# hiruna72/poregen

Measured on AMD Instinct MI355X. Metric: signal samples/sec aggregated into k-mer buckets, higher is better.
Workload: dtype int16 in / f64 arithmetic; 1 GPU; BASELINE configs[1]: synthetic rna004 SLOW5+PAF, 50000 reads x 4000 samples per GPU, k=5, scaling med-MAD, sample_limit=100, min/max_dur 20/40, --rna; reads_per_gpu=50000, samples_per_gpu=200000000, ss_ops_per_gpu=6499363, n_slots=1024, stats_mode=every read (as the reference), parallelism=read-shard x1

## Files before the change

### poregen_amd/csrc/pg_api.hip

```cpp
#include "../../include/pgmove.h"
#include "pg_internal.h"
#include "pg_hostmem.h"
#include "pg_hip_host.h"
#include "pg_select.h"
#include "pg_stats_plan.h"
#include "pg_model.h"
#include "pg_evstat.h"
#include "pg_modelcols.h"

#include <algorithm>
#include <thread>
#include <climits>
#include <cstdio>
#include <cstring>
#include <map>
#include <string>
#include <vector>

#define PG_VERSION_STR "pgmove 0.1.0 (gfx950)"

namespace {

hipError_t grow(PgDev<> &b, size_t bytes) { return b.ensure(bytes, bytes + bytes / 8 + 256); }

struct HostBatchResult {
    uint64_t n_reads = 0, n_events = 0, n_samples = 0;
    std::vector<uint64_t> keep, ev_off;
    BigVec64 samp_off;
    BigVec32 ev_len, ev_read;
    SampleVec samples;
    std::vector<uint8_t> skipped;
    PgDev<> dsamples; bool on_device = false;
    bool in_ctx = false;
};

struct ProfEntry { const char *name; hipEvent_t a, b; bool bracket; };

struct BatchState {
    PgStatsPlan plan{};
    uint32_t front_tiles = 0;
    bool in_submit = false;
    bool all_matches = false;
    bool cut_in_scan = false;
    bool stats_pending = false;
    bool rare_pending = false;
    PgRareArgs rare{};
};

}

struct pg_ctx {
    pg_params prm{};
    int device = 0;
    hipStream_t st = nullptr;
    PgStream st2, own_st;
    PgEvent ev_fork;
    PgEvent ev_join[2], ev_gathered[2];
    bool slot_used[2] = {false, false};
    PgPinned<PgSettlePack> settle_host;
    int slot = 0;
    bool user_stream = false, batch_is_host = false;
    std::string err;
    uint32_t n_codes = 0, key_bits = 1;

    PgDev<> table_t, table_u;
    int32_t tab_ok[2] = {0, 0}; uint32_t tab_lo[2] = {1, 1}, tab_hi[2] = {0, 0}; int32_t tab_delta[2] = {0, 0};
    PgDev<> s_sig, s_sig_off, s_dig, s_off, s_range, s_qs, s_ts, s_te, s_seq, s_seq_off, s_op_n, s_op_t, s_op_off;
    PgDev<> m_start, m_len, m_base, m_tix, ev_slot, status, errflag;
    PgDev<> sk[2], sv[2], hist, wcnt, totals, dbase, scount;
    PgDev<> slot_start, slot_end, acc_cnt, running, keep, keep32, ev_off, plan_totals, base_stage, tile_last;
    PgDev<> ev_rec, ev_len, ev_read, read_needed, samp_off, scan_scratch, samples;
    bool unpacked = false;
    uint32_t win_hint = 0;
    bool part_mode = false; uint32_t part_hi = 0, part_lo = 0;
    PgDev<> part_elem, part_lodig, part_rbase, part_tile_region, part_ntiles, part_histB, part_Bp, chunk_part, region_state; uint32_t region_epoch = 0;
    PgDev<> med[2], mad[2], gcal[2], read_plan[2], stat_status[2], stat_err[2], wide_list[2];
    PgDev<> long_ring; uint32_t long_seq = 0;
    PgDev<> meta, huge_scratch, oor;
    PgDev<> blk_read, gen_flag, gen_list, cum, btot, tile_read;
    uint32_t batch_id = 0;
    BatchState bt;
    uint64_t front_complete = 0, front_missed = 0, stats_cut_batches = 0, stats_cut_reads = 0, front_one_stream = 0;
    PgEvent ev_front;
    bool prev_one_stream = false;
    uint32_t gen_reads = 0;
    PgDev<> job_total, job_freq; bool have_job_totals = false;
    PgDev<> md_ev_off, md_samp_off, md_ev_len, md_samples, md_out, md_dwell, md_class;
    bool zero_running = false, totals_known = false;
    bool stats_in_flight = false;
    uint32_t wide_blocks = 0;
    PgDev<> cancel_flag; bool cancel_pending = false; uint64_t stats_cancelled = 0;
    PgDev<> long_tab, long_hist; uint32_t long_cap = 0, long_use = 0, long_want = 256; uint64_t long_reads_split = 0, long_helpers_short = 0;
    uint64_t gather_forms[PG_GATHER_FORMS] = {0, 0, 0, 0, 0};
    uint64_t sort_scatters = 0;

    PgDevBatch B{};
    bool have_count = false, have_batch_result = false, downloaded = true;
    int sorted_idx = 0;
    uint64_t cur_n_kept = 0, cur_n_samples = 0;
    uint64_t reads_before = 0;
    uint64_t full_slots = 0;
    bool full_before_batch = false;

    std::vector<HostBatchResult> batches;
    bool single_moved = false;
    bool want_samples = true;
    const double *fin_dev = nullptr;
    bool merged_valid = false;
    uint64_t m_events = 0, m_samples = 0, m_reads = 0;
    std::vector<uint64_t> r_counts, r_ev_off;
    BigVec64 r_samp_off;
    BigVec32 r_ev_len, r_ev_read;
    SampleVec r_samples;
    PgDev<> dmerged, dseg;
    PgDev<> tx_samp_off, tx_ev_off, tx_len, tx_off, tx_text, tx_slot_off, tx_flag;
    std::vector<uint64_t> tx_slot_off_host; uint64_t tx_bytes = 0;
    std::vector<uint8_t> r_skipped;
    std::vector<PgSlotModel> mo_raw;
    std::vector<PgSlotDwell> mo_dw;
    PgModelCols mo;
    PgDev<> me_mean, me_sd, me_flags, me_carry, me_id_off, me_len1, me_out, me_dw;
    std::vector<PgSlotModel> me_raw; std::vector<PgSlotDwell> me_rdw; std::vector<uint32_t> me_rflags;
    PgModelCols me_cm, me_cs;
    std::vector<uint32_t> me_status; std::vector<uint64_t> me_n;

    std::vector<ProfEntry> prof;
    std::vector<std::pair<hipEvent_t, hipEvent_t>> prof_pool;
    std::map<std::string, std::pair<uint64_t, double>> prof_acc;
    std::vector<std::string> prof_names;
};

static const char *read_status_text(int code) {
    switch (code) {
        case PGR_ERR_RNA: return "record is RNA-oriented (target_start > target_end) but allow_rna is 0 (gmove.cpp:795-797)";
        case PGR_ERR_NEG: return "negative PAF column or query_start >= len_raw_signal (assert at gmove.cpp:752)";
        case PGR_ERR_OP: return "ss op type outside {',','I','D'}";
        case PGR_ERR_SEQ_OVERRUN: return "ss consumes more bases than the fetched sequence holds (undefined in the reference, gmove.cpp:850-852)";
        case PGR_ERR_SHORT: return "fewer than k matched bases (unsigned wrap at gmove.cpp:891 in the reference)";
        case PGR_ERR_WINDOW: return "an accepted event has an empty/out-of-signal window or margin > start (undefined in the reference, gmove.cpp:928-941)";
        case PGR_ERR_RANGE: return "sample index exceeds INT32_MAX";
        case PGR_ERR_SCALE: return "range/digitisation is not a positive finite number";
        case PGR_ERR_WIDE: return "internal: statistics histogram too narrow for this read";
        case PGR_ERR_LAYOUT: return "op_off of the device batch is not monotone or ends behind pg_batch.n_ops";
        default: return "unknown";
    }
}

static void prof_begin(pg_ctx *c, const char *name, hipStream_t st, bool bracket = false) {
    if (!(c->prm.flags & PG_FLAG_PROFILE)) return;
    std::pair<hipEvent_t, hipEvent_t> ev;
    if (!c->prof_pool.empty()) { ev = c->prof_pool.back(); c->prof_pool.pop_back(); }
    else { (void)hipEventCreate(&ev.first); (void)hipEventCreate(&ev.second); }
    if (bracket) (void)hipEventRecord(ev.first, st);
    else { pg_prof_start = ev.first; pg_prof_stop = ev.second; }
    c->prof.push_back({name, ev.first, ev.second, bracket});
}
static void prof_end(pg_ctx *c, hipStream_t st) {
    if (!(c->prm.flags & PG_FLAG_PROFILE)) return;
    if (c->prof.back().bracket) { (void)hipEventRecord(c->prof.back().b, st); return; }
    if (pg_prof_start) {
        (void)hipEventRecord(c->prof.back().a, st); (void)hipEventRecord(c->prof.back().b, st);
        pg_prof_start = nullptr; pg_prof_stop = nullptr;
    }
}
static void prof_drain(pg_ctx *c) {
    for (auto &p : c->prof) {
        float ms = 0.f;
        if (hipEventElapsedTime(&ms, p.a, p.b) == hipSuccess) {
            auto it = c->prof_acc.find(p.name);
            if (it == c->prof_acc.end()) { c->prof_acc[p.name] = {1, (double)ms}; c->prof_names.push_back(p.name); }
            else { it->second.first++; it->second.second += ms; }
        }
        c->prof_pool.push_back({p.a, p.b});
    }
    c->prof.clear();
}

extern "C" {

const char *pg_version(void) { return PG_VERSION_STR; }

const char *pg_last_error(const pg_ctx *ctx) { return ctx ? ctx->err.c_str() : pg_create_error<pg_ctx>().c_str(); }

void pg_default_params(pg_params *p) {
    memset(p, 0, sizeof(*p));
    p->struct_size = sizeof(pg_params);
    p->kmer_size = 9; p->sig_move_offset = 0; p->signal_print_margin = 0; p->sample_limit = 100;
    p->max_dur = 70; p->min_dur = 5; p->kmer_pick_margin = 2; p->scaling = 0; p->allow_rna = 0;
    p->pa_min = 40.0; p->pa_max = 180.0; p->n_slots = 0; p->flags = 0; p->device = 0;
}

pg_status pg_build_slot_tables(uint32_t k, const char *const *kmers, uint32_t n_slots, int32_t *table_t, int32_t *table_u) {
    if (k < 1 || k > 13 || !kmers || !table_t || !table_u) return pg_fail<pg_ctx>(nullptr, PG_ERR_INVALID_ARG, "pg_build_slot_tables: bad arguments (1 <= k <= 13)");
    const size_t n_codes = (size_t)1 << (2 * k);
    for (size_t i = 0; i < n_codes; i++) table_t[i] = table_u[i] = -1;
    std::map<std::string, uint32_t> seen;
    for (uint32_t s = 0; s < n_slots; s++) {
        const char *km = kmers[s];
        if (!km || strlen(km) != k) return pg_fail<pg_ctx>(nullptr, PG_ERR_INVALID_ARG, "k-mer %u does not have length %u", s, k);
        if (!seen.emplace(km, s).second) return pg_fail<pg_ctx>(nullptr, PG_ERR_INVALID_ARG, "duplicate k-mer %s in the slice", km);
        uint32_t code = 0; bool has_t = false, has_u = false, other = false;
        for (uint32_t i = 0; i < k; i++) {
            uint32_t b;
            switch (km[i]) {
                case 'A': b = 0; break; case 'C': b = 1; break; case 'G': b = 2; break;
                case 'T': b = 3; has_t = true; break; case 'U': b = 3; has_u = true; break;
                default: b = 0; other = true;
            }
            code = (code << 2) | b;
        }
        if (other || (has_t && has_u)) continue;
        if (!has_u) table_t[code] = (int32_t)s;
        if (!has_t) table_u[code] = (int32_t)s;
    }
    return PG_OK;
}

void pg_destroy(pg_ctx *c) {
    if (!c) return;
    (void)hipSetDevice(c->device);
    if (c->st) (void)hipStreamSynchronize(c->st);
    if (c->st2) (void)hipStreamSynchronize(c->st2);
    for (auto &p : c->prof) { (void)hipEventDestroy(p.a); (void)hipEventDestroy(p.b); }
    for (auto &p : c->prof_pool) { (void)hipEventDestroy(p.first); (void)hipEventDestroy(p.second); }
    delete c;
}

static double wall_now() { struct timespec ts; clock_gettime(CLOCK_MONOTONIC, &ts); return ts.tv_sec + 1e-9 * ts.tv_nsec; }
static bool timing_on() { static const bool on = getenv("PGMOVE_TIMING") != nullptr; return on; }
#define PG_TMARK(label) do { if (timing_on()) { const double n_ = wall_now(); fprintf(stderr, "[pgmove timing] %-34s %8.3f ms\n", label, (n_ - tmark_) * 1e3); tmark_ = n_; } } while (0)

pg_status pg_runtime_init(int32_t device) {
    double tmark_ = timing_on() ? wall_now() : 0.0;
    if (timing_on()) {
        int ndev = 0;
// ... 115 lines not shown
    return PG_OK;
}

static pg_status settle_batch(pg_ctx *c);
static pg_status check_read_errors(pg_ctx *c, const PgSettlePack &pk);
static pg_status ensure_unpacked(pg_ctx *c);

static pg_status download_last(pg_ctx *c, bool more_coming) {
    if (!c->have_batch_result || c->downloaded) return PG_OK;
    { pg_status s0 = settle_batch(c); if (s0 != PG_OK) return s0; }
    c->batches.emplace_back();
    c->merged_valid = false;
    HostBatchResult &h = c->batches.back();
    const uint32_t ns = c->prm.n_slots;
    h.n_reads = c->B.n_reads; h.n_events = c->cur_n_kept; h.n_samples = c->cur_n_samples;
    h.keep.resize(ns); h.ev_off.resize(ns + 1); h.samp_off.resize(h.n_events + 1);
    h.ev_len.resize(h.n_events); h.ev_read.resize(h.n_events); h.samples.resize(h.n_samples);
    PG_HIP_TRY(c, hipMemcpy(h.keep.data(), c->keep.p, ns * 8ull, hipMemcpyDeviceToHost));
    PG_HIP_TRY(c, hipMemcpy(h.ev_off.data(), c->ev_off.p, (ns + 1) * 8ull, hipMemcpyDeviceToHost));
    if (h.n_events) {
        { pg_status su = ensure_unpacked(c); if (su != PG_OK) return su; }
        PG_HIP_TRY(c, hipMemcpy(h.samp_off.data(), c->samp_off.p, (h.n_events + 1) * 8ull, hipMemcpyDeviceToHost));
        PG_HIP_TRY(c, hipMemcpy(h.ev_len.data(), c->ev_len.p, h.n_events * 4ull, hipMemcpyDeviceToHost));
        PG_HIP_TRY(c, hipMemcpy(h.ev_read.data(), c->ev_read.p, h.n_events * 4ull, hipMemcpyDeviceToHost));
    } else h.samp_off[0] = 0;
    const char *hm = getenv("PGMOVE_HOLD_MIN_BYTES");
    const uint64_t hold_min = hm ? strtoull(hm, nullptr, 10) : (8ull << 20);
    if (h.n_samples && !c->want_samples && !more_coming && c->batches.size() == 1) {
        h.on_device = true; h.in_ctx = true;
        h.samples.clear(); h.samples.shrink_to_fit();
    } else if (h.n_samples && h.n_samples * 8ull >= hold_min && (more_coming || c->batches.size() > 1) && !getenv("PGMOVE_HOST_MERGE")) {
        if (grow(h.dsamples, h.n_samples * 8ull) == hipSuccess &&
            hipMemcpyAsync(h.dsamples.p, c->samples.p, h.n_samples * 8ull, hipMemcpyDeviceToDevice, c->st) == hipSuccess) {
            h.on_device = true;
            h.samples.clear(); h.samples.shrink_to_fit();
        } else { (void)hipGetLastError(); h.dsamples.release(); h.samples.resize(h.n_samples); }
    }
    if (h.n_samples && !h.on_device) {
        const uint64_t bytes = h.n_samples * 8ull;
        const unsigned parts = bytes >= (64ull << 20) ? 8u : 1u;
        if (parts == 1) PG_HIP_TRY(c, hipMemcpy(h.samples.data(), c->samples.p, bytes, hipMemcpyDeviceToHost));
        else {
            std::vector<hipError_t> rc(parts, hipSuccess);
            std::vector<std::thread> pool;
            const uint64_t step = ((h.n_samples + parts - 1) / parts + 511) & ~511ull;
            for (unsigned t = 0; t < parts; t++)
                pool.emplace_back([&, t]() {
                    const uint64_t a = std::min<uint64_t>(h.n_samples, t * step), b = std::min<uint64_t>(h.n_samples, a + step);
                    if (b <= a) return;
                    rc[t] = hipSetDevice(c->device);
                    if (rc[t] == hipSuccess) rc[t] = hipMemcpy(h.samples.data() + a, c->samples.as<double>() + a, (b - a) * 8ull, hipMemcpyDeviceToHost);
                });
            for (auto &th : pool) th.join();
            for (hipError_t e : rc) PG_HIP_TRY(c, e);
        }
    }
    std::vector<int32_t> st(h.n_reads);
    if (h.n_reads) PG_HIP_TRY(c, hipMemcpy(st.data(), c->status.p, h.n_reads * 4ull, hipMemcpyDeviceToHost));
    h.skipped.resize(h.n_reads);
    for (uint64_t i = 0; i < h.n_reads; i++) h.skipped[i] = st[i] == PGR_SKIPPED;
    c->downloaded = true;
    return PG_OK;
}

static pg_status stage_host_batch(pg_ctx *c, const pg_batch *b) {
    const uint32_t n = b->n_reads;
    if (!b->sig_off || !b->seq_off || !b->op_off) return pg_fail(c, PG_ERR_INVALID_ARG, "batch offsets missing");
    const uint64_t ns = b->sig_off[n], nq = b->seq_off[n], no = b->op_off[n];
    if (b->sig_off[0] != 0 || b->seq_off[0] != 0 || b->op_off[0] != 0) return pg_fail(c, PG_ERR_INVALID_ARG, "host batch offsets must start at 0");
    uint64_t helpers = 0;
    for (uint32_t r = 0; r < n; r++) {
        if (b->sig_off[r + 1] < b->sig_off[r] || b->seq_off[r + 1] < b->seq_off[r] || b->op_off[r + 1] < b->op_off[r])
            return pg_fail(c, PG_ERR_INVALID_ARG, "batch offsets of read %u are not monotone", r);
        const uint64_t L = b->sig_off[r + 1] - b->sig_off[r];
        if (L > PG_LONG_MIN) { uint32_t S; uint64_t sl; pg_long_geometry(L, &S, &sl); helpers += S - 1; }
    }
    c->long_want = (uint32_t)std::min<uint64_t>(helpers, 1u << 22);
    struct Item { PgDev<> *d; const void *src; size_t bytes; };
    Item items[] = {{&c->s_sig, b->sig, ns * 2}, {&c->s_sig_off, b->sig_off, (n + 1) * 8ull}, {&c->s_dig, b->digitisation, n * 8ull},
                    {&c->s_off, b->offset, n * 8ull}, {&c->s_range, b->range, n * 8ull}, {&c->s_qs, b->query_start, n * 4ull},
                    {&c->s_ts, b->target_start, n * 4ull}, {&c->s_te, b->target_end, n * 4ull}, {&c->s_seq, b->seq, nq},
                    {&c->s_seq_off, b->seq_off, (n + 1) * 8ull}, {&c->s_op_n, b->op_n, no * 4}, {&c->s_op_t, b->op_t, no},
                    {&c->s_op_off, b->op_off, (n + 1) * 8ull}};
    for (auto &it : items) {
        if (it.bytes && !it.src) return pg_fail(c, PG_ERR_INVALID_ARG, "batch array missing");
        PG_HIP_TRY(c, grow(*it.d, it.bytes + 16));
        if (it.bytes) PG_HIP_TRY(c, hipMemcpyAsync(it.d->p, it.src, it.bytes, hipMemcpyHostToDevice, c->st));
    }
    PgDevBatch &B = c->B;
    B.n_reads = n; B.n_ops = no;
    B.sig = c->s_sig.as<int16_t>(); B.sig_off = c->s_sig_off.as<uint64_t>();
    B.dig = c->s_dig.as<double>(); B.off = c->s_off.as<double>(); B.range = c->s_range.as<double>();
    B.qstart = c->s_qs.as<int32_t>(); B.tstart = c->s_ts.as<int32_t>(); B.tend = c->s_te.as<int32_t>();
    B.seq = c->s_seq.as<uint8_t>(); B.seq_off = c->s_seq_off.as<uint64_t>();
    B.op_n = c->s_op_n.as<uint32_t>(); B.op_t = c->s_op_t.as<uint8_t>(); B.op_off = c->s_op_off.as<uint64_t>();
    return PG_OK;
}

static pg_status check_read_errors(pg_ctx *c, const PgSettlePack &pk) {
    struct { unsigned long long word; int32_t layout, pad; uint32_t gen_count[2]; } ef;
    int32_t errv[1] = {INT_MAX}, errs[6] = {INT_MAX, 0, 0, 0, 0, 0};
    static_assert(sizeof ef == sizeof pk.errflag, "PgWalkOut's error words");
    memcpy(&ef, pk.errflag, sizeof ef);
    if (ef.layout) return pg_fail(c, PG_ERR_INVALID_ARG, "pg_batch.n_ops (%llu) is not op_off[n_reads] of the device batch", (unsigned long long)c->B.n_ops);
    if ((uint32_t)(ef.word >> 32) == c->batch_id) errv[0] = (int32_t)(0xFFFFFFFFu - (uint32_t)ef.word);
    c->gen_reads = ef.gen_count[c->batch_id & 1u];
    if (c->bt.all_matches && c->gen_reads) return pg_fail(c, PG_ERR_INVALID_ARG, "pg_batch.flags says PG_BATCH_ALL_MATCHES but %u reads hold I / D / unknown ops (or fewer ops than k, or more than bases)", c->gen_reads);
    memcpy(errs, pk.stat_err, sizeof errs);
    if (errs[4] > 0 || errs[5] > 0) {
        c->long_reads_split += (uint64_t)errs[5];
        if ((uint32_t)errs[4] > c->long_use) c->long_helpers_short++;
    }
    if (!c->batch_is_host) c->long_want = std::max<uint32_t>(256u, errs[4] > 0 ? (uint32_t)errs[4] : 0u);
    c->wide_blocks = errs[1] > 0 ? (uint32_t)errs[1] : 0u;
    if (c->bt.plan.place == PG_STATS_NONE) errs[0] = INT_MAX;
    if (errv[0] == INT_MAX && errs[0] == INT_MAX) return PG_OK;
    const bool walk = errv[0] <= errs[0];
    const int32_t idx = walk ? errv[0] : errs[0];
    if (c->prm.flags & PG_FLAG_STOP_WHEN_FULL) {
        if (c->full_before_batch) return PG_OK;
        const uint64_t tot[2] = {pk.n_kept, pk.full_slots};
        if (tot[1] == c->prm.n_slots && tot[0] == 0) return PG_OK;
        if (tot[1] == c->prm.n_slots && tot[0] > 0) {
            std::vector<uint32_t> er(tot[0]);
            const uint64_t kept_before = c->cur_n_kept; c->cur_n_kept = tot[0];
            const pg_status su = ensure_unpacked(c);
            c->cur_n_kept = kept_before; c->unpacked = false;
            if (su != PG_OK) return su;
            PG_HIP_TRY(c, hipMemcpy(er.data(), c->ev_read.p, tot[0] * 4ull, hipMemcpyDeviceToHost));
            uint32_t last = 0;
            for (uint32_t v : er) last = v > last ? v : last;
            if ((uint32_t)idx > last) return PG_OK;
        }
    }
    int32_t code = 0;
    PG_HIP_TRY(c, hipMemcpy(&code, (walk ? c->status.as<int32_t>() : c->stat_status[c->slot].as<int32_t>()) + idx, 4, hipMemcpyDeviceToHost));
    pg_status s = code == PGR_ERR_RNA ? PG_ERR_RNA_FLAG : (code == PGR_ERR_WIDE ? PG_ERR_UNSUPPORTED : (code == PGR_ERR_LAYOUT ? PG_ERR_INVALID_ARG : PG_ERR_INPUT));
    return pg_fail(c, s, "read %llu of the batch (global read %llu): %s", (unsigned long long)idx,
                (unsigned long long)(c->reads_before + idx), read_status_text(code));
}

static pg_status ensure_stats_buffers(pg_ctx *c) {
    const uint32_t n = c->B.n_reads;
    const int sl = c->slot;
    if (c->prm.flags & PG_FLAG_SKIP_OUT_OF_RANGE) PG_HIP_TRY(c, grow(c->oor, n + 1ull));
    PG_HIP_TRY(c, grow(c->med[sl], (n + 1) * 8ull)); PG_HIP_TRY(c, grow(c->mad[sl], (n + 1) * 8ull));
    PG_HIP_TRY(c, grow(c->gcal[sl], (n + 1) * 32ull));
    PG_HIP_TRY(c, grow(c->read_plan[sl], (n + 1) * (size_t)PG_STAT_REC_BYTES)); PG_HIP_TRY(c, grow(c->wide_list[sl], (n + 1) * 4ull));
    PG_HIP_TRY(c, grow(c->stat_status[sl], (n + 2) * 4ull)); PG_HIP_TRY(c, grow(c->huge_scratch, PG_HUGE_SCRATCH_WORDS * 4));
    return PG_OK;
}

static pg_status fill_long(pg_ctx *c, PgLongState &LS, bool ensure);
static pg_status launch_stats(pg_ctx *c) {
    const PgStatsPlan &P = c->bt.plan;
    hipStream_t st = pg_stats_on_second_stream(P.place) ? c->st2.h : c->st;
    const uint8_t *needed = P.place == PG_STATS_LAZY ? c->read_needed.as<uint8_t>() : nullptr;
    const int sl = c->slot;
    pg_status se = ensure_stats_buffers(c);
    if (se != PG_OK) return se;
    uint8_t *oor = P.place == PG_STATS_OOR_FIRST ? c->oor.as<uint8_t>() : nullptr;
    const int range_only = c->prm.scaling != 1;
    int32_t *flags = c->stat_err[sl].as<int32_t>();
    PgLongState LS{};
    { pg_status sl_ = fill_long(c, LS, false); if (sl_ != PG_OK) return sl_; }
    if (!P.records_in_init) {
        prof_begin(c, "k_read_plan", st);
        PG_HIP_TRY(c, pg_launch_read_plan(st, c->B, needed, c->prm.pa_min, c->prm.pa_max, c->read_plan[sl].p, flags, c->stat_status[sl].as<int32_t>(), P.flags_in_init, LS));
        prof_end(c, st);
    }
    const int win = (c->prm.flags & PG_FLAG_DEBUG_NARROW) ? 0 : 15;
    const bool cut = P.behind_cut;
    if (cut && P.place == PG_STATS_SECOND_STREAM) PG_HIP_TRY(c, hipStreamWaitEvent(st, c->ev_front, 0));
    uint32_t group_from = 0xffffffffu;
    if (cut) {
        const char *ov = getenv("PGMOVE_STATS_GROUP_FROM");
        group_from = ov ? (uint32_t)std::min<unsigned long long>(strtoull(ov, nullptr, 10), 0xffffffffull) : pg_stats_group_from(c->B.n_reads, c->B.n_ops, c->bt.front_tiles);
    }
    prof_begin(c, "k_read_stats", st);
    PG_HIP_TRY(c, pg_launch_read_stats(st, c->B, c->read_plan[sl].p, c->med[sl].as<double>(), c->mad[sl].as<double>(),
                         c->stat_status[sl].as<int32_t>(), flags, win, c->wide_list[sl].as<uint32_t>(), flags + 1, oor, range_only,
                         c->gcal[sl].as<double>(), LS, cut ? c->errflag.as<unsigned long long>() + 5 : nullptr, c->batch_id, group_from));
    prof_end(c, st);
    PgRareArgs &A = c->bt.rare;
    A.B = c->B; A.plan = c->read_plan[sl].as<PgStatRec>(); A.med = c->med[sl].as<double>(); A.mad = c->mad[sl].as<double>(); A.gcal = c->gcal[sl].as<double>();
    A.status = c->stat_status[sl].as<int32_t>(); A.err = flags; A.win = win; A.wide_list = c->wide_list[sl].as<uint32_t>(); A.wide_count = flags + 1;
    A.scratch = c->huge_scratch.as<uint32_t>(); A.oor = oor; A.range_only = range_only; A.wide_blocks = c->wide_blocks;
    if (P.rare_with_scan) c->bt.rare_pending = true;
    else {
        prof_begin(c, "k_read_stats_rare", st);
        PG_HIP_TRY(c, pg_launch_read_stats_rare(st, A));
        prof_end(c, st);
    }
    return PG_OK;
}

static void fill_walk(pg_ctx *c, PgWalkParams &W, PgWalkOut &O) {
    W.k = c->prm.kmer_size; W.sig_move_offset = c->prm.sig_move_offset; W.print_margin = c->prm.signal_print_margin;
    W.max_dur = c->prm.max_dur; W.min_dur = c->prm.min_dur; W.pick_margin = c->prm.kmer_pick_margin; W.allow_rna = c->prm.allow_rna;
    W.short_ok = (c->prm.flags & PG_FLAG_SHORT_READS_OK) ? 1 : 0;
    W.no_generic = c->bt.all_matches ? 1 : 0;
    W.n_codes = c->n_codes; W.table_t = c->table_t.as<int32_t>(); W.table_u = c->table_t.as<int32_t>() + c->n_codes;
    for (int x = 0; x < 2; x++) { W.aff_ok[x] = c->tab_ok[x]; W.aff_lo[x] = c->tab_lo[x]; W.aff_hi[x] = c->tab_hi[x]; W.aff_delta[x] = c->tab_delta[x]; }
    O.m_start = c->m_start.as<uint32_t>(); O.m_len = c->m_len.as<uint32_t>(); O.m_base = c->m_base.as<uint8_t>();
    O.m_tix = c->m_tix.as<uint32_t>() + PG_TIX_FRONT(c->prm.kmer_pick_margin); O.ev_slot = c->ev_slot.as<uint32_t>();
    O.meta = c->meta.as<PgReadMeta>();
    O.status = c->status.as<int32_t>();
    O.err = c->errflag.as<unsigned long long>(); O.layout_err = c->errflag.as<int32_t>() + 2; O.gen_count = c->errflag.as<uint32_t>() + 4;
    O.blk_read = c->blk_read.as<uint32_t>(); O.gen_flag = c->gen_flag.as<uint32_t>(); O.gen_list = c->gen_list.as<uint32_t>();
    O.cum = c->cum.as<uint32_t>(); O.btot = c->btot.as<uint32_t>(); O.batch_id = c->batch_id; O.tile_read = c->tile_read.as<uint32_t>();
    O.oor = (c->prm.flags & PG_FLAG_SKIP_OUT_OF_RANGE) ? c->oor.as<uint8_t>() : nullptr;
}

static pg_status fill_long(pg_ctx *c, PgLongState &LS, bool ensure) {
    LS = PgLongState{};
    if (getenv("PGMOVE_NO_LONG_SPLIT")) return PG_OK;
    if (ensure) {
        const char *ov = getenv("PGMOVE_LONG_HELPERS");
        uint32_t want = ov ? (uint32_t)strtoul(ov, nullptr, 10) : c->long_want;
        if (want > (1u << 22)) want = 1u << 22;
        if (want > c->long_cap || !c->long_tab.p) {
            const uint32_t cap = want + want / 4 + 64;
            PG_HIP_TRY(c, grow(c->long_tab, (size_t)cap * 8));
            const size_t before = c->long_hist.cap;
            PG_HIP_TRY(c, grow(c->long_hist, (size_t)cap * PG_LONG_WORDS * 4));
            if (c->long_hist.cap != before) {
                PG_HIP_TRY(c, hipMemsetAsync(c->long_hist.p, 0, c->long_hist.cap, c->st));
                PG_HIP_TRY(c, hipStreamSynchronize(c->st));
            }
            c->long_cap = cap;
        }
        c->long_use = ov ? std::min<uint32_t>(c->long_cap, want) : std::min<uint32_t>(c->long_cap, want + want / 4 + 64);
    }
    LS.tab = c->long_tab.as<uint2>(); LS.hist = c->long_hist.as<uint32_t>(); LS.cap = c->long_use;
    LS.cnt = c->long_ring.as<int32_t>() + 4u * (c->long_seq & 3u); LS.cnt_next = c->long_ring.as<int32_t>() + 4u * ((c->long_seq + 2u) & 3u);
    return PG_OK;
}

static void fill_sort(pg_ctx *c, PgSortBufs &S, uint32_t n_tiles) {
    S.keys[0] = c->sk[0].as<uint32_t>(); S.keys[1] = c->sk[1].as<uint32_t>();
    S.vals[0] = c->sv[0].as<uint32_t>(); S.vals[1] = c->sv[1].as<uint32_t>();
    S.hist = c->hist.as<uint32_t>(); S.wcnt = c->wcnt.as<uint32_t>(); S.totals = c->totals.as<uint32_t>();
    S.dbase = c->dbase.as<uint32_t>(); S.count = c->scount.as<uint32_t>(); S.n_tiles = n_tiles;
}

static int gather_lanes(const pg_ctx *c) {
    const char *ov = getenv("PGMOVE_GATHER_LANES");
    if (ov) return atoi(ov);
    const uint32_t mw = c->win_hint ? c->win_hint : c->prm.min_dur + (c->prm.max_dur > c->prm.min_dur ? (c->prm.max_dur - c->prm.min_dur) / 8 : 0) + 2 * c->prm.signal_print_margin;
    return mw > 16 ? 1 : 0;
}

static uint64_t dense_min() { const char *e = getenv("PGMOVE_DENSE_MIN"); return e ? strtoull(e, nullptr, 10) : 64ull * 4096; }
static bool dense_direct(const pg_ctx *c, uint64_t n_ops) {
    return c->prm.n_slots <= PG_DIRECT_MAX_SLOTS && std::min<uint64_t>(n_ops, (uint64_t)c->prm.n_slots * c->prm.sample_limit) > dense_min();
}

static uint32_t front_tiles_for(const pg_ctx *c, uint64_t n_ops, bool counts_wanted) {
    if (!c->bt.in_submit || counts_wanted || n_ops == 0 || c->prm.n_slots > PG_DIRECT_MAX_SLOTS || dense_direct(c, n_ops)) return 0;
    if (c->prm.sample_limit == 0 || c->prm.sig_move_offset != 0) return 0;
    const uint32_t n_tiles = pg_tiles(n_ops, true);
    uint64_t f;
    if (const char *ov = getenv("PGMOVE_FRONT_TILES")) f = (strtoull(ov, nullptr, 10) + 3) & ~3ull;
    else {
        f = ((n_tiles + 7) / 8 + 3) & ~3ull;
        if (n_tiles < 64 || f * PG_SORT_TILE < 4ull * c->prm.n_slots * c->prm.sample_limit) return 0;
    }
    return f > 0 && f < n_tiles ? (uint32_t)f : 0;
}

static void fill_part(pg_ctx *c, PgPartBufs &P, uint64_t n_ops) {
    P.elemA = c->part_elem.as<uint4>(); P.loA = c->part_lodig.as<uint16_t>(); P.hist = c->hist.as<uint32_t>(); P.totals = c->totals.as<uint32_t>(); P.rbase = c->part_rbase.as<uint32_t>();
    P.tile_region = c->part_tile_region.as<uint32_t>(); P.n_tilesB = c->part_ntiles.as<uint32_t>(); P.histB = c->part_histB.as<uint32_t>();
    P.Bp = c->part_Bp.as<uint32_t>(); P.hi_bits = c->part_hi; P.lo_bits = c->part_lo; P.tilesB_cap = pg_part_tiles_cap(n_ops, c->part_hi);
}

static pg_status ensure_unpacked(pg_ctx *c) {
    if (c->unpacked) return PG_OK;
    PG_HIP_TRY(c, grow(c->ev_len, (c->cur_n_kept + 1) * 4)); PG_HIP_TRY(c, grow(c->ev_read, (c->cur_n_kept + 1) * 4));
    PG_HIP_TRY(c, pg_launch_unpack_recs(c->st, c->ev_rec.as<PgKeptRec>(), c->cur_n_kept, c->ev_len.as<uint32_t>(), c->ev_read.as<uint32_t>()));
    PG_HIP_TRY(c, hipStreamSynchronize(c->st));
    c->unpacked = true;
    return PG_OK;
}

static pg_status count_impl(pg_ctx *c, const pg_batch *b, uint64_t *counts_out, int32_t counts_location, bool in_submit) {
    if (!c || !b) return PG_ERR_INVALID_ARG;
    if (b->struct_size != sizeof(pg_batch)) return pg_fail(c, PG_ERR_INVALID_ARG, "pg_batch.struct_size mismatch");
    PG_HIP_TRY(c, hipSetDevice(c->device));
    pg_status s = download_last(c, true);
    if (s != PG_OK) return s;
    for (auto &hb : c->batches)
        if (hb.in_ctx) {
            PG_HIP_TRY(c, grow(hb.dsamples, hb.n_samples * 8ull));
            PG_HIP_TRY(c, hipMemcpyAsync(hb.dsamples.p, c->samples.p, hb.n_samples * 8ull, hipMemcpyDeviceToDevice, c->st));
            hb.in_ctx = false; c->merged_valid = false; c->fin_dev = nullptr;
        }
    if (c->have_batch_result) { c->reads_before += c->B.n_reads; c->have_batch_result = false; }
    c->have_count = false;
    c->bt = BatchState{};
    c->bt.in_submit = in_submit;
    const uint32_t n = b->n_reads;

    double tmark_ = timing_on() ? wall_now() : 0.0;
    c->batch_is_host = b->location == PG_LOC_HOST;
    c->bt.all_matches = (b->flags & PG_BATCH_ALL_MATCHES) != 0 && !(c->prm.flags & PG_FLAG_DEBUG_SPLIT_WALK);
    if (b->location == PG_LOC_HOST) {
        s = stage_host_batch(c, b);
        if (s != PG_OK) return s;
        PG_TMARK("count: staging copies queued");
        if (timing_on()) { PG_HIP_TRY(c, hipStreamSynchronize(c->st)); PG_TMARK("count: staging copies done (sync)"); }
    } else if (b->location == PG_LOC_DEVICE) {
        PgDevBatch &B = c->B;
        B.sig = b->sig; B.sig_off = b->sig_off; B.dig = b->digitisation; B.off = b->offset; B.range = b->range;
        B.qstart = b->query_start; B.tstart = b->target_start; B.tend = b->target_end; B.seq = b->seq; B.seq_off = b->seq_off;
        B.op_n = b->op_n; B.op_t = b->op_t; B.op_off = b->op_off;
        if (!B.sig_off || !B.seq_off || !B.op_off) return pg_fail(c, PG_ERR_INVALID_ARG, "batch offsets missing");
        uint64_t no = b->n_ops;
        if (no == 0 && n > 0) {
            PG_HIP_TRY(c, hipMemcpyAsync(&no, b->op_off + n, 8, hipMemcpyDeviceToHost, c->st));
            PG_HIP_TRY(c, hipStreamSynchronize(c->st));
        }
        B.n_reads = n;
        B.n_ops = no;
    } else return pg_fail(c, PG_ERR_INVALID_ARG, "pg_batch.location must be PG_LOC_HOST or PG_LOC_DEVICE");
    if (((uintptr_t)c->B.sig & 15) != 0) return pg_fail(c, PG_ERR_INVALID_ARG, "sig must be 16-byte aligned");
    if (((uintptr_t)c->B.seq & 3) != 0 || ((uintptr_t)c->B.op_n & 15) != 0) return pg_fail(c, PG_ERR_INVALID_ARG, "seq must be 4-byte aligned and op_n 16-byte aligned");
    const uint64_t N = c->B.n_ops;
    if (N >= 0x7fffffffull) return pg_fail(c, PG_ERR_INVALID_ARG, "more than 2^31 ss ops in one batch; split the batch");

    const uint64_t Nn = N ? N : 1;
    const bool direct = c->prm.n_slots <= PG_DIRECT_MAX_SLOTS;
    PG_HIP_TRY(c, grow(c->m_start, (Nn + 32) * 4)); PG_HIP_TRY(c, grow(c->m_len, (Nn + 32) * 4)); PG_HIP_TRY(c, grow(c->m_base, Nn + 32));
    PG_HIP_TRY(c, grow(c->m_tix, (Nn + 64 + c->prm.kmer_size + 2 * PG_TIX_FRONT(c->prm.kmer_pick_margin)) * 4));
    PG_HIP_TRY(c, grow(c->ev_slot, (Nn + 32) * 4));
    PG_HIP_TRY(c, grow(c->blk_read, (Nn / 64 + 2) * 4)); PG_HIP_TRY(c, grow(c->cum, (Nn / 4 + 64) * 4)); PG_HIP_TRY(c, grow(c->btot, (Nn / 256 + 2) * 4));
    PG_HIP_TRY(c, grow(c->gen_list, (n + 1) * 4ull)); PG_HIP_TRY(c, grow(c->tile_read, (Nn / PG_SORT_TILE + 8) * 4));
    {
        const size_t before = c->gen_flag.cap;
        PG_HIP_TRY(c, grow(c->gen_flag, (n + 1) * 4ull));
        if (c->gen_flag.cap != before) PG_HIP_TRY(c, hipMemsetAsync(c->gen_flag.p, 0, c->gen_flag.cap, c->st));
    }
    if (++c->batch_id == 0) {
        c->batch_id = 1;
        PG_HIP_TRY(c, hipMemsetAsync(c->gen_flag.p, 0, c->gen_flag.cap, c->st));
        PG_HIP_TRY(c, hipMemsetAsync(c->errflag.as<uint32_t>() + 8, 0, 16, c->st));
    }
    PG_HIP_TRY(c, grow(c->meta, (n + 1) * sizeof(PgReadMeta))); PG_HIP_TRY(c, grow(c->status, (n + 1) * 4ull));
    PG_HIP_TRY(c, grow(c->read_needed, n + 2ull));
    const uint32_t n_tiles = pg_tiles(Nn, direct);
    uint32_t ndig;
    if (direct) {
        ndig = 2; while (ndig < c->prm.n_slots) ndig <<= 1;
        if (dense_direct(c, N)) { PG_HIP_TRY(c, grow(c->part_Bp, (Nn / 256 + 4) * 4)); PG_HIP_TRY(c, grow(c->chunk_part, PG_CHUNK_PART_N * 8)); }
    }
    else if (c->part_mode) {
        ndig = 1u << c->part_hi;
        const uint32_t tcap = pg_part_tiles_cap(Nn, c->part_hi);
        PG_HIP_TRY(c, grow(c->part_elem, (size_t)tcap * PG_SORT_TILE * 16)); PG_HIP_TRY(c, grow(c->part_lodig, (size_t)tcap * PG_SORT_TILE * 2)); PG_HIP_TRY(c, grow(c->part_rbase, (ndig + 2) * 4ull));
        PG_HIP_TRY(c, grow(c->part_tile_region, (tcap + 1) * 4ull)); PG_HIP_TRY(c, grow(c->part_ntiles, 16));
        PG_HIP_TRY(c, grow(c->part_histB, ((size_t)tcap << c->part_lo) * 4)); PG_HIP_TRY(c, grow(c->part_Bp, (Nn / 256 + 4) * 4));
        PG_HIP_TRY(c, grow(c->chunk_part, PG_CHUNK_PART_N * 8));
    } else {
        const uint32_t passes = (c->key_bits + PG_RANK_MAX_BITS - 1) / PG_RANK_MAX_BITS;
        ndig = 1u << ((c->key_bits + passes - 1) / passes);
        for (int i = 0; i < 2; i++) { PG_HIP_TRY(c, grow(c->sk[i], Nn * 4)); PG_HIP_TRY(c, grow(c->sv[i], Nn * 4)); }
    }
    const uint32_t n_tiles_hist = c->part_mode ? pg_tiles(Nn, true) : n_tiles;
    PG_HIP_TRY(c, grow(c->hist, (size_t)n_tiles_hist * ndig * 4));
    if (!direct && !c->part_mode) PG_HIP_TRY(c, grow(c->wcnt, (size_t)n_tiles * ndig * 16));
    PG_HIP_TRY(c, grow(c->totals, ndig * 4ull)); PG_HIP_TRY(c, grow(c->dbase, ndig * 4ull));

    PG_TMARK("count: work buffers");
    c->full_before_batch = c->full_slots == c->prm.n_slots && c->prm.n_slots > 0;
    c->slot ^= 1;
    c->bt.front_tiles = front_tiles_for(c, N, counts_out != nullptr);
    const PgFront FR{c->bt.front_tiles, c->errflag.as<uint32_t>() + 8};
    const PgStatsPlan P = c->bt.plan = pg_stats_plan(c->prm.flags, c->prm.scaling, FR.tiles, n, getenv("PGMOVE_FRONT_TWO_STREAMS") != nullptr);
    if (P.one_stream_batch && c->stats_in_flight) PG_HIP_TRY(c, hipStreamWaitEvent(c->st, c->ev_join[c->slot ^ 1], 0));
    if (P.place == PG_STATS_SECOND_STREAM) {
        if (pg_stats_fork_waits(c->batch_is_host, c->user_stream, (b->flags & PG_BATCH_RESIDENT) != 0, c->prev_one_stream)) {
            PG_HIP_TRY(c, hipEventRecord(c->ev_fork, c->st));
            PG_HIP_TRY(c, hipStreamWaitEvent(c->st2, c->ev_fork, 0));
        }
        if (c->slot_used[c->slot]) PG_HIP_TRY(c, hipStreamWaitEvent(c->st2, c->ev_gathered[c->slot], 0));
    }
    c->prev_one_stream = P.one_stream_batch;
    if (P.records_in_init) { pg_status se = ensure_stats_buffers(c); if (se != PG_OK) return se; }
    PgWalkParams W{}; PgWalkOut O{};
    fill_walk(c, W, O);
    const bool force_generic = (c->prm.flags & PG_FLAG_DEBUG_SPLIT_WALK) != 0;
    PgLongState LS{};
    ++c->long_seq;
    { pg_status sl_ = fill_long(c, LS, true); if (sl_ != PG_OK) return sl_; }
    prof_begin(c, "k_batch_init", c->st);
    PG_HIP_TRY(c, pg_launch_batch_init(c->st, n, c->read_needed.as<uint8_t>(), c->running.as<uint64_t>(), c->prm.n_slots,
                         c->zero_running ? 1 : 0, P.flags_in_init ? c->stat_err[c->slot].as<int32_t>() : nullptr, c->B, c->prm.pa_min, c->prm.pa_max,
                         P.records_in_init ? c->read_plan[c->slot].p : nullptr, P.records_in_init ? c->stat_status[c->slot].as<int32_t>() : nullptr,
                         W, O, force_generic ? 1 : 0, LS, FR.tiles ? FR.word + 1 : nullptr));
    prof_end(c, c->st);
    c->zero_running = false;

    if (P.place == PG_STATS_OOR_FIRST) {
        pg_status s2 = launch_stats(c); if (s2 != PG_OK) return s2;
        PG_HIP_TRY(c, pg_launch_apply_oor(c->st, c->B, O));
    }
    if (!c->bt.all_matches) {
        prof_begin(c, "k_walk", c->st);
        PG_HIP_TRY(c, pg_launch_walk(c->st, c->B, W, O));
        prof_end(c, c->st);
    }

    PgSortBufs S{};
    fill_sort(c, S, n_tiles);
    prof_begin(c, "k_events", c->st);
    PG_HIP_TRY(c, pg_launch_events(c->st, c->B, W, O, c->prm.n_slots, (direct || c->part_mode) ? S.hist : nullptr, c->part_mode ? c->part_hi : 0u, c->part_lo,
                                   FR, FR.tiles ? PG_PASS_FRONT : PG_PASS_WHOLE));
    prof_end(c, c->st);
    uint64_t *acc_copy = (counts_out && counts_location == PG_LOC_DEVICE) ? counts_out : nullptr;
    if (direct) {
        prof_begin(c, "rank_scan", c->st);
        const bool fuse_plan = c->bt.in_submit;
        PG_HIP_TRY(c, pg_launch_rank_direct_count(c->st, O.ev_slot, N, c->prm.n_slots, S, c->acc_cnt.as<uint64_t>(), c->running.as<uint64_t>(), c->prm.sample_limit,
                                    c->tile_last.as<int32_t>(), acc_copy, fuse_plan ? c->keep.as<uint64_t>() : nullptr, c->ev_off.as<uint64_t>(),
                                    c->plan_totals.as<uint64_t>(), c->errflag.as<uint32_t>() + 6, &c->bt.cut_in_scan,
                                    O.btot, dense_direct(c, N) ? c->part_Bp.as<uint32_t>() : nullptr, dense_direct(c, N) ? c->chunk_part.as<uint64_t>() : nullptr,
                                    FR, FR.tiles ? PG_PASS_FRONT : PG_PASS_WHOLE, c->batch_id, O.tile_read, n));
        prof_end(c, c->st);
        if (P.behind_cut && P.place == PG_STATS_SECOND_STREAM) PG_HIP_TRY(c, hipEventRecord(c->ev_front, c->st));
        if (FR.tiles) {
            prof_begin(c, "k_events_tail", c->st);
            PG_HIP_TRY(c, pg_launch_events(c->st, c->B, W, O, c->prm.n_slots, S.hist, 0u, 0u, FR, PG_PASS_TAIL));
            prof_end(c, c->st);
            prof_begin(c, "rank_scan_tail", c->st);
            PG_HIP_TRY(c, pg_launch_rank_direct_count(c->st, O.ev_slot, N, c->prm.n_slots, S, c->acc_cnt.as<uint64_t>(), c->running.as<uint64_t>(), c->prm.sample_limit,
                                        c->tile_last.as<int32_t>(), nullptr, c->keep.as<uint64_t>(), c->ev_off.as<uint64_t>(), c->plan_totals.as<uint64_t>(),
                                        c->errflag.as<uint32_t>() + 6, &c->bt.cut_in_scan, O.btot, nullptr, nullptr, FR, PG_PASS_TAIL, c->batch_id));
            prof_end(c, c->st);
        }
    } else if (c->part_mode) {
        PgPartBufs P{};
        fill_part(c, P, Nn);
        if (N) {
            prof_begin(c, "part_tile_scan", c->st);
            PG_HIP_TRY(c, pg_launch_part_tile_scan(c->st, P, N, O.btot, c->chunk_part.as<uint64_t>()));
            prof_end(c, c->st);
            prof_begin(c, "k_part_bases", c->st);
            PG_HIP_TRY(c, pg_launch_part_bases(c->st, P, c->B, O));
            prof_end(c, c->st);
            prof_begin(c, "k_part_scatter", c->st);
            PG_HIP_TRY(c, pg_launch_part_scatter(c->st, P, O.ev_slot, N, c->B, W, O));
            prof_end(c, c->st);
            PgRegionCutArgs cut{};
            const bool fuse_cut = c->bt.in_submit && !acc_copy && !getenv("PGMOVE_NO_FUSED_CUT");
            if (fuse_cut) {
                const size_t before = c->region_state.cap;
                PG_HIP_TRY(c, grow(c->region_state, ((size_t)(1u << c->part_hi) + 2) * 8));
                if (c->region_state.cap != before) PG_HIP_TRY(c, hipMemsetAsync(c->region_state.p, 0, c->region_state.cap, c->st));
                if (++c->region_epoch > pg_region_cut_epochs()) { c->region_epoch = 1; PG_HIP_TRY(c, hipMemsetAsync(c->region_state.p, 0, c->region_state.cap, c->st)); }
                PG_HIP_TRY(c, grow(c->keep32, c->prm.n_slots * 4ull));
                cut.running = c->running.as<uint64_t>(); cut.keep = c->keep.as<uint64_t>(); cut.ev_off = c->ev_off.as<uint64_t>(); cut.totals = c->plan_totals.as<uint64_t>();
                cut.keep32 = c->keep32.as<uint32_t>(); cut.state = c->region_state.as<uint64_t>(); cut.limit = c->prm.sample_limit; cut.epoch = c->region_epoch;
            }
            prof_begin(c, "region_counts", c->st, true);
            PG_HIP_TRY(c, pg_launch_region_counts(c->st, P, c->prm.n_slots, c->acc_cnt.as<uint64_t>(), acc_copy, fuse_cut ? &cut : nullptr));
            prof_end(c, c->st);
            c->bt.cut_in_scan = fuse_cut;
        } else {
            PG_HIP_TRY(c, hipMemsetAsync(c->acc_cnt.p, 0, c->prm.n_slots * 8ull, c->st));
            if (acc_copy) PG_HIP_TRY(c, hipMemsetAsync(acc_copy, 0, c->prm.n_slots * 8ull, c->st));
            PG_HIP_TRY(c, hipMemsetAsync(c->part_ntiles.p, 0, 4, c->st));
        }
    } else {
        prof_begin(c, "sort_events", c->st, true);
        if (N) PG_HIP_TRY(c, pg_launch_sort_events(c->st, O.ev_slot, N, c->key_bits, S, &c->sorted_idx, &c->sort_scatters));
        else { c->sorted_idx = 0; PG_HIP_TRY(c, hipMemsetAsync(c->scount.p, 0, 8, c->st)); }
        prof_end(c, c->st);
        prof_begin(c, "slot_bounds", c->st, true);
        PG_HIP_TRY(c, pg_launch_slot_bounds(c->st, S.keys[c->sorted_idx], S.count, N, c->slot_start.as<uint32_t>(), c->slot_end.as<uint32_t>(),
                              c->prm.n_slots, c->acc_cnt.as<uint64_t>(), acc_copy));
        prof_end(c, c->st);
    }

    c->stats_in_flight = false;
    c->bt.stats_pending = P.place == PG_STATS_DEFERRED;
    if (P.place == PG_STATS_SECOND_STREAM || P.place == PG_STATS_CHAIN || P.place == PG_STATS_TAIL_FORK) {
        if (P.place == PG_STATS_TAIL_FORK) {
            PG_HIP_TRY(c, hipEventRecord(c->ev_fork, c->st));
            PG_HIP_TRY(c, hipStreamWaitEvent(c->st2, c->ev_fork, 0));
        }
        pg_status s2 = launch_stats(c);
        if (s2 != PG_OK) return s2;
        if (pg_stats_on_second_stream(P.place)) {
            PG_HIP_TRY(c, hipEventRecord(c->ev_join[c->slot], c->st2));
            c->stats_in_flight = true;
        }
    }

    if (counts_out && counts_location != PG_LOC_DEVICE) {
        PG_HIP_TRY(c, hipMemcpyAsync(counts_out, c->acc_cnt.p, c->prm.n_slots * 8ull, hipMemcpyDeviceToHost, c->st));
        PG_HIP_TRY(c, hipStreamSynchronize(c->st));
    }
    c->have_count = true;
    PG_TMARK("count: kernels queued");
    if (timing_on()) { PG_HIP_TRY(c, hipStreamSynchronize(c->st)); PG_TMARK("count: kernels done (sync)"); }
    return PG_OK;
}

static pg_status collect_impl(pg_ctx *c, const uint64_t *base, int32_t base_location, const uint64_t *all_counts, uint32_t world, uint32_t rank);

pg_status pg_count(pg_ctx *c, const pg_batch *b, uint64_t *counts_out, int32_t counts_location) { return count_impl(c, b, counts_out, counts_location, false); }

static pg_status launch_pending_stats(pg_ctx *c) {
    if (!c->bt.stats_pending) return PG_OK;
    c->bt.stats_pending = false;
    return launch_stats(c);
}

pg_status pg_stats(pg_ctx *c) {
    if (!c) return PG_ERR_INVALID_ARG;
    if (!c->have_count) return pg_fail(c, PG_ERR_STATE, "pg_stats without a preceding pg_count");
    if (!c->bt.stats_pending) return PG_OK;
    PG_HIP_TRY(c, hipSetDevice(c->device));
    return launch_pending_stats(c);
}

pg_status pgi_stats_gathered(pg_ctx *c, const uint64_t *all_counts, uint32_t world, uint32_t rank) {
    if (!c) return PG_ERR_INVALID_ARG;
    if (!c->have_count) return pg_fail(c, PG_ERR_STATE, "pgi_stats_gathered without a preceding pg_count");
    if (!all_counts || rank >= world) return pg_fail(c, PG_ERR_INVALID_ARG, "pgi_stats_gathered: all_counts / world / rank");
    if (!c->bt.stats_pending) return PG_OK;
    if (rank == 0 || c->prm.sample_limit == 0 || !c->bt.plan.records_in_init) return pg_stats(c);
    PG_HIP_TRY(c, hipSetDevice(c->device));
    { pg_status se = ensure_stats_buffers(c); if (se != PG_OK) return se; }
    PG_HIP_TRY(c, grow(c->cancel_flag, 16));
    PG_HIP_TRY(c, pg_launch_stats_cancel_if_full(c->st, all_counts, rank, c->prm.n_slots, c->prm.sample_limit, c->cancel_flag.as<uint32_t>(),
                                              c->read_plan[c->slot].p, c->B.n_reads));
    c->cancel_pending = true;
    return launch_pending_stats(c);
}

pg_status pg_collect(pg_ctx *c, const uint64_t *base, int32_t base_location) { return collect_impl(c, base, base_location, nullptr, 0, 0); }

pg_status pg_collect_gathered(pg_ctx *c, const uint64_t *all_counts, uint32_t world, uint32_t rank) {
    if (!c) return PG_ERR_INVALID_ARG;
    if (!all_counts || world == 0 || rank >= world) return pg_fail(c, PG_ERR_INVALID_ARG, "pg_collect_gathered: all_counts / world / rank");
    return collect_impl(c, nullptr, PG_LOC_DEVICE, all_counts, world, rank);
}

static pg_status collect_impl(pg_ctx *c, const uint64_t *base, int32_t base_location, const uint64_t *all_counts, uint32_t world, uint32_t rank) {
    if (!c) return PG_ERR_INVALID_ARG;
    if (!c->have_count) return pg_fail(c, PG_ERR_STATE, "pg_collect without a preceding pg_count");
    PG_HIP_TRY(c, hipSetDevice(c->device));
    double tmark_ = timing_on() ? wall_now() : 0.0;
    { pg_status s2 = launch_pending_stats(c); if (s2 != PG_OK) return s2; }
    const uint32_t ns = c->prm.n_slots;
    const uint64_t N = c->B.n_ops;
    const bool direct = ns <= PG_DIRECT_MAX_SLOTS;
    const uint64_t *d_base = c->running.as<uint64_t>();
    PgGathered G{};
    if (all_counts) {
        G.all_counts = all_counts; G.world = world; G.rank = rank; G.total = c->job_total.as<uint64_t>(); G.freq = c->job_freq.as<uint64_t>();
        c->have_job_totals = true;
        d_base = nullptr;
    } else if (base) {
        PG_HIP_TRY(c, hipMemcpyAsync(c->base_stage.p, base, ns * 8ull,
                                  base_location == PG_LOC_DEVICE ? hipMemcpyDeviceToDevice : hipMemcpyHostToDevice, c->st));
        d_base = c->base_stage.as<uint64_t>();
    }
    uint64_t *totals = c->plan_totals.as<uint64_t>();
    const uint64_t ke_cap = std::min<uint64_t>(N, (uint64_t)ns * c->prm.sample_limit);
    {
        const size_t before = c->scan_scratch.cap;
        PG_HIP_TRY(c, grow(c->scan_scratch, (std::max<uint64_t>(ke_cap, ns) / 4096 + 84) * 8));
        if (c->scan_scratch.cap != before) PG_HIP_TRY(c, hipMemsetAsync(c->scan_scratch.p, 0, c->scan_scratch.cap, c->st));
    }
    if (!direct) PG_HIP_TRY(c, grow(c->keep32, ns * 4ull));
    const bool plan_in_scan = c->bt.cut_in_scan && !all_counts && !base;
    c->bt.cut_in_scan = false;
    if (!plan_in_scan) {
    prof_begin(c, "k_slot_plan", c->st, true);
    PG_HIP_TRY(c, pg_launch_slot_plan(c->st, c->acc_cnt.as<uint64_t>(), d_base, c->running.as<uint64_t>(), c->prm.sample_limit, ns,
                        c->keep.as<uint64_t>(), c->ev_off.as<uint64_t>(), totals, direct ? c->hist.as<uint32_t>() : nullptr,
                        pg_tiles(N ? N : 1, true), direct ? nullptr : c->keep32.as<uint32_t>(), c->scan_scratch.as<uint64_t>(),
                        direct ? c->tile_last.as<int32_t>() : nullptr, G));
    prof_end(c, c->st);
    }

    const uint64_t win_cap = (uint64_t)c->prm.max_dur + 2ull * c->prm.signal_print_margin;
    const uint64_t samp_cap = ke_cap * win_cap;
    PG_HIP_TRY(c, grow(c->ev_rec, (ke_cap + 1) * sizeof(PgKeptRec)));
    PG_HIP_TRY(c, grow(c->samp_off, (ke_cap + 2) * 8));
    c->unpacked = false;

    PgWalkParams W{}; PgWalkOut O{};
    fill_walk(c, W, O);
    PgKeptOut K{};
    K.rec = c->ev_rec.as<PgKeptRec>();
    K.read_needed = c->bt.plan.place == PG_STATS_LAZY ? c->read_needed.as<uint8_t>() : nullptr;
    const bool chunked = ke_cap > dense_min() && (win_cap + 1) * 4096 < (1ull << 32);
    bool sums_ready = false;
    if (chunked) PG_HIP_TRY(c, grow(c->chunk_part, PG_CHUNK_PART_N * 8));
    if (direct) {
        PgSortBufs S{};
        fill_sort(c, S, 0);
        prof_begin(c, "k_rank_emit", c->st);
        if (dense_direct(c, N)) PG_HIP_TRY(c, pg_launch_rank_emit2(c->st, O.ev_slot, N, ns, S.hist, c->keep.as<uint64_t>(), c->ev_off.as<uint64_t>(), totals, c->B, W, O, K, c->part_Bp.as<uint32_t>()));
        else PG_HIP_TRY(c, pg_launch_rank_direct_emit(c->st, O.ev_slot, N, ns, S, c->keep.as<uint64_t>(), c->ev_off.as<uint64_t>(), totals, c->B, W, O, K));
        prof_end(c, c->st);
    } else if (c->part_mode) {
        PgPartBufs P{};
        fill_part(c, P, N ? N : 1);
        if (N) {
            prof_begin(c, "k_region_place", c->st);
            PG_HIP_TRY(c, pg_launch_region_place(c->st, P, ns, c->keep32.as<uint32_t>(), c->ev_off.as<uint64_t>(), O, K, chunked ? c->chunk_part.as<uint64_t>() : nullptr, chunked ? ke_cap : 0));
            prof_end(c, c->st);
            sums_ready = chunked;
        }
    } else {
        prof_begin(c, "k_kept_meta", c->st, true);
        PG_HIP_TRY(c, pg_launch_kept_meta(c->st, c->sk[c->sorted_idx].as<uint32_t>(), c->sv[c->sorted_idx].as<uint32_t>(), c->scount.as<uint32_t>(), N,
                            c->slot_start.as<uint32_t>(), c->keep.as<uint64_t>(), c->ev_off.as<uint64_t>(), c->B, W, O, K,
                            c->sv[c->sorted_idx ^ 1].as<uint32_t>()));
        prof_end(c, c->st);
    }

    if (c->bt.plan.place == PG_STATS_LAZY) { pg_status s2 = launch_stats(c); if (s2 != PG_OK) return s2; }

    uint64_t gather_cap = ke_cap;
    if (chunked) {
        if (!sums_ready) {
            if (!(direct && dense_direct(c, N)) && !c->part_mode) PG_HIP_TRY(c, hipMemsetAsync(c->chunk_part.p, 0, PG_CHUNK_PART_N * 8, c->st));
            prof_begin(c, "len_partials", c->st);
            PG_HIP_TRY(c, pg_launch_len_partials(c->st, ke_cap, totals, c->ev_rec.as<PgKeptRec>(), c->chunk_part.as<uint64_t>(), c->bt.rare_pending ? &c->bt.rare : nullptr));
            prof_end(c, c->st);
        } else if (c->bt.rare_pending) {
            prof_begin(c, "k_read_stats_rare", c->st);
            PG_HIP_TRY(c, pg_launch_read_stats_rare(c->st, c->bt.rare));
            prof_end(c, c->st);
        }
        c->bt.rare_pending = false;
    } else {
        prof_begin(c, "scan_ev_len", c->st, (ke_cap + 4095) / 4096 > 64);
        PG_HIP_TRY(c, pg_launch_scan_u32_u64(c->st, reinterpret_cast<const uint32_t *>(c->ev_rec.p) + 2, 4, ke_cap, totals, c->samp_off.as<uint64_t>(), c->scan_scratch.as<uint64_t>(),
                                          c->bt.rare_pending ? &c->bt.rare : nullptr, totals + 2));
        c->bt.rare_pending = false;
        prof_end(c, c->st);
    }

    if (samp_cap * 8 > c->samples.cap) {
        size_t mem_free = 0, mem_total = 0;
        if (hipMemGetInfo(&mem_free, &mem_total) != hipSuccess) { (void)hipGetLastError(); mem_total = 0; }
        const uint64_t moderate = std::max<uint64_t>(4ull << 30, std::min<uint64_t>(mem_total / 8, mem_free / 2));
        bool sized = false;
        if (samp_cap * 8 <= moderate && !getenv("PGMOVE_SAMPLES_EXACT")) {
            sized = grow(c->samples, samp_cap * 8 + 8) == hipSuccess;
            if (!sized) (void)hipGetLastError();
        }
        if (!sized) {
            uint64_t tot[3] = {0, 0, 0};
            PG_HIP_TRY(c, hipMemcpyAsync(tot, totals, 24, hipMemcpyDeviceToHost, c->st));
            if (chunked) {
                uint64_t coarse[PG_CHUNK_COARSE];
                PG_HIP_TRY(c, hipMemcpyAsync(coarse, c->chunk_part.as<uint64_t>() + PG_CHUNK_FINE, sizeof coarse, hipMemcpyDeviceToHost, c->st));
                PG_HIP_TRY(c, hipStreamSynchronize(c->st));
                tot[2] = 0;
                for (uint64_t v : coarse) tot[2] += v;
            } else PG_HIP_TRY(c, hipStreamSynchronize(c->st));
            PG_HIP_TRY(c, grow(c->samples, (tot[2] + 1) * 8));
            gather_cap = tot[0];
        }
    }
    if (c->stats_in_flight) { PG_HIP_TRY(c, hipStreamWaitEvent(c->st, c->ev_join[c->slot], 0)); c->stats_in_flight = false; }
    prof_begin(c, "k_gather", c->st);
    const int lanes = chunked ? gather_lanes(c) : 0;
    if (chunked) c->gather_forms[pg_gather_form(lanes)]++;
    if (chunked)
        PG_HIP_TRY(c, pg_launch_gather_chunks(c->st, c->B, ke_cap, totals, c->ev_rec.as<PgKeptRec>(), c->chunk_part.as<uint64_t>(), c->samp_off.as<uint64_t>(), totals + 2, c->prm.scaling,
                                           c->prm.pa_min, c->prm.pa_max, c->samples.as<double>(), c->prm.scaling == 1 ? c->gcal[c->slot].as<double>() : nullptr, lanes,
                                           c->prm.scaling == 1 ? c->stat_err[c->slot].as<int32_t>() : nullptr));
    else
        PG_HIP_TRY(c, pg_launch_gather(c->st, c->B, gather_cap, totals, c->ev_rec.as<PgKeptRec>(),
                     c->samp_off.as<uint64_t>(), c->prm.scaling, c->prm.pa_min, c->prm.pa_max, c->med[c->slot].as<double>(), c->mad[c->slot].as<double>(),
                     c->samples.as<double>(), c->prm.scaling == 1 ? c->gcal[c->slot].as<double>() : nullptr));
    prof_end(c, c->st);
    if (c->st2) PG_HIP_TRY(c, hipEventRecord(c->ev_gathered[c->slot], c->st));
    PG_TMARK("collect: buffers + kernels queued");
    if (timing_on()) { PG_HIP_TRY(c, hipStreamSynchronize(c->st)); PG_TMARK("collect: kernels done (sync)"); }
    c->slot_used[c->slot] = true;
    c->have_count = false; c->have_batch_result = true; c->downloaded = false; c->totals_known = false;
    return PG_OK;
}

static pg_status settle_batch(pg_ctx *c) {
    if (!c->have_batch_result || c->totals_known) return PG_OK;
    if (c->st2) PG_HIP_TRY(c, hipStreamSynchronize(c->st2));
    PG_HIP_TRY(c, pg_launch_settle_pack(c->st, c->errflag.as<uint32_t>(), c->stat_err[c->slot].as<int32_t>(), c->long_ring.as<int32_t>() + 4u * (c->long_seq & 3u), c->plan_totals.as<uint64_t>(),
                                     c->samp_off.as<uint64_t>(), c->samp_off.cap / 8, c->cancel_pending ? c->cancel_flag.as<uint32_t>() : nullptr,
                                     c->bt.front_tiles ? c->errflag.as<uint32_t>() + 8 : nullptr, c->settle_host.p));
    PG_HIP_TRY(c, hipStreamSynchronize(c->st));
    const PgSettlePack pk = *c->settle_host.p;
    if (c->bt.front_tiles) { if (pk.front[0]) c->front_complete++; else c->front_missed++; }
    if (c->bt.plan.one_stream_batch) c->front_one_stream++;
    if (c->bt.plan.behind_cut && pk.front[0]) { c->stats_cut_batches++; c->stats_cut_reads += c->B.n_reads - std::min(pk.front[1], c->B.n_reads); }
    pg_status s = check_read_errors(c, pk);
    if (s != PG_OK) { c->have_batch_result = false; c->downloaded = true; return s; }
    const uint64_t tot[2] = {pk.n_kept, pk.full_slots};
    c->cur_n_kept = tot[0]; c->full_slots = tot[1];
    const uint64_t n_samples = pk.n_samples;
    c->cur_n_samples = n_samples;
    if (c->cancel_pending) {
        if (pk.cancel[1]) c->stats_cancelled++;
        c->cancel_pending = false;
    }
    if (tot[0]) c->win_hint = (uint32_t)((n_samples + tot[0] - 1) / tot[0]);
    c->totals_known = true;
    return PG_OK;
}

pg_status pg_submit(pg_ctx *c, const pg_batch *b) {
    if (!c) return PG_ERR_INVALID_ARG;
    pg_status s = count_impl(c, b, nullptr, PG_LOC_HOST, true);
    if (s != PG_OK) return s;
    return pg_collect(c, nullptr, PG_LOC_HOST);
}

pg_status pg_job_totals_device(pg_ctx *c, const uint64_t **d_total, const uint64_t **d_freq) {
    if (!c) return PG_ERR_INVALID_ARG;
    if (!c->have_job_totals) return pg_fail(c, PG_ERR_STATE, "pg_job_totals_device without a preceding pg_collect_gathered");
    if (d_total) *d_total = c->job_total.as<uint64_t>();
    if (d_freq) *d_freq = c->job_freq.as<uint64_t>();
    return PG_OK;
}

pg_status pg_sync(pg_ctx *c) {
    if (!c) return PG_ERR_INVALID_ARG;
    PG_HIP_TRY(c, hipSetDevice(c->device));
    PG_HIP_TRY(c, hipStreamSynchronize(c->st));
    if (c->st2) PG_HIP_TRY(c, hipStreamSynchronize(c->st2));
    return settle_batch(c);
}

pg_status pg_set_stream(pg_ctx *c, void *hip_stream) {
    if (!c) return PG_ERR_INVALID_ARG;
    PG_HIP_TRY(c, hipSetDevice(c->device));
    PG_HIP_TRY(c, hipStreamSynchronize(c->st));
    if (c->st2) PG_HIP_TRY(c, hipStreamSynchronize(c->st2));
    c->prev_one_stream = false;
    c->st = hip_stream ? (hipStream_t)hip_stream : c->own_st;
    c->user_stream = hip_stream != nullptr;
    return PG_OK;
}

void *pgi_stream(pg_ctx *c) { return c ? (void *)c->st : nullptr; }
const double *pgi_fin_dev(pg_ctx *c) { return c && c->merged_valid ? c->fin_dev : nullptr; }
pg_status pgi_skip_stats(pg_ctx *c) {
    if (!c) return PG_ERR_INVALID_ARG;
    if (!c->have_count) return pg_fail(c, PG_ERR_STATE, "pgi_skip_stats without a preceding pg_count");
    c->bt.stats_pending = false;
    return PG_OK;
}

int32_t pg_all_slots_full(pg_ctx *c) {
    if (!c) return 0;
    if (settle_batch(c) != PG_OK) return 0;
    return c->full_slots == c->prm.n_slots;
}

int32_t pg_poll(pg_ctx *c) {
    if (!c) return PG_ERR_INVALID_ARG;
    if (!c->have_batch_result || c->totals_known) return 1;
    if (hipSetDevice(c->device) != hipSuccess) return PG_ERR_HIP;
    if (hipStreamQuery(c->st) != hipSuccess || (c->st2 && hipStreamQuery(c->st2) != hipSuccess)) { (void)hipGetLastError(); return 0; }
    const pg_status s = settle_batch(c);
    return s == PG_OK ? 1 : s;
}

int32_t pg_all_slots_full_settled(const pg_ctx *c) { return c && c->full_slots == c->prm.n_slots; }
uint64_t pgi_full_slots_settled(const pg_ctx *c) { return c ? c->full_slots : 0; }

pg_status pg_last_batch_device(pg_ctx *c, pg_device_view *v) {
    if (!c || !v) return PG_ERR_INVALID_ARG;
    if (!c->have_batch_result) return pg_fail(c, PG_ERR_STATE, "no collected batch");
    { pg_status s0 = settle_batch(c); if (s0 != PG_OK) return s0; }
    { pg_status su = ensure_unpacked(c); if (su != PG_OK) return su; }
    v->n_events = c->cur_n_kept; v->n_samples = c->cur_n_samples;
    v->d_keep = c->keep.as<uint64_t>(); v->d_ev_off = c->ev_off.as<uint64_t>(); v->d_ev_len = c->ev_len.as<uint32_t>();
    v->d_ev_read = c->ev_read.as<uint32_t>(); v->d_samp_off = c->samp_off.as<uint64_t>(); v->d_samples = c->samples.as<double>();
    v->d_med = c->prm.scaling == 1 ? c->med[c->slot].as<double>() : nullptr; v->d_mad = c->prm.scaling == 1 ? c->mad[c->slot].as<double>() : nullptr;
    return PG_OK;
}

pg_status pg_finish(pg_ctx *c, pg_result *out) {
    if (!c || !out) return PG_ERR_INVALID_ARG;
    PG_HIP_TRY(c, hipSetDevice(c->device));
    pg_status s = download_last(c, false);
    if (s != PG_OK) return s;
    const uint32_t ns = c->prm.n_slots;
    if (c->merged_valid && c->want_samples && c->fin_dev && c->m_samples) {
        c->r_samples.resize(c->m_samples);
        PG_HIP_TRY(c, hipMemcpy(c->r_samples.data(), c->fin_dev, c->m_samples * 8ull, hipMemcpyDeviceToHost));
        c->fin_dev = nullptr;
        for (auto &hb : c->batches) if (hb.on_device && c->batches.size() == 1) { hb.on_device = false; hb.in_ctx = false; hb.dsamples.release(); }
    }
    if (c->merged_valid) {
        out->n_slots = ns; out->reserved = 0; out->n_events = c->m_events; out->n_samples = c->m_samples; out->n_reads = c->m_reads;
        out->counts = c->r_counts.data(); out->ev_off = c->r_ev_off.data(); out->ev_len = c->r_ev_len.data();
        out->ev_read = c->r_ev_read.data(); out->samp_off = c->r_samp_off.data(); out->samples = c->fin_dev ? nullptr : c->r_samples.data();
        out->read_skipped = c->r_skipped.data();
        return PG_OK;
    }
    if (c->single_moved && !c->batches.empty()) {
        HostBatchResult &h = c->batches[0];
        c->r_ev_off.swap(h.ev_off); c->r_samp_off.swap(h.samp_off); c->r_ev_len.swap(h.ev_len); c->r_ev_read.swap(h.ev_read);
        c->r_samples.swap(h.samples); c->r_skipped.swap(h.skipped);
    }
    c->single_moved = false;
    uint64_t n_events = 0, n_samples = 0, n_reads = 0;
    for (auto &h : c->batches) { n_events += h.n_events; n_samples += h.n_samples; n_reads += h.n_reads; }
    if (c->batches.size() == 1) {
        HostBatchResult &h = c->batches[0];
        c->fin_dev = nullptr;
        if (h.on_device && !c->want_samples) c->fin_dev = h.in_ctx ? c->samples.as<double>() : h.dsamples.as<double>();
        else if (h.on_device) {
            h.samples.resize(h.n_samples);
            PG_HIP_TRY(c, hipMemcpy(h.samples.data(), h.in_ctx ? c->samples.p : h.dsamples.p, h.n_samples * 8ull, hipMemcpyDeviceToHost));
            h.dsamples.release(); h.on_device = false; h.in_ctx = false;
        }
        c->r_counts.resize(ns);
        for (uint32_t sl = 0; sl < ns; sl++) c->r_counts[sl] = h.ev_off[sl + 1] - h.ev_off[sl];
        c->r_ev_off.swap(h.ev_off); c->r_samp_off.swap(h.samp_off); c->r_ev_len.swap(h.ev_len); c->r_ev_read.swap(h.ev_read);
        c->r_samples.swap(h.samples); c->r_skipped.swap(h.skipped);
        c->single_moved = true;
        out->n_slots = ns; out->reserved = 0; out->n_events = n_events; out->n_samples = n_samples; out->n_reads = n_reads;
        out->counts = c->r_counts.data(); out->ev_off = c->r_ev_off.data(); out->ev_len = c->r_ev_len.data();
        out->ev_read = c->r_ev_read.data(); out->samp_off = c->r_samp_off.data(); out->samples = c->fin_dev ? nullptr : c->r_samples.data();
        out->read_skipped = c->r_skipped.data();
        c->merged_valid = true; c->m_events = n_events; c->m_samples = n_samples; c->m_reads = n_reads;
        return PG_OK;
    }
    c->fin_dev = nullptr;
    c->r_counts.assign(ns, 0); c->r_ev_off.assign(ns + 1, 0); c->r_samp_off.resize(n_events + 1);
    c->r_ev_len.resize(n_events); c->r_ev_read.resize(n_events);
    c->r_skipped.resize(n_reads);
    std::vector<uint64_t> slot_e(ns + 1, 0), slot_s(ns + 1, 0);
    for (uint32_t sl = 0; sl < ns; sl++) {
        uint64_t ne = 0, nsmp = 0;
        for (auto &h : c->batches) { const uint64_t a = h.ev_off[sl], b = h.ev_off[sl + 1]; ne += b - a; nsmp += h.samp_off[b] - h.samp_off[a]; }
        slot_e[sl + 1] = slot_e[sl] + ne; slot_s[sl + 1] = slot_s[sl] + nsmp;
        c->r_counts[sl] = ne; c->r_ev_off[sl] = slot_e[sl];
    }
    bool all_dev = true;
    for (auto &h : c->batches) if (h.n_samples && !h.on_device) all_dev = false;
    if (all_dev && n_samples) {
        size_t nseg = 0;
        for (uint32_t sl = 0; sl < ns; sl++) for (auto &h : c->batches) nseg += h.ev_off[sl + 1] > h.ev_off[sl];
// ... 186 lines not shown
    c->mo.fill(*out, flags);
    return PG_OK;
}

static pg_status model_arrays(pg_ctx *c, pg_result &R, const uint64_t *&d_ev_off, const uint64_t *&d_samp_off, const uint32_t *&d_ev_len, const double *&d_samples) {
    pg_status s = pg_finish_deferred(c, &R);
    if (s != PG_OK) return s;
    const uint32_t ns = c->prm.n_slots;
    if (c->batches.size() == 1 && c->have_batch_result && c->cur_n_kept == R.n_events && c->cur_n_samples == R.n_samples) {
        { pg_status su = ensure_unpacked(c); if (su != PG_OK) return su; }
        d_ev_off = c->ev_off.as<uint64_t>(); d_samp_off = c->samp_off.as<uint64_t>(); d_ev_len = c->ev_len.as<uint32_t>(); d_samples = c->samples.as<double>();
    } else {
        PG_HIP_TRY(c, grow(c->md_ev_off, (ns + 1) * 8ull)); PG_HIP_TRY(c, grow(c->md_samp_off, (R.n_events + 1) * 8ull));
        PG_HIP_TRY(c, grow(c->md_ev_len, R.n_events * 4ull + 4));
        PG_HIP_TRY(c, hipMemcpyAsync(c->md_ev_off.p, R.ev_off, (ns + 1) * 8ull, hipMemcpyHostToDevice, c->st));
        PG_HIP_TRY(c, hipMemcpyAsync(c->md_samp_off.p, R.samp_off, (R.n_events + 1) * 8ull, hipMemcpyHostToDevice, c->st));
        if (R.n_events) PG_HIP_TRY(c, hipMemcpyAsync(c->md_ev_len.p, R.ev_len, R.n_events * 4ull, hipMemcpyHostToDevice, c->st));
        if (c->fin_dev || !R.n_samples) d_samples = c->fin_dev;
        else {
            PG_HIP_TRY(c, grow(c->md_samples, R.n_samples * 8ull + 8));
            PG_HIP_TRY(c, hipMemcpyAsync(c->md_samples.p, R.samples, R.n_samples * 8ull, hipMemcpyHostToDevice, c->st));
            d_samples = c->md_samples.as<double>();
        }
        d_ev_off = c->md_ev_off.as<uint64_t>(); d_samp_off = c->md_samp_off.as<uint64_t>(); d_ev_len = c->md_ev_len.as<uint32_t>();
    }
    return PG_OK;
}

pg_status pg_model(pg_ctx *c, uint32_t flags, pg_model_result *out) {
    if (!c || !out) return PG_ERR_INVALID_ARG;
    pg_result R;
    const uint64_t *d_ev_off, *d_samp_off; const uint32_t *d_ev_len; const double *d_samples;
    if (pg_status s = model_arrays(c, R, d_ev_off, d_samp_off, d_ev_len, d_samples)) return s;
    const uint32_t ns = c->prm.n_slots;
    int any_kind[PG_MODEL_KINDS] = {0, 0, 0, 0};
    const uint64_t drop = (flags & PG_MODEL_KEEP_FIRST) ? 0 : 1;
    for (uint32_t i = 0; i < ns; i++) {
        const uint64_t all = R.samp_off[R.ev_off[i + 1]] - R.samp_off[R.ev_off[i]], nv = all > drop ? all - drop : 0;
        any_kind[pg_model_kind(nv, R.ev_off[i + 1] - R.ev_off[i])]++;
    }
    return model_run(c, ns, any_kind, d_ev_off, d_samp_off, d_ev_len, d_samples, flags, out);
}

pg_status pg_model_events(pg_ctx *c, uint32_t flags, pg_events_result *out) {
    if (!c || !out) return PG_ERR_INVALID_ARG;
    if (flags) return pg_fail(c, PG_ERR_INVALID_ARG, "pg_model_events: unknown flags 0x%x", flags);
    pg_result R;
    const uint64_t *d_ev_off, *d_samp_off; const uint32_t *d_ev_len; const double *d_samples;
    if (pg_status s = model_arrays(c, R, d_ev_off, d_samp_off, d_ev_len, d_samples)) return s;
    const uint32_t ns = c->prm.n_slots;
    const uint64_t ne = R.n_events, nv = R.n_samples;
    if (ne && R.samp_off[0] != 0) return pg_fail(c, PG_ERR_UNSUPPORTED, "pg_model_events: the kept samples' offsets do not begin at 0");
    for (uint64_t e = 0; e < ne; e++)
        if (R.ev_len[e] == 0) return pg_fail(c, PG_ERR_UNSUPPORTED, "pg_model_events: kept event %llu holds no sample", (unsigned long long)e);
    PG_HIP_TRY(c, grow(c->me_mean, (ne + 1) * 8)); PG_HIP_TRY(c, grow(c->me_sd, (ne + 1) * 8)); PG_HIP_TRY(c, grow(c->me_flags, (ns + 1) * 4ull));
    PG_HIP_TRY(c, grow(c->me_carry, pg_ev_carry_bytes(nv))); PG_HIP_TRY(c, grow(c->me_id_off, (ne + 1) * 8)); PG_HIP_TRY(c, grow(c->me_len1, (ne + 1) * 4));
    PG_HIP_TRY(c, grow(c->me_out, 2 * (ns + 1ull) * sizeof(PgSlotModel))); PG_HIP_TRY(c, grow(c->me_dw, 2 * (ns + 1ull) * sizeof(PgSlotDwell)));
    PG_HIP_TRY(c, grow(c->md_class, pg_slot_model_scratch_bytes(ns)));
    int64_t *ev_mean = c->me_mean.as<int64_t>(), *ev_sd = c->me_sd.as<int64_t>();
    PgSlotModel *om = c->me_out.as<PgSlotModel>(); PgSlotDwell *od = c->me_dw.as<PgSlotDwell>();
    PG_HIP_TRY(c, hipMemsetAsync(c->me_flags.p, 0, (ns + 1) * 4ull, c->st));
    PG_HIP_TRY(c, pg_launch_ev_identity(c->st, ne, c->me_id_off.as<uint64_t>(), c->me_len1.as<uint32_t>()));
    prof_begin(c, "k_ev_stats", c->st, true);
    PG_HIP_TRY(c, pg_launch_ev_stats(c->st, ns, d_ev_off, d_samp_off, d_samples, ne, nv, ev_mean, ev_sd, c->me_flags.as<uint32_t>(), c->me_carry.p));
    prof_end(c, c->st);
    const int all_kinds[PG_MODEL_KINDS] = {1 << 20, 1 << 20, 1 << 20, 1 << 20};
    PG_HIP_TRY(c, pg_launch_slot_model_units(c->st, ns, all_kinds, d_ev_off, c->me_id_off.as<uint64_t>(), c->me_len1.as<uint32_t>(), ev_mean, 0u, om, od, c->md_class.p));
    PG_HIP_TRY(c, pg_launch_slot_model_units(c->st, ns, all_kinds, d_ev_off, c->me_id_off.as<uint64_t>(), c->me_len1.as<uint32_t>(), ev_sd, 0u, om + ns, od + ns, c->md_class.p));
    c->me_raw.resize(2 * (size_t)ns); c->me_rdw.resize(2 * (size_t)ns); c->me_rflags.resize(ns);
    if (ns) {
        PG_HIP_TRY(c, hipMemcpyAsync(c->me_raw.data(), om, 2 * (size_t)ns * sizeof(PgSlotModel), hipMemcpyDeviceToHost, c->st));
        PG_HIP_TRY(c, hipMemcpyAsync(c->me_rdw.data(), od, 2 * (size_t)ns * sizeof(PgSlotDwell), hipMemcpyDeviceToHost, c->st));
        PG_HIP_TRY(c, hipMemcpyAsync(c->me_rflags.data(), c->me_flags.p, (size_t)ns * 4, hipMemcpyDeviceToHost, c->st));
    }
    PG_HIP_TRY(c, hipStreamSynchronize(c->st));
    c->me_cm.clear(); c->me_cs.clear(); c->me_status.clear(); c->me_n.clear();
    for (uint32_t i = 0; i < ns; i++) {
        const uint32_t declined = (c->me_rdw[i].flags | c->me_rdw[ns + i].flags) & (PG_MODEL_BAD_VALUE | PG_MODEL_BAD_SPREAD | PG_MODEL_BAD_COUNT);
        uint32_t st = (c->me_rflags[i] & 15u) << 1;
        if (!st && declined) st = PG_EVENTS_DECLINED;
        c->me_status.push_back(st); c->me_n.push_back(R.ev_off[i + 1] - R.ev_off[i]);
        c->me_cm.push(st ? PgSlotModel{} : c->me_raw[i]); c->me_cs.push(st ? PgSlotModel{} : c->me_raw[ns + i]);
    }
    c->me_cm.fill(out->means, PG_MODEL_KEEP_FIRST); c->me_cs.fill(out->sds, PG_MODEL_KEEP_FIRST);
    out->status = c->me_status.data(); out->n_events = c->me_n.data();
    return PG_OK;
}

pg_status pg_model_device(pg_ctx *c, uint32_t n_slots, const uint64_t *d_ev_off, const uint64_t *d_samp_off, const uint32_t *d_ev_len,
                          const double *d_samples, uint32_t flags, pg_model_result *out) {
    if (!c || !out) return PG_ERR_INVALID_ARG;
    if (n_slots && (!d_ev_off || !d_samp_off)) return pg_fail(c, PG_ERR_INVALID_ARG, "pg_model_device: ev_off / samp_off missing");
    PG_HIP_TRY(c, hipSetDevice(c->device));
    const int all_kinds[PG_MODEL_KINDS] = {1 << 20, 1 << 20, 1 << 20, 1 << 20};
    return model_run(c, n_slots, all_kinds, d_ev_off, d_samp_off, d_ev_len, d_samples, flags, out);
}

size_t pg_model_format(const pg_model_result *m, uint32_t slot, int32_t which, char *buf, size_t cap) {
    if (!m || !buf || cap == 0 || slot >= m->n_slots) return 0;
    int w = 0;
    buf[0] = 0;
    if (which == PG_MODEL_TEXT_DWELL) {
        if (m->dwell_n[slot] == 0) return 0;
        w = snprintf(buf, cap, "%.14Lg", (long double)m->dwell_median[slot]);
    } else if (which == PG_MODEL_TEXT_MEDIAN || which == PG_MODEL_TEXT_SSTDEV) {
        if (m->n_values[slot] == 0) return 0;
        PgSlotModel r{};
        r.n = m->n_values[slot]; r.mid_lo = m->mid_lo[slot]; r.mid_hi = m->mid_hi[slot]; r.s1 = m->sum1[slot];
        if (which == PG_MODEL_TEXT_MEDIAN) w = snprintf(buf, cap, "%.14Lg", pg_model_median(r));
        else if (r.n < 2) w = snprintf(buf, cap, "nan");
        else {
            const unsigned __int128 s2 = ((unsigned __int128)m->sum2_hi[slot] << 64) | m->sum2_lo[slot];
            const __int128 s1 = r.s1;
            const unsigned __int128 num = (unsigned __int128)r.n * s2 - (unsigned __int128)(s1 * s1);
            w = pg_model_sstdev_text(r.n, num, buf, cap);
        }
    } else return 0;
    return (w < 0 || (size_t)w >= cap) ? 0 : (size_t)w;
}

pg_status pg_kernel_stats(pg_ctx *c, pg_kernel_stat *out, uint32_t cap, uint32_t *n_out) {
    if (!c || !n_out) return PG_ERR_INVALID_ARG;
    PG_HIP_TRY(c, hipSetDevice(c->device));
    PG_HIP_TRY(c, hipStreamSynchronize(c->st));
    if (c->st2) PG_HIP_TRY(c, hipStreamSynchronize(c->st2));
    prof_drain(c);
    uint32_t n = 0;
    for (auto &name : c->prof_names) {
        if (out && n < cap) { auto &a = c->prof_acc[name]; out[n].name = name.c_str(); out[n].launches = a.first; out[n].total_ms = a.second; }
        n++;
    }
    if (c->stats_cancelled) {
        if (out && n < cap) { out[n].name = "stats_cancelled_on_device"; out[n].launches = c->stats_cancelled; out[n].total_ms = 0.0; }
        n++;
    }
    if (c->long_reads_split) {
        if (out && n < cap) { out[n].name = "long_reads_split"; out[n].launches = c->long_reads_split; out[n].total_ms = 0.0; }
        n++;
    }
    if (c->front_complete) {
        if (out && n < cap) { out[n].name = "front_complete"; out[n].launches = c->front_complete; out[n].total_ms = 0.0; }
        n++;
    }
    if (c->front_missed) {
        if (out && n < cap) { out[n].name = "front_missed"; out[n].launches = c->front_missed; out[n].total_ms = 0.0; }
        n++;
    }
    if (c->stats_cut_batches) {
        if (out && n < cap) { out[n].name = "stats_cut_batches"; out[n].launches = c->stats_cut_batches; out[n].total_ms = 0.0; }
        n++;
        if (out && n < cap) { out[n].name = "stats_cut_reads"; out[n].launches = c->stats_cut_reads; out[n].total_ms = 0.0; }
        n++;
    }
    if (c->front_one_stream) {
        if (out && n < cap) { out[n].name = "front_one_stream"; out[n].launches = c->front_one_stream; out[n].total_ms = 0.0; }
        n++;
    }
    if (c->long_helpers_short) {
        if (out && n < cap) { out[n].name = "long_helpers_short_batches"; out[n].launches = c->long_helpers_short; out[n].total_ms = 0.0; }
        n++;
    }
    static const char *const form_names[PG_GATHER_FORMS] = {"gather_form_wave", "gather_form_evpair", "gather_form_lanes4", "gather_form_lanes8", "gather_form_lanes16"};
    for (int f = 0; f < PG_GATHER_FORMS; ++f)
        if (c->gather_forms[f]) {
            if (out && n < cap) { out[n].name = form_names[f]; out[n].launches = c->gather_forms[f]; out[n].total_ms = 0.0; }
            n++;
        }
    if (c->sort_scatters) {
        if (out && n < cap) { out[n].name = "k_sort_scatter"; out[n].launches = c->sort_scatters; out[n].total_ms = 0.0; }
        n++;
    }
    *n_out = n;
    return PG_OK;
}

pg_status pg_kernel_stats_reset(pg_ctx *c) {
    if (!c) return PG_ERR_INVALID_ARG;
    PG_HIP_TRY(c, hipStreamSynchronize(c->st));
    if (c->st2) PG_HIP_TRY(c, hipStreamSynchronize(c->st2));
    prof_drain(c);
    c->prof_acc.clear(); c->prof_names.clear(); c->stats_cancelled = 0; c->long_reads_split = 0; c->long_helpers_short = 0; c->front_complete = 0; c->front_missed = 0; c->stats_cut_batches = 0; c->stats_cut_reads = 0; c->front_one_stream = 0;
    for (uint64_t &f : c->gather_forms) f = 0;
    c->sort_scatters = 0;
    return PG_OK;
}

}
```

### poregen_amd/csrc/pg_hosttest.cpp

```cpp
#include "pg_select.h"
#include <vector>
#include <cstdint>
#include <cstring>

extern "C" int pgt_plan(double dig, double off, double range, double pa_min, double pa_max, int32_t *out4) {
    PgReadPlan p = pg_make_plan(dig, off, range, pa_min, pa_max);
    out4[0] = p.c_lo; out4[1] = p.span; out4[2] = p.z0; out4[3] = p.status;
    return p.status;
}

extern "C" int pgt_medmad(const int16_t *raw, uint64_t n, double dig, double off, double range,
                          double pa_min, double pa_max, double *med, double *mad, double *mad_raw) {
    PgReadPlan p = pg_make_plan(dig, off, range, pa_min, pa_max);
    if (p.status != 0) return p.status;
    std::vector<uint32_t> pre((size_t)(p.span > 0 ? p.span : 1), 0u);
    for (uint64_t i = 0; i < n; i++) {
        int idx = (int)raw[i] - p.c_lo;
        if (idx >= 0 && idx < p.span) pre[(size_t)idx]++;
    }
    for (int b = 1; b < p.span; b++) pre[(size_t)b] += pre[(size_t)b - 1];
    PgMedMad mm = pg_medmad_from_prefix(pre.data(), p, n, off, range / dig);
    *med = mm.med; *mad = mm.mad; *mad_raw = mm.mad_raw;
    return 0;
}
// ... 22 lines not shown
}
extern "C" int pgt_div_domain_ok(double offset, double scale) { return pg_div_domain_ok(offset, scale) ? 1 : 0; }

#include "host/pg_host.h"
#include <cstring>
#include <string>

extern "C" size_t pgt_format_f8(double v, char *buf) { return pgh::format_f8(v, buf); }

extern "C" long pgt_tokenize_ss(const char *ss, uint32_t *op_n, uint8_t *op_t, size_t cap) {
    std::vector<uint32_t> n; std::vector<uint8_t> t; std::string err;
    if (!pgh::tokenize_ss(ss, strlen(ss), n, t, err)) return -1;
    for (size_t i = 0; i < n.size() && i < cap; i++) { op_n[i] = n[i]; op_t[i] = t[i]; }
    return (long)n.size();
}

extern "C" long pgt_fastx_fetch(const char *path, const char *name, long beg, long end, char *out, size_t cap) {
    pgh::FastxIndex fx; std::string err, s;
    if (!fx.load(path, err)) return -3;
    if (!fx.fetch(name, beg, end, s)) return -2;
    if (s.size() < cap) { memcpy(out, s.data(), s.size()); out[s.size()] = 0; }
    return (long)s.size();
}

extern "C" long pgt_slow5_get(const char *path, const char *read_id, double *dig_off_range, int16_t *raw, size_t cap) {
    pgh::Slow5File f; std::string err;
    if (!f.open(path, err)) return -1;
    pgh::Slow5Rec r;
    if (!f.get(read_id, r, err)) return -1;
    dig_off_range[0] = r.digitisation; dig_off_range[1] = r.offset; dig_off_range[2] = r.range;
    for (size_t i = 0; i < r.raw.size() && i < cap; i++) raw[i] = r.raw[i];
    return (long)r.raw.size();
}

extern "C" long pgt_slow5_count(const char *path) {
    pgh::Slow5File f; std::string err;
    if (!f.open(path, err)) return -1;
    return (long)f.n_reads();
}

extern "C" int pgt_parse_paf(char *line, int32_t *cols6, char *rid, char *tid, char *ss, size_t cap) {
    pgh::PafRec p;
    int rc = pgh::parse_paf_line(line, strlen(line), p);
    if (rc != 0) return rc;
    cols6[0] = p.qlen; cols6[1] = p.query_start; cols6[2] = p.query_end; cols6[3] = p.tlen; cols6[4] = p.target_start; cols6[5] = p.target_end;
    snprintf(rid, cap, "%s", p.rid.c_str()); snprintf(tid, cap, "%s", p.tid.c_str());
    if (p.ss_len < cap) { memcpy(ss, p.ss, p.ss_len); ss[p.ss_len] = 0; }
    return 0;
}

extern "C" long pgt_sam_first(const char *path, char *qname, char *seq, size_t cap, long long *stride_ns_ts, uint8_t *is_one, size_t mcap) {
    pgh::SamBamReader r; std::string err;
    if (!r.open(path, err)) return -1;
    pgh::MoveRec m;
    if (r.next(m, err) != 1) return -1;
    snprintf(qname, cap, "%s", m.qname.c_str()); snprintf(seq, cap, "%s", m.seq.c_str());
    stride_ns_ts[0] = m.stride; stride_ns_ts[1] = m.has_ns ? (long long)m.ns : -1; stride_ns_ts[2] = m.has_ts ? (long long)m.ts : -1;
    const long n_moves = (long)m.is_one.size();
    for (size_t i = 0; i < m.is_one.size() && i < mcap; i++) is_one[i] = m.is_one[i];
    pgh::MoveRec m2;
    if (r.next(m2, err) != 0) return -2;
    return n_moves;
}

#include "pg_model.h"
#include <algorithm>
#include <cstdio>
extern "C" long long pgt_fixed8(double x, int *bad) { bool b = false; const long long v = pg_fixed8(x, b); *bad = b; return v; }
extern "C" void pgt_model_texts(const long long *units, size_t n, char *med, char *sd, size_t cap) {
    std::vector<long long> v(units, units + n);
    PgSlotModel m{};
    m.n = n; m.origin = n ? v[0] : 0;
    for (size_t i = 0; i < n; i++) {
        const long long d = v[i] - m.origin; const unsigned long long ad = (unsigned long long)(d < 0 ? -d : d);
        const unsigned long long h = ad >> PG_MODEL_LIMB_BITS, l = ad & ((1u << PG_MODEL_LIMB_BITS) - 1);
        m.s1 += d; m.s2_hh += h * h; m.s2_hl += h * l; m.s2_ll += l * l;
    }
    std::sort(v.begin(), v.end());
    if (n) { m.mid_lo = v[(n - 1) / 2]; m.mid_hi = v[n / 2]; }
    med[0] = sd[0] = 0;
    if (!n) return;
    snprintf(med, cap, "%.14Lg", pg_model_median(m));
    if (n < 2) snprintf(sd, cap, "nan");
    else {
        const unsigned __int128 s2 = ((unsigned __int128)m.s2_hh << 40) + ((unsigned __int128)m.s2_hl << 21) + m.s2_ll;
        const __int128 s1 = m.s1;
        pg_model_sstdev_text(n, (unsigned __int128)n * s2 - (unsigned __int128)(s1 * s1), sd, cap);
    }
}
extern "C" void pgt_sstdev_text(unsigned long long n, unsigned long long num_hi, unsigned long long num_lo, char *exact, char *plain, size_t cap) {
    const unsigned __int128 num = ((unsigned __int128)num_hi << 64) | num_lo;
    pg_model_sstdev_text(n, num, exact, cap);
    snprintf(plain, cap, "%.14Lg", sqrtl((long double)num / ((long double)n * (long double)(n - 1))) / 1e8L);
}

#include "pg_hostmem.h"
#include <fstream>
#include <sstream>
extern "C" int pgt_samplevec_hugepage(size_t n, long *anon_huge_kb) {
    SampleVec v;
    v.resize(n);
    for (size_t i = 0; i < n; i += 512) v[i] = 1.0;
    const uintptr_t p = reinterpret_cast<uintptr_t>(v.data());
    std::ifstream f("/proc/self/smaps");
    if (!f) return -1;
    std::string line; bool inside = false; int hg = 0; long ahp = 0;
    while (std::getline(f, line)) {
        unsigned long a = 0, b = 0;
        if (sscanf(line.c_str(), "%lx-%lx ", &a, &b) == 2) { inside = p >= a && p < b; continue; }
        if (!inside) continue;
        if (line.rfind("AnonHugePages:", 0) == 0) ahp = atol(line.c_str() + 14);
        if (line.rfind("VmFlags:", 0) == 0) { std::istringstream is(line.substr(8)); std::string t; while (is >> t) if (t == "hg") hg = 1; }
    }
    if (anon_huge_kb) *anon_huge_kb = ahp;
    return hg;
}

static void put_err(const std::string &e, char *errbuf, size_t cap) { if (errbuf && cap) { const size_t n = e.size() < cap - 1 ? e.size() : cap - 1; memcpy(errbuf, e.data(), n); errbuf[n] = 0; } }
extern "C" long pgt_slow5_scan(const char *path, char *errbuf, size_t cap) {
    pgh::Slow5File f; std::string err;
    if (!f.open(path, err)) { put_err(err, errbuf, cap); return -1; }
    long n = 0;
    for (const std::string &id : f.ids_in_file_order()) {
        pgh::Slow5Rec r;
        if (!f.get(id, r, err)) { put_err(err, errbuf, cap); return -1; }
        ++n;
    }
    return n;
}
extern "C" long pgt_sambam_scan(const char *path, char *errbuf, size_t cap) {
    pgh::SamBamReader rd; std::string err;
    if (!rd.open(path, err)) { put_err(err, errbuf, cap); return -1; }
    long n = 0;
    for (;;) {
        pgh::MoveRec m;
        const int rc = rd.next(m, err);
        if (rc < 0) { put_err(err, errbuf, cap); return -1; }
        if (rc == 0) break;
        ++n;
    }
    return n;
}

#include "pg_job_rule.h"
extern "C" int pgt_job_stats_rule(uint32_t rank, const uint64_t *shard_ops, const uint64_t *shard_reads, uint32_t n_slots, uint64_t sample_limit,
                                  int have_batch, uint64_t full_slots_prev, const char *mode) {
    return (int)pg_job_stats_place(rank, shard_ops, shard_reads, n_slots, sample_limit, have_batch != 0, full_slots_prev, mode && *mode ? mode : nullptr);
}

#include "pg_stats_plan.h"
extern "C" void pgt_stats_plan(uint32_t ctx_flags, int32_t scaling, uint32_t front_tiles, uint32_t n_reads, int front_two_streams, int32_t *out6) {
    const PgStatsPlan p = pg_stats_plan(ctx_flags, scaling, front_tiles, n_reads, front_two_streams != 0);
    out6[0] = p.place; out6[1] = p.behind_cut; out6[2] = p.one_stream_batch; out6[3] = p.records_in_init; out6[4] = p.flags_in_init; out6[5] = p.rare_with_scan;
}
extern "C" int pgt_stats_fork_waits(int batch_is_host, int user_stream, int batch_resident, int prev_one_stream) {
    return pg_stats_fork_waits(batch_is_host != 0, user_stream != 0, batch_resident != 0, prev_one_stream != 0) ? 1 : 0;
}

#include "pg_pamean.h"
extern "C" int pgt_pa_shift(double offset) { return pg_pa_shift(offset); }
extern "C" int pgt_pa_certify(uint64_t n, int64_t s1, uint64_t sa, double offset, double scale, double *mean) {
    return pg_pa_certify(n, s1, sa, pg_pa_shift(offset), offset, scale, mean);
}
extern "C" double pgt_pa_sequential_mean(const int16_t *raw, uint64_t n, double dig, double off, double range) {
    return pg_pa_sequential_mean(raw, n, dig, off, range);
}
extern "C" long pgt_slow5_walk(const char *path, char *ids, size_t cap, uint64_t *lens, size_t max, char *errbuf, size_t ecap) {
    pgh::Slow5File f; std::string err, all;
    if (!f.open_walk(path, err)) { put_err(err, errbuf, ecap); return -1; }
    for (size_t i = 0; i < f.n_records(); i++) {
        std::string id; pgh::Slow5Rec r;
        if (!f.record(i, id, r, err)) { put_err(err, errbuf, ecap); return -1; }
        all += id; all += '\n';
        if (i < max) lens[i] = r.raw.size();
    }
    if (all.size() < cap) { memcpy(ids, all.data(), all.size()); ids[all.size()] = 0; }
    return (long)f.n_records();
}

#include "pg_svb.h"
extern "C" int pgt_svb_check(uint64_t len, uint32_t count) { return pg_svb_check(len, count); }
extern "C" uint64_t pgt_svb_nctrl(uint32_t count) { return pg_svb_nctrl(count); }
extern "C" void pgt_svb_levels(uint32_t *out3) { out3[0] = PG_SVB_LANE_VALUES; out3[1] = PG_SVB_WAVE_VALUES; out3[2] = PG_SVB_PIECE_VALUES; }
extern "C" long pgt_slow5_svb_walk(const char *path, uint32_t *counts, uint64_t *lens, size_t max, uint8_t *blocks, size_t cap, char *errbuf, size_t ecap) {
    pgh::Slow5File f; std::string err;
    if (!f.open_walk(path, err)) { put_err(err, errbuf, ecap); return -1; }
    if (!f.has_svb_views()) { put_err("no svb-zd signals", errbuf, ecap); return -1; }
    size_t at = 0;
    for (size_t i = 0; i < f.n_records(); i++) {
        std::string id; pgh::Slow5File::SvbView v; std::vector<unsigned char> inflated;
        if (!f.record_svb(i, id, v, inflated, err)) { put_err("record " + std::to_string(i) + ": " + err, errbuf, ecap); return -1; }
        if (i < max) { counts[i] = v.count; lens[i] = v.len; }
        if (at + v.len <= cap) memcpy(blocks + at, v.block, v.len);
        at += v.len;
    }
    return (long)f.n_records();
}

#include "pg_dumphost.h"
#include "host/pg_dumpdir.h"
extern "C" long pgt_dump_model_host(const char *const *dirs, size_t n_dirs, int which, const char *limit, int keep_first, int n_threads,
                                    char *out, size_t cap, char *errbuf, size_t ecap) {
    pgh::DumpSet ds; std::string err, text;
    if (!pgh::list_dump_dirs(std::vector<std::string>(dirs, dirs + n_dirs), n_threads, ds, err)) { put_err(err, errbuf, ecap); return -1; }
    std::vector<uint8_t> bytes; std::vector<uint64_t> off;
    if (!pgh::read_dump_files(ds, 0, ds.names.size(), n_threads, bytes, off, err)) { put_err(err, errbuf, ecap); return -1; }
    for (size_t i = 0; i < ds.names.size(); i++) {
        const char *b = reinterpret_cast<const char *>(bytes.data()) + off[i];
        const size_t len = off[i + 1] - off[i];
        text += ds.names[i]; text += '\t';
        if (which == 0) {
            PgDumpHostStats hs;
            pg_dump_host_stats(b, len, keep_first != 0, hs);
            text += hs.median; text += '\t'; text += pg_dump_sd_capped(hs.sstdev.c_str(), limit) ? std::string(limit) : hs.sstdev;
        } else {
            PgDumpHostDwell hd;
            pg_dump_host_dwell(b, len, hd);
            char t[64]; t[0] = 0;
            if (hd.n) snprintf(t, sizeof t, "%.14Lg", ((long double)hd.mid_lo + (long double)hd.mid_hi) / 2.0L);
            text += t;
        }
        text += '\n';
    }
    if (out && cap) { const size_t n = text.size() < cap - 1 ? text.size() : cap - 1; memcpy(out, text.data(), n); out[n] = 0; }
    return (long)text.size();
}

#include "pg_kfreq_codes.h"
extern "C" int pgt_kf_code_of_byte(int byte) { return (int)pg_kf_code_of_byte((uint32_t)byte & 0xff); }
extern "C" int pgt_kf_letter(int code) { return (int)pg_kf_letter((uint32_t)code & 15); }
extern "C" int pgt_kf_complement(int code) { return (int)pg_kf_complement((uint32_t)code & 15); }

#include "pg_kfreq_fasta.h"
#include <map>
namespace {
constexpr uint64_t kFaTile = (uint64_t)kFaSpan * kFaTileSpans;
struct FaHostSink {
    uint32_t k; std::map<uint32_t, uint64_t> *hist; std::map<std::string, uint64_t> *odd_map;
    void dense(uint32_t code) { (*hist)[code]++; }
    void odd(uint64_t lo, uint32_t hi) {
        std::string key(k, '\0');
        for (uint32_t i = 0; i < k; i++) { const uint32_t sh = k - 1 - i; key[i] = (char)(sh < 8 ? lo >> (8 * sh) : hi >> (8 * (sh - 8))); }
        (*odd_map)[key]++;
    }
};
struct FaHostLoad {
    const uint8_t *p; uint64_t base, n;
    void operator()(uint32_t ch, uint32_t (&ws)[4]) const {
        for (int i = 0; i < 4; i++) ws[i] = 0;
        for (uint32_t b = 0; b < 16; b++) { const uint64_t o = base + 16 * ch + b; if (o < n) ws[b >> 2] |= (uint32_t)p[o] << (8 * (b & 3)); }
    }
};
struct FaHostState { uint32_t kind; PgFaSum rec; };
uint32_t fa_host_span(const uint8_t *p, uint64_t base, uint64_t n, PgFaSpan &sp) {
    uint32_t w[kFaSpan / 4];
    FaHostLoad load{p, base, n};
    for (uint32_t ch = 0; ch < kFaSpan / 16; ch++) { uint32_t ws[4]; load(ch, ws); for (int i = 0; i < 4; i++) w[4 * ch + i] = ws[i]; }
    pg_fa_span_summary(w, (uint32_t)std::min<uint64_t>(kFaSpan, n - base), sp);
    return w[0] & 0xff;
}
bool fa_host_unit(const uint8_t *p, uint64_t n, uint32_t k, FaHostState &st, FaHostSink &sink) {
    const uint64_t n_tiles = (n + kFaTile - 1) / kFaTile;
    std::vector<uint64_t> tile_ls(n_tiles, 0);
    std::vector<PgFaSum> tile_fa(n_tiles), tile_pb(n_tiles);
    for (uint64_t t = 0; t < n_tiles; t++) {
        const uint64_t tile0 = t * kFaTile, tile_end = std::min<uint64_t>(n, tile0 + kFaTile);
        uint64_t ls = 0, fa_end = tile_end;
        PgFaSum rest = pg_fa_empty();
        for (uint64_t base = tile0; base < tile_end; base += kFaSpan) {
            PgFaSpan sp;
            const uint32_t first_byte = fa_host_span(p, base, n, sp);
            rest = pg_fa_compose(rest, ls ? pg_fa_resolve(pg_fa_kind_at(p, ls, base, PG_FA_SEQ), first_byte, sp.fa, sp.pb) : sp.pb);
            if (sp.has_nl) {
                if (!ls) { fa_end = base; while (p[fa_end] != '\n') fa_end++; }
                ls = base + sp.last_nl + 1;
            }
        }
        PgFaSum f = pg_fa_empty();
        for (uint64_t q = fa_end - tile0 > kFaTail ? fa_end - kFaTail : tile0; q < fa_end; q++) pg_fa_append(f, p[q]);
        tile_ls[t] = ls; tile_fa[t] = f; tile_pb[t] = rest;
    }
    bool bad = false;
    uint64_t line_in = 0;
    PgFaSum rec_in = st.rec;
    for (uint64_t t = 0; t < n_tiles; t++) {
        const uint64_t tile0 = t * kFaTile, tile_end = std::min<uint64_t>(n, tile0 + kFaTile);
        uint64_t ls = line_in;
        PgFaSum rec = rec_in;
        for (uint64_t base = tile0; base < tile_end; base += kFaSpan) {
            PgFaSpan sp;
            const uint32_t first_byte = fa_host_span(p, base, n, sp);
            const uint32_t kind = pg_fa_kind_at(p, ls, base, st.kind);
            FaHostLoad load{p, base, n};
            bad |= pg_fa_walk(load, (uint32_t)std::min<uint64_t>(kFaSpan, n - base), k, kind, rec, sink);
            rec = pg_fa_compose(rec, pg_fa_resolve(kind, first_byte, sp.fa, sp.pb));
            if (sp.has_nl) ls = base + sp.last_nl + 1;
        }
        rec_in = pg_fa_compose(rec_in, pg_fa_resolve(pg_fa_kind_at(p, line_in, tile0, st.kind), p[tile0], tile_fa[t], tile_pb[t]));
        line_in = std::max(line_in, tile_ls[t]);
    }
    st.kind = pg_fa_kind_at(p, line_in, n, st.kind);
    st.rec = rec_in;
    return bad;
}
}
extern "C" long pgt_kf_fasta(const uint8_t *data, uint64_t n, const uint64_t *cuts, size_t n_cuts, uint32_t k, uint64_t unit,
// ... 389 lines not shown
```

### poregen_amd/csrc/pg_internal.h

```cpp
#pragma once
#include <hip/hip_runtime.h>
#include <stdint.h>

struct PgDevBatch {
    uint32_t n_reads;
    uint64_t n_ops;
    const int16_t *sig;
    const uint64_t *sig_off;
    const double *dig, *off, *range;
    const int32_t *qstart, *tstart, *tend;
    const uint8_t *seq;
    const uint64_t *seq_off;
    const uint32_t *op_n;
    const uint8_t *op_t;
    const uint64_t *op_off;
};

struct PgWalkParams {
    uint32_t k, sig_move_offset, print_margin, max_dur, min_dur;
    int32_t pick_margin, allow_rna, short_ok;
    int32_t no_generic;
    uint32_t n_codes;
    const int32_t *table_t, *table_u;
    int32_t aff_ok[2]; uint32_t aff_lo[2], aff_hi[2]; int32_t aff_delta[2];
// ... 114 lines not shown
hipError_t pg_launch_len_partials(hipStream_t st, uint64_t n_kept_cap, const uint64_t *n_kept_ptr, const PgKeptRec *rec, uint64_t *part, const PgRareArgs *rare);
uint32_t pg_gather_chunks(uint64_t n_kept_cap, uint32_t *sub_per_chunk);
#define PG_GATHER_FORMS 5
int pg_gather_form(int lanes);
hipError_t pg_launch_gather_chunks(hipStream_t st, const PgDevBatch &B, uint64_t n_kept_cap, const uint64_t *n_kept_ptr, const PgKeptRec *rec, const uint64_t *part,
                                   uint64_t *samp_off, uint64_t *total_out, int scaling, double pa_min, double pa_max, double *samples, const double *gcal, int lanes,
                                   const int32_t *stat_flags );
hipError_t pg_launch_text_lens(hipStream_t st, const double *samples, const uint64_t *samp_off, uint64_t n_events, uint32_t *tlen, uint32_t *flag);
hipError_t pg_launch_text_write(hipStream_t st, const double *samples, const uint64_t *samp_off, uint64_t n_events, const uint64_t *toff, char *text,
                                const uint64_t *ev_off, uint32_t n_slots, uint64_t *slot_toff);
hipError_t pg_launch_unpack_recs(hipStream_t st, const PgKeptRec *rec, uint64_t n, uint32_t *ev_len, uint32_t *ev_read);

#define PG_STATS_BINS 2048
#define PG_HUGE_BLOCKS 64
struct PgStatRec {
    uint64_t beg, end;
    int32_t c_lo, span, z0;
    int32_t mode;
    double offset, scale;
    double inv;
    uint32_t sym;
    uint32_t split;
};
enum { PG_STAT_RUN = 0, PG_STAT_SKIP = 1, PG_STAT_BAD = 2 };
#ifndef PG_LONG_MIN
#define PG_LONG_MIN 32768u
#endif
#ifndef PG_LONG_SLICE
#define PG_LONG_SLICE 16384u
#endif
#define PG_LONG_MAX_SLICES 1024u
#define PG_LONG_WORDS 1128u
#define PG_LONG_INVALID 0xFFFFFFFFu
struct PgLongState {
    uint2 *tab;
    uint32_t *hist;
    int32_t *cnt;
    int32_t *cnt_next;
    uint32_t cap;
};
static inline __host__ __device__ void pg_long_geometry(uint64_t L, uint32_t *slices, uint64_t *slen) {
    uint64_t sl = PG_LONG_SLICE;
    while ((L + sl - 1) / sl > PG_LONG_MAX_SLICES) sl *= 2;
    *slen = sl; *slices = (uint32_t)((L + sl - 1) / sl);
}
#define PG_STAT_REC_BYTES 64
#define PG_HUGE_SCRATCH_WORDS ((size_t)PG_HUGE_BLOCKS * (65536 + 64))

struct PgGathered {
    const uint64_t *all_counts;
    uint32_t world, rank;
    uint64_t *total, *freq;
};
struct PgFront { uint32_t tiles; uint32_t *word; };
enum { PG_PASS_WHOLE = 0, PG_PASS_FRONT = 1, PG_PASS_TAIL = 2 };
struct __attribute__((aligned(16))) PgKeptRec {
    uint64_t src;
    uint32_t len;
    uint32_t read;
};
struct PgKeptOut {
    PgKeptRec *rec;
    uint8_t *read_needed;
};
extern thread_local hipEvent_t pg_prof_start, pg_prof_stop;
hipError_t pg_launch_batch_init(hipStream_t st, uint32_t n_reads, uint8_t *read_needed, uint64_t *running, uint32_t n_slots,
                          int zero_running, int32_t *stat_flags,
                          const PgDevBatch &B, double pa_min, double pa_max, void *plan_buf, int32_t *stat_status,
                          const PgWalkParams &W, const PgWalkOut &O, int force_generic, const PgLongState &LS,
                          uint32_t *big_op = nullptr);
static inline uint32_t pg_tiles(uint64_t n_events, bool direct) {
    const uint64_t t = (n_events + PG_SORT_TILE - 1) / PG_SORT_TILE;
    return (uint32_t)(direct ? (t + 3) & ~3ull : t);
}
struct PgSlotModel; struct PgSlotDwell;
hipError_t pg_launch_slot_model(hipStream_t st, uint32_t n_slots, const int any_kind[4], const uint64_t *ev_off, const uint64_t *samp_off,
                                const uint32_t *ev_len, const double *samples, uint32_t drop_first, PgSlotModel *out, PgSlotDwell *dwell,
                                void *scratch );
hipError_t pg_launch_slot_model_units(hipStream_t st, uint32_t n_slots, const int any_kind[4], const uint64_t *ev_off, const uint64_t *samp_off,
                                      const uint32_t *ev_len, const int64_t *units, uint32_t drop_first, PgSlotModel *out, PgSlotDwell *dwell, void *scratch);
size_t pg_slot_model_scratch_bytes(uint32_t n_slots);
struct PgDtBatch {
    const uint8_t *p; uint64_t n;
    const uint64_t *file_off; uint32_t n_files;
    uint32_t n_tiles;
    uint2 *tile_pre;
    uint32_t *fflags;
    uint2 *fstart;
    uint64_t *val_base;
    uint64_t *ev_off;
    int64_t *units; uint64_t *samp_off; uint32_t *ev_len;
    uint64_t cap_values;
};
hipError_t pg_launch_dump_parse(hipStream_t st, const PgDtBatch &b);
static inline uint64_t pg_ev_tiles(uint64_t cap_values) { return (cap_values + 127) / 128 + 1; }
size_t pg_ev_carry_bytes(uint64_t cap_values);
hipError_t pg_launch_ev_stats_units(hipStream_t st, uint32_t n_files, const uint64_t *ev_off, const uint64_t *samp_off, const int64_t *units, uint64_t cap_events,
                                    uint64_t cap_values, int64_t *ev_mean, int64_t *ev_sd, uint32_t *fflags, void *carry);
hipError_t pg_launch_ev_stats(hipStream_t st, uint32_t n_files, const uint64_t *ev_off, const uint64_t *samp_off, const double *samples, uint64_t cap_events,
                              uint64_t cap_values, int64_t *ev_mean, int64_t *ev_sd, uint32_t *fflags, void *carry);
hipError_t pg_launch_ev_identity(hipStream_t st, uint64_t n, uint64_t *id_off, uint32_t *len1);
hipError_t pg_launch_walk(hipStream_t st, const PgDevBatch &B, const PgWalkParams &W, const PgWalkOut &O);
hipError_t pg_launch_events(hipStream_t st, const PgDevBatch &B, const PgWalkParams &W, const PgWalkOut &O, uint32_t n_slots, uint32_t *hist,
                            uint32_t part_hi_bits, uint32_t part_lo_bits, const PgFront &F = PgFront{}, int pass = PG_PASS_WHOLE);
hipError_t pg_launch_apply_oor(hipStream_t st, const PgDevBatch &B, const PgWalkOut &O);
hipError_t pg_launch_rank_direct_count(hipStream_t st, const uint32_t *ev_slot, uint64_t n, uint32_t n_slots, const PgSortBufs &S,
                                 uint64_t *acc_cnt, uint64_t *running, uint32_t limit, int32_t *tile_last,
                                 uint64_t *acc_copy ,
                                 uint64_t *plan_keep, uint64_t *plan_ev_off, uint64_t *plan_totals, uint32_t *plan_ticket, bool *plan_done,
                                 const uint32_t *btot , uint32_t *Bp ,
                                 uint64_t *zero64 ,
                                 const PgFront &F = PgFront{}, int pass = PG_PASS_WHOLE, uint32_t batch_id = 0,
                                 const uint32_t *tile_read = nullptr, uint32_t n_reads = 0);
hipError_t pg_launch_rank_direct_emit(hipStream_t st, const uint32_t *ev_slot, uint64_t n, uint32_t n_slots, const PgSortBufs &S,
                                const uint64_t *keep, const uint64_t *ev_off, const uint64_t *totals, const PgDevBatch &B,
                                const PgWalkParams &W, const PgWalkOut &O, const PgKeptOut &K);
hipError_t pg_launch_sort_events(hipStream_t st, const uint32_t *ev_slot, uint64_t n, uint32_t key_bits, const PgSortBufs &S, int *sorted_idx,
                                 uint64_t *scatter_launches);
hipError_t pg_launch_slot_bounds(hipStream_t st, const uint32_t *skey, const uint32_t *m_ptr, uint64_t n_upper,
                           uint32_t *slot_start, uint32_t *slot_end, uint32_t n_slots, uint64_t *acc_cnt, uint64_t *acc_copy);
hipError_t pg_launch_kept_meta(hipStream_t st, const uint32_t *skey, const uint32_t *sval, const uint32_t *m_ptr, uint64_t n_upper,
                         const uint32_t *slot_start, const uint64_t *keep, const uint64_t *ev_off,
                         const PgDevBatch &B, const PgWalkParams &W, const PgWalkOut &O, const PgKeptOut &K, uint32_t *dst_scratch);
hipError_t pg_launch_slot_plan(hipStream_t st, const uint64_t *acc_cnt, const uint64_t *base, uint64_t *running,
                         uint32_t limit, uint32_t n_slots, uint64_t *keep, uint64_t *ev_off, uint64_t *totals,
                         const uint32_t *hist, uint32_t n_tiles, uint32_t *keep32, uint64_t *scan_scratch,
                         const int32_t *tile_last ,
                         const PgGathered &G );
struct PgRareArgs {
    PgDevBatch B;
    const PgStatRec *plan;
    double *med, *mad, *gcal;
    int32_t *status, *err;
    int win;
    const uint32_t *wide_list;
    const int32_t *wide_count;
    uint32_t *scratch;
    uint8_t *oor;
    int range_only;
    uint32_t wide_blocks;
};
hipError_t pg_launch_scan_u32_u64(hipStream_t st, const uint32_t *in, uint32_t stride, uint64_t n_cap, const uint64_t *n_ptr, uint64_t *out, uint64_t *scratch,
                                  const PgRareArgs *rare, uint64_t *total_out);
hipError_t pg_launch_read_stats_rare(hipStream_t st, const PgRareArgs &A);
struct PgSettlePack { uint32_t errflag[6]; int32_t stat_err[6]; uint64_t n_kept, full_slots, n_samples; uint32_t cancel[2]; uint32_t front[2]; };
hipError_t pg_launch_settle_pack(hipStream_t st, const uint32_t *errflag, const int32_t *stat_err, const int32_t *long_cnt, const uint64_t *totals, const uint64_t *samp_off,
                                 uint64_t samp_off_entries, const uint32_t *cancel_flag, const uint32_t *front_word, PgSettlePack *out);
hipError_t pg_launch_stats_cancel_if_full(hipStream_t st, const uint64_t *all_counts, uint32_t rows_below, uint32_t n_slots, uint64_t limit, uint32_t *flag, void *plan_buf, uint32_t n_reads);
hipError_t pg_launch_read_plan(hipStream_t st, const PgDevBatch &B, const uint8_t *read_needed, double pa_min, double pa_max, void *plan_buf,
                         int32_t *flags, int32_t *stat_status, bool flags_are_reset, const PgLongState &LS);
hipError_t pg_launch_read_stats(hipStream_t st, const PgDevBatch &B, const void *plan_buf, double *med, double *mad, int32_t *status, int32_t *err, int win,
                                uint32_t *wide_list, int32_t *wide_count, uint8_t *oor, int range_only, double *gcal, const PgLongState &LS,
                                const unsigned long long *cut_word = nullptr, uint32_t batch_id = 0, uint32_t group_from = 0xffffffffu);
uint32_t pg_stats_group_from(uint32_t n_reads, uint64_t n_ops, uint32_t front_tiles);
struct PgSeg { const double *src; uint64_t dst_off, n; };
hipError_t pg_launch_merge_segments(hipStream_t st, const PgSeg *d_seg, uint32_t n_seg, double *dst, uint64_t n_total );
hipError_t pg_launch_gather(hipStream_t st, const PgDevBatch &B, uint64_t n_kept_cap, const uint64_t *n_kept_ptr, const PgKeptRec *rec,
                      const uint64_t *samp_off, int scaling, double pa_min,
                      double pa_max, const double *med, const double *mad, double *samples, const double *gcal);
```

### poregen_amd/csrc/pg_kernels.hip

```cpp
#include "pg_dev.h"
#include "pg_select.h"
#include <limits.h>
#include <type_traits>

#ifdef PG_PHASE_PROBE
#define PG_PROBE_WAVES 65536
__device__ unsigned long long g_pg_phase[3][PG_PROBE_WAVES][8];
extern "C" void pg_debug_phases(unsigned long long *out, int kernel, int reset) {
    (void)hipMemcpyFromSymbol(out, HIP_SYMBOL(g_pg_phase), sizeof(unsigned long long) * PG_PROBE_WAVES * 8, sizeof(unsigned long long) * PG_PROBE_WAVES * 8 * kernel);
    if (reset) { void *p = nullptr; (void)hipGetSymbolAddress(&p, HIP_SYMBOL(g_pg_phase)); (void)hipMemset(p, 0, sizeof(unsigned long long) * 3 * PG_PROBE_WAVES * 8); }
}
#define PG_PROBE_BEGIN(k) unsigned long long pg_acc_[8] = {0, 0, 0, 0, 0, 0, 0, 0}; unsigned long long pg_t_ = __builtin_readcyclecounter(); const unsigned long long pg_t0_ = pg_t_
#define PG_MARK(k, i) do { __builtin_amdgcn_s_waitcnt(0); const unsigned long long n_ = __builtin_readcyclecounter(); pg_acc_[i] += n_ - pg_t_; pg_t_ = n_; } while (0)
#define PG_PROBE_END(k, wave) do { if (lane_id() == 0 && (wave) < PG_PROBE_WAVES) { pg_acc_[7] = __builtin_readcyclecounter() - pg_t0_; for (int i_ = 0; i_ < 8; ++i_) g_pg_phase[k][wave][i_] = pg_acc_[i_]; } } while (0)
#define PG_PROBE_PARAM , unsigned long long &pg_t_, unsigned long long (&pg_acc_)[8]
#define PG_PROBE_ARG , pg_t_, pg_acc_
#else
#define PG_PROBE_BEGIN(k) do {} while (0)
#define PG_MARK(k, i) do {} while (0)
#define PG_PROBE_END(k, wave) do {} while (0)
#define PG_PROBE_PARAM
#define PG_PROBE_ARG
#endif

// ... 957 lines not shown
                                                  uint64_t *__restrict__ acc_cnt, uint32_t n_slots, uint32_t n_digits, const uint64_t *running,
                                                  uint32_t limit, int32_t *__restrict__ tile_last, PgScanPlan plan, uint32_t *front_word, uint32_t batch_id,
                                                  const uint32_t *tile_read, uint32_t n_reads) {
    if (TAIL && front_word[0]) return;
    const uint32_t d = blockIdx.x * PG_SCAN_WAVES + (threadIdx.x >> 6);
    const int lane = lane_id();
    if (d < n_digits) {
        const uint32_t c_begin = TAIL ? F : 0u, c_end = TAIL ? n_tiles : F;
        uint32_t run = TAIL ? totals[d] : 0u;
        const bool want_last = d < n_slots;
        const uint64_t base0 = want_last ? running[d] : 0;
        const uint32_t room = base0 >= limit ? 0u : limit - (uint32_t)base0;
        int candA = -1, candB = -1;
        uint32_t *__restrict__ row = hist + (uint64_t)d * n_tiles;
        for (uint32_t c0 = c_begin; c0 < c_end; c0 += 8 * WAVE) {
            uint32_t v[8];
#pragma unroll
            for (int u = 0; u < 8; ++u) { const uint32_t i = c0 + u * WAVE + lane; v[u] = i < c_end ? row[i] : 0u; }
#pragma unroll
            for (int u = 0; u < 8; ++u) {
                const uint32_t i = c0 + u * WAVE + lane;
                const uint32_t inc = wave_incl_scan_u32(v[u]);
                const uint32_t excl = run + inc - v[u];
                if (i < c_end) {
                    row[i] = excl;
                    if (excl < room) candA = (int)i;
                    if (v[u] > 0) candB = (int)i;
                }
                run += (uint32_t)__builtin_amdgcn_readlane((int)inc, WAVE - 1);
            }
        }
        int last = -1;
        if (want_last) {
            last = run >= room ? candA : candB;
            for (int o = 32; o >= 1; o >>= 1) { const int t = __shfl_xor(last, o, WAVE); last = t > last ? t : last; }
            if (TAIL && last < 0) last = __hip_atomic_load(tile_last + d, __ATOMIC_RELAXED, __HIP_MEMORY_SCOPE_AGENT);
            if (room == 0 || run == 0) last = -1;
        }
        if (lane == 0) {
            totals[d] = run;
            if (d < n_slots) {
                __hip_atomic_store(reinterpret_cast<unsigned long long *>(acc_cnt + d), (unsigned long long)run, __ATOMIC_RELAXED, __HIP_MEMORY_SCOPE_AGENT);
                __hip_atomic_store(tile_last + d, last, __ATOMIC_RELAXED, __HIP_MEMORY_SCOPE_AGENT);
            }
        }
    }
    rank_scan_cut(plan, acc_cnt, tile_last, running, limit, n_slots, gridDim.x - 1u, TAIL ? nullptr : front_word, batch_id, tile_read, F, n_reads);
}

__global__ __launch_bounds__(256) void k_sort_dbase(const uint32_t *__restrict__ totals, uint32_t ndig, uint32_t *__restrict__ dbase,
                                                    uint32_t *__restrict__ count_out) {
    __shared__ uint32_t wsum[4];
    const uint32_t tid = threadIdx.x;
    const uint32_t per = ndig >= 256 ? ndig / 256 : 1;
    uint32_t v[4] = {0, 0, 0, 0}, s = 0;
    for (uint32_t i = 0; i < per; ++i) { const uint32_t d = tid * per + i; v[i] = d < ndig ? totals[d] : 0u; s += v[i]; }
    const uint32_t inc = wave_incl_scan_u32(s);
    if (lane_id() == WAVE - 1) wsum[tid >> 6] = inc;
    __syncthreads();
    uint32_t off = inc - s;
    for (uint32_t w = 0; w < (tid >> 6); ++w) off += wsum[w];
    for (uint32_t i = 0; i < per; ++i) { const uint32_t d = tid * per + i; if (d < ndig) dbase[d] = off; off += v[i]; }
    if (tid == 255) *count_out = off;
}

__global__ __launch_bounds__(256) void k_sort_scatter(const uint32_t *__restrict__ keys, const uint32_t *__restrict__ vals,
                                                      uint32_t n_scalar, const uint32_t *__restrict__ n_ptr, uint32_t shift,
                                                      int nbits, uint32_t n_tiles, const uint32_t *__restrict__ hist,
                                                      const uint32_t *__restrict__ dbase, const uint32_t *__restrict__ wcnt,
                                                      uint32_t *__restrict__ keys_out, uint32_t *__restrict__ vals_out) {
    __shared__ uint32_t wbase[4][PG_RANK_MAX_DIGITS];
    __shared__ uint32_t gb[PG_RANK_MAX_DIGITS], ls[PG_RANK_MAX_DIGITS + 1];
    __shared__ uint32_t lkey[PG_SORT_TILE], lval[PG_SORT_TILE];
    __shared__ uint32_t wsum[4];
    const uint32_t tid = threadIdx.x, tile = blockIdx.x, w = tid >> 6;
    const int lane = lane_id();
    const uint32_t ndig = 1u << nbits;
    const uint32_t n = n_ptr ? *n_ptr : n_scalar;
    const uint32_t mask = ndig - 1u;
    const uint64_t base = (uint64_t)tile * PG_SORT_TILE + (uint64_t)w * PG_SORT_ROWS * WAVE;
    uint32_t kv[PG_SORT_ROWS], vv[PG_SORT_ROWS];
#pragma unroll
    for (int row = 0; row < PG_SORT_ROWS; ++row) {
        const uint64_t idx = base + (uint64_t)row * WAVE + lane;
        kv[row] = idx < n ? keys[idx] : PG_INVALID_SLOT;
        vv[row] = idx < n ? (vals ? vals[idx] : (uint32_t)idx) : 0u;
    }
    const uint32_t per = ndig >= 256 ? ndig / 256 : 1;
    uint32_t cnt_d[4] = {0, 0, 0, 0}, sum = 0;
    for (uint32_t i = 0; i < per; ++i) {
        const uint32_t d = tid * per + i;
        if (d < ndig) {
            uint32_t b = dbase[d] + hist[(uint64_t)d * n_tiles + tile];
            gb[d] = b;
            for (uint32_t ww = 0; ww < 4; ++ww) { wbase[ww][d] = b; b += wcnt[((uint64_t)tile * 4 + ww) * ndig + d]; }
            cnt_d[i] = b - gb[d]; sum += cnt_d[i];
        }
    }
    const uint32_t inc = wave_incl_scan_u32(sum);
    if (lane == WAVE - 1) wsum[w] = inc;
    __syncthreads();
    {
        uint32_t off = inc - sum;
        for (uint32_t ww = 0; ww < w; ++ww) off += wsum[ww];
        for (uint32_t i = 0; i < per; ++i) { const uint32_t d = tid * per + i; if (d < ndig) { ls[d] = off; off += cnt_d[i]; } }
        if (tid == 255) ls[ndig] = off;
    }
    __syncthreads();
    volatile uint32_t *mybase = wbase[w];
#pragma unroll
    for (int row = 0; row < PG_SORT_ROWS; ++row) {
        const uint32_t key = kv[row];
        const bool valid = key != PG_INVALID_SLOT;
        const uint32_t d = (key >> shift) & mask;
        const uint64_t peers = match_digit(d, valid, nbits);
        uint32_t b = 0;
        if (valid) b = mybase[d];
        __builtin_amdgcn_wave_barrier();
        if (valid && lane == __ffsll((long long)peers) - 1) mybase[d] = b + (uint32_t)__popcll(peers);
        __builtin_amdgcn_wave_barrier();
        if (valid) {
            const uint32_t dest = b + (uint32_t)__popcll(peers & lanemask_lt());
            const uint32_t j = ls[d] + (dest - gb[d]);
            lkey[j] = key; lval[j] = vv[row];
        }
    }
    __syncthreads();
    const uint32_t total = ls[ndig];
    for (uint32_t j = tid; j < total; j += 256) {
        const uint32_t key = lkey[j], d = (key >> shift) & mask;
        const uint32_t dest = gb[d] + (j - ls[d]);
        keys_out[dest] = key;
        vals_out[dest] = lval[j];
    }
}

__device__ __forceinline__ void write_kept(const PgDevBatch &B, const PgWalkParams &W, const PgWalkOut &O, const PgKeptOut &K,
                                           uint64_t e, uint64_t g) {
    const uint32_t rd = owner_of(B, O, g);
    const KeptRead kr = kept_read(O, rd);
    uint32_t start, len;
    if (!kept_window(B, W, O, kr, g, start, len)) { report_error(O, rd, PGR_ERR_RANGE); start = 0; len = 0; }
    const uint64_t L = kr.L;
    const uint64_t we64 = (uint64_t)start + len + W.print_margin;
    uint32_t we = (uint32_t)(we64 > L ? L : we64), ws = start - W.print_margin;
    if (W.print_margin > start || we <= ws) { report_error(O, rd, PGR_ERR_WINDOW); ws = we = 0; }
    K.rec[e] = PgKeptRec{kr.sig0 + ws, we - ws, rd};
    if (K.read_needed) K.read_needed[rd] = 1;
}

#define PG_EMIT_WAVES 16
#define PG_EMIT_GRID 512
#define PG_EMIT_ROWS (PG_SORT_TILE / (PG_EMIT_WAVES * WAVE))
__global__ __launch_bounds__(PG_EMIT_WAVES * WAVE) void k_rank_emit(const uint32_t *__restrict__ keys, uint32_t n, int nbits, uint32_t n_slots, uint32_t n_tiles,
                                                   const uint32_t *__restrict__ hist,
                                                   const uint64_t *__restrict__ keep, const uint64_t *__restrict__ ev_off,
                                                   const uint64_t *__restrict__ totals, PgDevBatch B, PgWalkParams W, PgWalkOut O,
                                                   PgKeptOut K) {
    __shared__ uint32_t wbase[PG_EMIT_WAVES][PG_RANK_MAX_DIGITS];
    __shared__ uint32_t s_keep[PG_RANK_MAX_DIGITS], s_off[PG_RANK_MAX_DIGITS];
    static_assert(PG_RANK_MAX_DIGITS <= PG_EMIT_WAVES * WAVE, "one digit per thread");
    const uint32_t tid = threadIdx.x, w = tid >> 6;
    const int lane = lane_id();
    const uint32_t ndig = 1u << nbits;
    PG_PROBE_BEGIN(2);
    const int64_t last_tile = (int64_t)totals[3];
    for (uint32_t tile = blockIdx.x; tile < n_tiles && (int64_t)tile <= last_tile; tile += gridDim.x) {
    if (tile != blockIdx.x) __syncthreads();
    PG_MARK(2, 0);
    const uint32_t tile_first = O.tile_read[tile];
    const uint64_t base = (uint64_t)tile * PG_SORT_TILE + (uint64_t)w * PG_EMIT_ROWS * WAVE;
    uint32_t kv[PG_EMIT_ROWS], kp[PG_EMIT_ROWS], eo[PG_EMIT_ROWS];
#pragma unroll
    for (int row = 0; row < PG_EMIT_ROWS; ++row) {
        const uint64_t idx = base + (uint64_t)row * WAVE + lane;
        kv[row] = idx < n ? keys[idx] : PG_INVALID_SLOT;
    }
    uint32_t hcol = 0; uint64_t kd = 0, od = 0;
    if (tid < n_slots) { hcol = hist[(uint64_t)tid * n_tiles + tile]; kd = keep[tid]; od = ev_off[tid]; }
    PG_MARK(2, 1);
    int any = 0;
    if (tid < ndig) {
        if (tid < n_slots && (uint64_t)hcol < kd) any = 1;
        s_keep[tid] = (uint32_t)kd;
        s_off[tid] = (uint32_t)od;
        for (uint32_t ww = 0; ww < PG_EMIT_WAVES; ++ww) wbase[ww][tid] = 0;
    }
    uint32_t rd[PG_EMIT_ROWS]; KeptRead kr[PG_EMIT_ROWS]; bool have[PG_EMIT_ROWS];
#pragma unroll
    for (int row = 0; row < PG_EMIT_ROWS; ++row) {
        const uint32_t rel = kv[row] >> PG_SLOT_BITS;
        have[row] = kv[row] != PG_INVALID_SLOT && rel != PG_REL_UNKNOWN;
        rd[row] = tile_first + rel;
        if (have[row]) kr[row] = kept_read(O, rd[row]);
    }
    if (!__syncthreads_or(any)) break;
    volatile uint32_t *mybase = wbase[w];
#pragma unroll
    for (int row = 0; row < PG_EMIT_ROWS; ++row) {
        const bool valid = kv[row] != PG_INVALID_SLOT;
        kp[row] = valid ? s_keep[kv[row] & (ndig - 1u)] : 0u;
        eo[row] = valid ? s_off[kv[row] & (ndig - 1u)] : 0u;
    }
#pragma unroll
    for (int row = 0; row < PG_EMIT_ROWS; ++row) if (kv[row] != PG_INVALID_SLOT) atomicAdd(&wbase[w][kv[row] & (ndig - 1u)], 1u);
    __syncthreads();
    if (tid < ndig) {
        uint32_t cw[PG_EMIT_WAVES];
#pragma unroll
        for (int ww = 0; ww < PG_EMIT_WAVES; ++ww) cw[ww] = wbase[ww][tid];
        uint32_t b = hcol;
#pragma unroll
        for (int ww = 0; ww < PG_EMIT_WAVES; ++ww) { wbase[ww][tid] = b; b += cw[ww]; }
    }
    __syncthreads();
    PG_MARK(2, 2);
    uint32_t dst[PG_EMIT_ROWS];
#pragma unroll
    for (int row = 0; row < PG_EMIT_ROWS; ++row) {
        const uint32_t key = kv[row];
        const bool valid = key != PG_INVALID_SLOT;
        const uint32_t d = key & (ndig - 1u);
        const uint64_t peers = match_digit(d, valid, nbits);
        uint32_t b = 0;
        if (valid) b = mybase[d];
        __builtin_amdgcn_wave_barrier();
        if (valid && lane == __ffsll((long long)peers) - 1) mybase[d] = b + (uint32_t)__popcll(peers);
        __builtin_amdgcn_wave_barrier();
        const uint32_t rank = b + (uint32_t)__popcll(peers & lanemask_lt());
        dst[row] = (valid && rank < kp[row]) ? eo[row] + rank : 0xFFFFFFFFu;
    }
    PG_MARK(2, 3);
#pragma unroll
    for (int row = 0; row < PG_EMIT_ROWS; ++row)
        if (dst[row] != 0xFFFFFFFFu && !have[row]) { rd[row] = owner_of(B, O, base + (uint64_t)row * WAVE + lane); kr[row] = kept_read(O, rd[row]); }
    uint32_t ws[PG_EMIT_ROWS], wl[PG_EMIT_ROWS]; bool okr[PG_EMIT_ROWS];
#pragma unroll
    for (int row = 0; row < PG_EMIT_ROWS; ++row) {
        ws[row] = 0; wl[row] = 0; okr[row] = true;
        if (dst[row] != 0xFFFFFFFFu) okr[row] = kept_window(B, W, O, kr[row], base + (uint64_t)row * WAVE + lane, ws[row], wl[row]);
    }
    PG_MARK(2, 4);
#pragma unroll
    for (int row = 0; row < PG_EMIT_ROWS; ++row) {
        if (dst[row] == 0xFFFFFFFFu) continue;
        if (!okr[row]) { report_error(O, rd[row], PGR_ERR_RANGE); ws[row] = 0; wl[row] = 0; }
        const uint32_t Lr = kr[row].L;
        uint32_t start = ws[row] - W.print_margin;
        const uint64_t we64 = (uint64_t)ws[row] + wl[row] + W.print_margin;
        uint32_t we = (uint32_t)(we64 > Lr ? Lr : we64);
        if (W.print_margin > ws[row] || we <= start) { report_error(O, rd[row], PGR_ERR_WINDOW); start = we = 0; }
        K.rec[dst[row]] = PgKeptRec{kr[row].sig0 + start, we - start, rd[row]};
        if (K.read_needed) K.read_needed[rd[row]] = 1;
    }
    PG_MARK(2, 5);
    if (tile == blockIdx.x) PG_PROBE_END(2, tile * PG_EMIT_WAVES + w);
    }
}


__global__ __launch_bounds__(256) void k_slot_bounds(const uint32_t *__restrict__ skey, const uint32_t *__restrict__ m_ptr,
                                                     uint32_t *__restrict__ slot_start, uint32_t *__restrict__ slot_end) {
    const uint64_t pos = (uint64_t)blockIdx.x * 256 + threadIdx.x;
    const uint32_t M = *m_ptr;
    if (pos >= M) return;
    const uint32_t s = skey[pos];
    if (pos == 0 || skey[pos - 1] != s) slot_start[s] = (uint32_t)pos;
    if (pos == M - 1 || skey[pos + 1] != s) slot_end[s] = (uint32_t)pos + 1;
}

__global__ __launch_bounds__(256) void k_slot_counts(const uint32_t *__restrict__ slot_start, const uint32_t *__restrict__ slot_end,
                                                     uint32_t n_slots, uint64_t *__restrict__ acc_cnt, uint64_t *__restrict__ acc_copy) {
    const uint32_t s = blockIdx.x * 256 + threadIdx.x;
    if (s < n_slots) {
        acc_cnt[s] = (uint64_t)(slot_end[s] - slot_start[s]);
        if (acc_copy) acc_copy[s] = acc_cnt[s];
    }
}

__device__ __forceinline__ uint64_t slot_base(const PgGathered &G, const uint64_t *base, uint32_t s, uint32_t n_slots, uint32_t limit) {
    if (!G.all_counts) return base[s];
    uint64_t b = 0, t = 0;
    for (uint32_t g = 0; g < G.world; ++g) {
        if (g == G.rank) b = t;
        t += G.all_counts[(uint64_t)g * n_slots + s];
    }
    G.total[s] = t;
    G.freq[s] = t < limit ? t : limit;
    return b;
}

__global__ __launch_bounds__(1024) void k_slot_plan(const uint64_t *__restrict__ acc_cnt, const uint64_t *base, uint64_t *running,
                                                    uint32_t limit, uint32_t n_slots, uint64_t *__restrict__ keep,
                                                    uint64_t *__restrict__ ev_off, uint64_t *__restrict__ totals,
                                                    const uint32_t *__restrict__ hist, uint32_t n_tiles, const int32_t *__restrict__ tile_last,
                                                    PgGathered G) {
    __shared__ uint64_t wsum[16];
    __shared__ uint64_t wfull[16];
    (void)hist; (void)n_tiles;
    const uint32_t tid = threadIdx.x, w = tid >> 6;
    const int lane = lane_id();
    uint64_t carry = 0, full = 0;
    int base_below_running = 0;
    for (uint32_t c = 0; c < n_slots; c += 1024) {
        const uint32_t s = c + tid;
        uint64_t kp = 0, isfull = 0;
        if (s < n_slots) {
            const uint64_t cnt = acc_cnt[s], b = slot_base(G, base, s, n_slots, limit);
            if (tile_last && running && b < running[s]) base_below_running = 1;
            const uint64_t room = b >= limit ? 0 : (uint64_t)limit - b;
            kp = cnt < room ? cnt : room;
            isfull = (limit > 0 && b + cnt >= limit) ? 1 : 0;
            if (running) running[s] = b + cnt;
            keep[s] = kp;
        }
        const uint64_t inc = wave_incl_scan_u64(kp);
        const uint64_t fsum = wave_incl_scan_u64(isfull);
        if (lane == WAVE - 1) { wsum[w] = inc; wfull[w] = fsum; }
        __syncthreads();
        uint64_t off = 0, tot = 0, ftot = 0;
        for (uint32_t ww = 0; ww < 16; ++ww) { if (ww < w) off += wsum[ww]; tot += wsum[ww]; ftot += wfull[ww]; }
        if (s < n_slots) ev_off[s] = carry + off + inc - kp;
        carry += tot; full += ftot;
        __syncthreads();
    }
    __syncthreads();
    int last = -1;
    if (tile_last) {
        __shared__ int wlast[16];
        for (uint32_t s2 = tid; s2 < n_slots; s2 += 1024) { const int t = tile_last[s2]; last = t > last ? t : last; }
        for (int o = 32; o >= 1; o >>= 1) { const int t = __shfl_xor(last, o, WAVE); last = t > last ? t : last; }
        if (lane == 0) wlast[w] = last;
        __syncthreads();
        if (tid == 0) for (int ww = 0; ww < 16; ++ww) last = wlast[ww] > last ? wlast[ww] : last;
    }
    base_below_running = __syncthreads_or(base_below_running);
    if (tid == 0) {
        ev_off[n_slots] = carry; totals[0] = carry; totals[1] = full;
        totals[3] = tile_last ? (base_below_running ? ~0ull >> 1 : (uint64_t)(int64_t)last) : (hist ? ~0ull : ~0ull >> 1);
    }
}

__global__ __launch_bounds__(256) void k_slot_keep(const uint64_t *__restrict__ acc_cnt, const uint64_t *base, uint64_t *running, uint32_t limit,
                                                   uint32_t n_slots, uint64_t *__restrict__ keep, uint32_t *__restrict__ keep32,
                                                   uint64_t *__restrict__ totals, PgGathered G) {
    __shared__ uint32_t wfull[4];
    const uint32_t s = blockIdx.x * 256 + threadIdx.x;
    bool isfull = false;
    if (s < n_slots) {
        const uint64_t cnt = acc_cnt[s], b = slot_base(G, base, s, n_slots, limit);
        const uint64_t room = b >= limit ? 0 : (uint64_t)limit - b;
        const uint64_t kp = cnt < room ? cnt : room;
        isfull = limit > 0 && b + cnt >= limit;
        if (running) running[s] = b + cnt;
        keep[s] = kp; keep32[s] = (uint32_t)kp;
    }
    const uint32_t nfull = (uint32_t)__popcll(__ballot(isfull));
    if (lane_id() == 0) wfull[threadIdx.x >> 6] = nfull;
    __syncthreads();
    if (threadIdx.x == 0) atomicAdd(reinterpret_cast<unsigned long long *>(&totals[1]), (unsigned long long)(wfull[0] + wfull[1] + wfull[2] + wfull[3]));
}
#define SCAN_CHUNK 4096
__global__ __launch_bounds__(256) void k_slot_cut(const uint64_t *__restrict__ acc_cnt, const uint64_t *base, uint64_t *running, uint32_t limit, uint32_t n_slots,
                                                  uint64_t *__restrict__ keep, uint32_t *__restrict__ keep32, uint64_t *__restrict__ ev_off, uint64_t *__restrict__ totals,
                                                  uint64_t *__restrict__ state, uint32_t n_scan, PgGathered G) {
    __shared__ uint64_t wsum[4];
    __shared__ uint64_t sh_prefix;
    __shared__ uint32_t sh_block, wfull[4];
    if (threadIdx.x == 0) sh_block = (uint32_t)atomicAdd(reinterpret_cast<unsigned long long *>(state), 1ull);
    __syncthreads();
    const uint32_t b = sh_block;
    const uint64_t s0 = (uint64_t)b * SCAN_CHUNK + (uint64_t)threadIdx.x * 16;
    uint32_t v[16]; uint64_t s = 0; uint32_t nfull = 0;
#pragma unroll
    for (int i = 0; i < 16; ++i) {
        const uint64_t sl = s0 + i;
        v[i] = 0;
        if (sl < n_slots) {
            const uint64_t cnt = acc_cnt[sl], bb = slot_base(G, base, (uint32_t)sl, n_slots, limit);
            const uint64_t room = bb >= limit ? 0 : (uint64_t)limit - bb;
            const uint64_t kp = cnt < room ? cnt : room;
            nfull += (limit > 0 && bb + cnt >= limit) ? 1u : 0u;
            if (running) running[sl] = bb + cnt;
            keep[sl] = kp; keep32[sl] = (uint32_t)kp; v[i] = (uint32_t)kp;
        }
        s += v[i];
    }
    const uint64_t inc = wave_incl_scan_u64(s);
    for (int o = 32; o >= 1; o >>= 1) nfull += __shfl_xor(nfull, o, WAVE);
    if (lane_id() == WAVE - 1) { wsum[threadIdx.x >> 6] = inc; wfull[threadIdx.x >> 6] = nfull; }
    __syncthreads();
    const uint64_t block_sum = wsum[0] + wsum[1] + wsum[2] + wsum[3];
    uint64_t *st = state + 2;
    if (threadIdx.x < WAVE) {
        const int lane = threadIdx.x;
        if (lane == 0) __hip_atomic_store(st + b, (block_sum << 2) | (b == 0 ? 2ull : 1ull), __ATOMIC_RELAXED, __HIP_MEMORY_SCOPE_AGENT);
        uint64_t excl = 0;
        int64_t hi = (int64_t)b - 1;
        while (hi >= 0) {
            const int64_t j = hi - lane;
            uint64_t wv = 0;
            if (j >= 0) do { wv = __hip_atomic_load(st + j, __ATOMIC_RELAXED, __HIP_MEMORY_SCOPE_AGENT); } while ((wv & 3ull) == 0);
            const uint64_t pm = __ballot(j >= 0 && (wv & 3ull) == 2ull);
            const int stop = pm ? __ffsll((long long)pm) - 1 : WAVE;
            uint64_t part = (j >= 0 && lane <= stop) ? (wv >> 2) : 0ull;
            part = wave_incl_scan_u64(part);
            excl += (uint64_t)__shfl(part, WAVE - 1, WAVE);
            if (pm) break;
            hi -= WAVE;
        }
// ... 591 lines not shown
                                                int32_t *__restrict__ status, int32_t *__restrict__ err) {
    if (lane == 0) stats_no_result_lane(r, code, med, mad, gcal, status, err);
}

template <int BINS>
__device__ __forceinline__ void stats_one_read(uint32_t *hist, const PgDevBatch &B, uint32_t r, const PgStatRec *__restrict__ rec,
                                               double *__restrict__ med, double *__restrict__ mad, double *__restrict__ gcal, int32_t *__restrict__ status,
                                               int32_t *__restrict__ err, int win, uint8_t *__restrict__ oor, int range_only) {
    using C = StatsCfg<BINS>;
    const int lane = lane_id();
    const PgStatRec m = rec[r];
    if (m.mode != PG_STAT_RUN) return;
    if (m.span > BINS) { stats_no_result(lane, r, PGR_ERR_WIDE, med, mad, gcal, status, err); return; }
    const uint64_t beg = m.beg, end = m.end;
    stats_zero<BINS>(hist, lane);
    const int c_lo = m.c_lo;
    const int16_t *__restrict__ sig = B.sig;
    auto bin8 = [&](const int4 &q) {
        if constexpr (C::GLOBAL) {
            const int w[4] = {q.x, q.y, q.z, q.w};
#pragma unroll
            for (int i = 0; i < 4; ++i) { stats_bin1<BINS>(hist, (int)(short)(w[i] & 0xffff), c_lo, lane); stats_bin1<BINS>(hist, w[i] >> 16, c_lo, lane); }
        } else {
            const uint32_t c16 = (uint32_t)c_lo & 0xffffu, cap = (uint32_t)BINS + (lane & 31u);
            stats_bin8<BINS>(hist, q, c16 | (c16 << 16), cap | (cap << 16));
        }
    };
    const uint64_t va = (beg + 7) >> 3, vb = end >> 3;
    if (va < vb) {
        for (uint64_t s2 = beg + lane; s2 < (va << 3); s2 += WAVE) stats_bin1<BINS>(hist, (int)sig[s2], c_lo, lane);
        for (uint64_t s2 = (vb << 3) + lane; s2 < end; s2 += WAVE) stats_bin1<BINS>(hist, (int)sig[s2], c_lo, lane);
        const int4 *__restrict__ vec = reinterpret_cast<const int4 *>(sig);
        for (uint64_t v = va + lane; v < vb; v += 8 * WAVE) {
            int4 q[8];
#pragma unroll
            for (int u = 0; u < 8; ++u) if (v + u * WAVE < vb) q[u] = vec[v + u * WAVE];
#pragma unroll
            for (int u = 0; u < 8; ++u) if (v + u * WAVE < vb) bin8(q[u]);
        }
    } else {
        for (uint64_t s2 = beg + lane; s2 < end; s2 += WAVE) stats_bin1<BINS>(hist, (int)sig[s2], c_lo, lane);
    }
#ifdef PG_PHASE_PROBE
    unsigned long long pg_t_ = 0, pg_acc_[8];
#endif
    if (lane == 0 && gcal && !pg_div_domain_ok(m.offset, m.scale)) atomicOr(err + 3, 1);
    stats_finish<BINS>(hist, lane, r, m, med, mad, gcal, win, oor, range_only PG_PROBE_ARG);
}

#ifndef PG_STATS_SETPRIO
#define PG_STATS_SETPRIO 2
#endif
#ifndef PG_STATS_NT_LOADS
#define PG_STATS_NT_LOADS 1
#endif
#ifndef PG_STATS_CACHED_FRACTION
#define PG_STATS_CACHED_FRACTION 8
#endif
#ifndef PG_STATS_WPB
#define PG_STATS_WPB 1
#endif
#ifndef PG_STATS_WAVES_PER_EU
#define PG_STATS_WAVES_PER_EU 6
#endif
#ifndef PG_STATS_GROUP
#define PG_STATS_GROUP 8
#endif
static_assert(PG_STATS_GROUP >= 1 && PG_STATS_GROUP <= 64, "a lane per read of the group");
__device__ __forceinline__ void stats_read_body(uint32_t *hist, const PgDevBatch &B, const uint32_t r, const uint32_t slice, const PgStatRec &m, const int lane,
                                                double *__restrict__ med, double *__restrict__ mad, int32_t *__restrict__ status, int32_t *__restrict__ err,
                                                int win, uint8_t *__restrict__ oor, int range_only, uint32_t *__restrict__ wide_list,
                                                int32_t *__restrict__ wide_count, uint32_t keep_cached, double *__restrict__ gcal, const PgLongState &LS) {
    PG_PROBE_BEGIN(0);
    if (m.span > 1024) { if (lane == 0) stats_list_wide(r, m.span, B.n_reads, wide_list, wide_count); return; }
    const int16_t *__restrict__ sig = B.sig;
    const int c_lo = m.c_lo;
    const uint32_t c16 = (uint32_t)c_lo & 0xffffu, c2 = c16 | (c16 << 16);
    const uint32_t cap = 1024u + (lane & 31u), cap2 = cap | (cap << 16);
    uint64_t beg = m.beg, end = m.end;
    uint32_t n_slices = 1;
    if (m.split) {
        uint64_t slen;
        pg_long_geometry(m.end - m.beg, &n_slices, &slen);
        beg = m.beg + (uint64_t)slice * slen;
        end = beg + slen < m.end ? beg + slen : m.end;
    }
    const uint64_t va = (beg + 7) >> 3, vb = end >> 3;
    if (va < vb) {
        const uint64_t n_vec = vb - va;
        for (uint64_t p = 0; p < n_vec; p += 8 * WAVE) {
            const int4 *__restrict__ vp = reinterpret_cast<const int4 *>(sig) + (va + p);
            const uint32_t last = n_vec - p > 8 * WAVE ? 8 * WAVE - 1 : (uint32_t)(n_vec - p) - 1;
            int4 q[8];
#if PG_STATS_NT_LOADS
            if (r >= keep_cached) {
                typedef int pg_i4 __attribute__((ext_vector_type(4)));
#pragma unroll
                for (int u = 0; u < 8; ++u) {
                    const pg_i4 x = __builtin_nontemporal_load(reinterpret_cast<const pg_i4 *>(vp) + min((uint32_t)(u * WAVE + lane), last));
                    q[u] = make_int4(x.x, x.y, x.z, x.w);
                }
            } else
#endif
            {
#pragma unroll
                for (int u = 0; u < 8; ++u) q[u] = vp[min((uint32_t)(u * WAVE + lane), last)];
            }
            if (p == 0) stats_zero<1024>(hist, lane);
            PG_MARK(0, 1);
#pragma unroll
            for (int u = 0; u < 8; ++u) if ((uint32_t)(u * WAVE + lane) <= last) stats_bin8<1024>(hist, q[u], c2, cap2);
            PG_MARK(0, 2);
        }
        if ((va << 3) != beg || (vb << 3) != end) {
            for (uint64_t s2 = beg + lane; s2 < (va << 3); s2 += WAVE) stats_bin1<1024>(hist, (int)sig[s2], c_lo, lane);
            for (uint64_t s2 = (vb << 3) + lane; s2 < end; s2 += WAVE) stats_bin1<1024>(hist, (int)sig[s2], c_lo, lane);
        }
    } else {
        stats_zero<1024>(hist, lane);
        for (uint64_t s2 = beg + lane; s2 < end; s2 += WAVE) stats_bin1<1024>(hist, (int)sig[s2], c_lo, lane);
    }
    if (m.split) {
        uint32_t *__restrict__ gh = LS.hist + (size_t)(m.split - 1u) * PG_LONG_WORDS;
        __builtin_amdgcn_fence(__ATOMIC_RELEASE, "wavefront");
        __builtin_amdgcn_wave_barrier();
        constexpr uint32_t REAL = 1024u + WAVE;
        static_assert(REAL % WAVE == 0, "rows of the padded histogram");
        uint32_t got[REAL / WAVE];
#pragma unroll
        for (uint32_t j = 0; j < REAL / WAVE; ++j) {
            const uint32_t v = hist[j * WAVE + lane];
            got[j] = 0;
            if (v) got[j] = __hip_atomic_fetch_add(gh + j * WAVE + lane, v, __ATOMIC_RELAXED, __HIP_MEMORY_SCOPE_AGENT);
        }
        uint32_t seen = 0;
#pragma unroll
        for (uint32_t j = 0; j < REAL / WAVE; ++j) seen += got[j];
        asm volatile("; long-read merge: per-bin sums returned" : "+v"(seen) : : "memory");
        __builtin_amdgcn_s_waitcnt(0);
        uint32_t t = 0;
        if (lane == 0) t = __hip_atomic_fetch_add(gh + PG_LONG_WORDS - 1u, 1u, __ATOMIC_RELAXED, __HIP_MEMORY_SCOPE_AGENT);
        t = (uint32_t)__builtin_amdgcn_readfirstlane((int)t);
        if (t + 1u != n_slices) return;
        for (uint32_t i = lane; i < REAL; i += WAVE) hist[i] = __hip_atomic_exchange(gh + i, 0u, __ATOMIC_RELAXED, __HIP_MEMORY_SCOPE_AGENT);
        if (lane == 0) __hip_atomic_store(gh + PG_LONG_WORDS - 1u, 0u, __ATOMIC_RELAXED, __HIP_MEMORY_SCOPE_AGENT);
    }
    if (PG_STATS_SETPRIO) __builtin_amdgcn_s_setprio(PG_STATS_SETPRIO);
    if (lane == 0 && gcal && !pg_div_domain_ok(m.offset, m.scale)) atomicOr(err + 3, 1);
    stats_finish<1024>(hist, lane, r, m, med, mad, gcal, win, oor, range_only PG_PROBE_ARG);
    PG_MARK(0, 4);
    PG_PROBE_END(0, r);
}

__global__ __launch_bounds__(64 * PG_STATS_WPB) __attribute__((amdgpu_waves_per_eu(PG_STATS_WAVES_PER_EU, PG_STATS_WAVES_PER_EU))) void k_read_stats(PgDevBatch B, const PgStatRec *__restrict__ rec, double *__restrict__ med,
                                                   double *__restrict__ mad, int32_t *__restrict__ status, int32_t *__restrict__ err,
                                                   int win, uint8_t *__restrict__ oor, int range_only, uint32_t *__restrict__ wide_list,
                                                   int32_t *__restrict__ wide_count, uint32_t keep_cached, double *__restrict__ gcal, PgLongState LS,
                                                   const unsigned long long *__restrict__ cut_word, uint32_t batch_id, uint32_t r1, uint32_t n_groups) {
    __shared__ __attribute__((aligned(16))) uint32_t hist_all[PG_STATS_WPB][StatsGeom<1024>::LDS_WORDS];
    static_assert(StatsGeom<1024>::LDS_WORDS + 1 <= PG_LONG_WORDS, "a long read's histogram in global memory");
    static_assert(PG_STATS_WPB == 1, "the group workgroups and the helpers of long reads are found from blockIdx.x: [0, r1) reads, [r1, r1 + n_groups) groups, then helper blockIdx.x - r1 - n_groups");
    uint32_t *hist = hist_all[0];
    const uint32_t b = blockIdx.x;
    const int lane = lane_id();
    uint32_t r = b;
    uint32_t slice = 0, base = 0;
    unsigned long long todo = 0;
    const bool grouped = b >= r1 && b - r1 < n_groups;
    unsigned long long cw = 0;
    if (grouped) {
        base = r1 + (b - r1) * (uint32_t)PG_STATS_GROUP;
        const uint32_t rl = base + (uint32_t)lane;
        const bool mine = lane < PG_STATS_GROUP && rl < B.n_reads;
        int32_t mode = PG_STAT_SKIP; uint32_t split = 0;
        if (mine) { mode = rec[rl].mode; split = rec[rl].split; }
        if (cut_word) cw = *cut_word;
        bool compute = false;
        if (mine) {
            if (mode != PG_STAT_RUN) stats_no_result_lane(rl, mode == PG_STAT_BAD ? PGR_ERR_SCALE : 0, med, mad, gcal, status, err);
            else if (split == 0 && (uint32_t)(cw >> 32) == batch_id && cut_word && rl >= (uint32_t)cw) stats_no_result_lane(rl, 0, med, mad, gcal, status, err);
            else compute = true;
        }
        todo = __ballot(compute);
        if (todo == 0) return;
    } else if (b >= r1) {
        const uint32_t h = b - r1 - n_groups;
        const uint32_t reserved = LS.tab ? (uint32_t)LS.cnt[0] : 0u;
        if (h >= LS.cap || h >= reserved) return;
        const uint2 e = LS.tab[h];
        if (e.x == PG_LONG_INVALID) return;
        r = (uint32_t)__builtin_amdgcn_readfirstlane((int)e.x); slice = (uint32_t)__builtin_amdgcn_readfirstlane((int)e.y);
    }
    for (;;) {
        if (grouped) {
            const int i = __builtin_ctzll(todo);
            todo &= todo - 1;
            r = (uint32_t)__builtin_amdgcn_readfirstlane((int)(base + (uint32_t)i));
        }
        const PgStatRec m = rec[r];
        if (!grouped) {
            if (cut_word) cw = *cut_word;
            if (m.mode != PG_STAT_RUN) { if (slice == 0) stats_no_result(lane, r, m.mode == PG_STAT_BAD ? PGR_ERR_SCALE : 0, med, mad, gcal, status, err); return; }
            if (cut_word && m.split == 0 && (uint32_t)(cw >> 32) == batch_id && r >= (uint32_t)cw) { stats_no_result(lane, r, 0, med, mad, gcal, status, err); return; }
        }
        stats_read_body(hist, B, r, slice, m, lane, med, mad, status, err, win, oor, range_only, wide_list, wide_count, keep_cached, gcal, LS);
        if (!grouped || todo == 0) return;
        __builtin_amdgcn_fence(__ATOMIC_RELEASE, "wavefront");
        __builtin_amdgcn_wave_barrier();
        if (PG_STATS_SETPRIO) __builtin_amdgcn_s_setprio(0);
    }
}

static_assert(PG_RARE_LDS_WORDS == StatsGeom<PG_STATS_BINS>::LDS_WORDS, "k_scan_chained's rare histogram");
__device__ __forceinline__ void rare_worker(uint32_t worker, uint32_t n_wide, uint32_t *hist, const PgRareArgs &A) {
    if (worker < n_wide) {
        const uint32_t n_list = (uint32_t)A.wide_count[0];
        for (uint32_t it = worker; it < n_list; it += n_wide) {
            stats_one_read<PG_STATS_BINS>(hist, A.B, A.wide_list[it], A.plan, A.med, A.mad, A.gcal, A.status, A.err, A.win, A.oor, A.range_only);
            __builtin_amdgcn_fence(__ATOMIC_RELEASE, "wavefront");
            __builtin_amdgcn_wave_barrier();
        }
    } else if (worker < n_wide + PG_HUGE_BLOCKS) {
        const uint32_t hb = worker - n_wide, n_list = (uint32_t)A.wide_count[1];
        uint32_t *gh = A.scratch + (size_t)hb * PG_HUGE_WORDS;
        for (uint32_t it = hb; it < n_list; it += PG_HUGE_BLOCKS) {
            stats_one_read<PG_HUGE_BINS>(gh, A.B, A.wide_list[A.B.n_reads - 1 - it], A.plan, A.med, A.mad, A.gcal, A.status, A.err, A.win, A.oor, A.range_only);
            __builtin_amdgcn_fence(__ATOMIC_RELEASE, "agent"); __builtin_amdgcn_s_waitcnt(0);
            __builtin_amdgcn_wave_barrier();
        }
    }
}
__global__ __launch_bounds__(64) void k_read_stats_rare(PgRareArgs A) {
    __shared__ __attribute__((aligned(16))) uint32_t hist[StatsGeom<PG_STATS_BINS>::LDS_WORDS];
    rare_worker(blockIdx.x, gridDim.x - PG_HUGE_BLOCKS, hist, A);
}

template <int G>
__device__ __forceinline__ void gather_events(const PgDevBatch &B, uint64_t n_kept, uint64_t total, const PgKeptRec *__restrict__ rec,
                                              const uint64_t *__restrict__ samp_off, int scaling, double pa_min, double pa_max,
                                              const double *__restrict__ med, const double *__restrict__ mad, const double *__restrict__ gcal, double *__restrict__ samples) {
    const int lane = lane_id();
    const int g0 = lane & ~(G - 1);
    const uint32_t sub = (uint32_t)lane & (uint32_t)(G - 1);
    const uint64_t stride = (uint64_t)gridDim.x * (256 / G);
    auto pair64 = [&](uint32_t v, int k) {
        return (uint64_t)(uint32_t)__shfl((int)v, g0 + k, WAVE) | ((uint64_t)(uint32_t)__shfl((int)v, g0 + k + 1, WAVE) << 32);
    };
    for (uint64_t e = (uint64_t)blockIdx.x * (256 / G) + (threadIdx.x / G); e < n_kept; e += stride) {
        const uint32_t *p1 = sub < 4 ? reinterpret_cast<const uint32_t *>(rec + e) + sub : reinterpret_cast<const uint32_t *>(samp_off + e) + (sub - 4);
        const uint32_t f = sub < 6 ? *p1 : 0u;
        const uint32_t len = (uint32_t)__shfl((int)f, g0 + 2, WAVE), rd = (uint32_t)__shfl((int)f, g0 + 3, WAVE);
        const uint64_t src = pair64(f, 0), dst = pair64(f, 4);
        gather_one<G>(B, sub, g0, rd, len, src, dst, total, scaling, pa_min, pa_max, med, mad, gcal, samples);
    }
}

__global__ __launch_bounds__(256) void k_gather(PgDevBatch B, const uint64_t *__restrict__ n_kept_ptr, const PgKeptRec *__restrict__ rec,
                                                const uint64_t *__restrict__ samp_off, int scaling, double pa_min, double pa_max,
                                                const double *__restrict__ med, const double *__restrict__ mad,
                                                double *__restrict__ samples, const double *__restrict__ gcal) {
    const uint64_t n_kept = n_kept_ptr[0], n_samples = n_kept_ptr[2];
    if (n_kept == 0) return;
    const uint64_t total = B.sig_off[B.n_reads];
    if (n_samples <= PG_GATHER8_MEAN * n_kept) gather_events<8>(B, n_kept, total, rec, samp_off, scaling, pa_min, pa_max, med, mad, gcal, samples);
    else gather_events<16>(B, n_kept, total, rec, samp_off, scaling, pa_min, pa_max, med, mad, gcal, samples);
}

__global__ __launch_bounds__(256) void k_batch_init(uint32_t n_reads, uint8_t *__restrict__ read_needed,
                                                    uint64_t *__restrict__ running, uint32_t n_slots, int zero_running,
                                                    int32_t *__restrict__ stat_flags, PgDevBatch B, double pa_min, double pa_max,
                                                    PgStatRec *__restrict__ plan_rec, int32_t *__restrict__ stat_status,
                                                    PgWalkParams W, PgWalkOut O, int force_generic, int op_t_aligned, PgLongState LS, uint32_t *__restrict__ big_op) {
    const uint32_t i = blockIdx.x * 256 + threadIdx.x;
    if (i < n_reads) read_head_one(B, W, O, i, force_generic);
    if (plan_rec && i < n_reads) read_plan_one(B, i, nullptr, pa_min, pa_max, plan_rec, stat_status, LS);
    if (i == 0 && LS.cnt_next) { LS.cnt_next[0] = 0; LS.cnt_next[1] = 0; }
    if (i == 0) {
        O.layout_err[0] = (n_reads ? B.op_off[n_reads] : B.n_ops) != B.n_ops;
        O.gen_count[(O.batch_id + 1u) & 1u] = 0;
    }
    if (i == 0 && stat_flags) { stat_flags[0] = INT_MAX; stat_flags[1] = 0; stat_flags[2] = 0; stat_flags[3] = 0; }
    if (i <= n_reads) read_needed[i] = 0;
    if (zero_running && i < n_slots) running[i] = 0;
    const uint64_t a = (uint64_t)i * 16u, ops_end = n_reads ? (B.op_off[n_reads] < B.n_ops ? B.op_off[n_reads] : B.n_ops) : 0;
    if (a < ops_end) {
        uint32_t w[4] = {0, 0, 0, 0};
        if (op_t_aligned && a + 16 <= ops_end) { const uint4 v = *reinterpret_cast<const uint4 *>(B.op_t + a); w[0] = v.x; w[1] = v.y; w[2] = v.z; w[3] = v.w; }
        else for (uint64_t x = a; x < a + 16 && x < ops_end; ++x) w[(x - a) >> 2] |= (uint32_t)B.op_t[x] << (8 * ((x - a) & 3));
        if (w[0] | w[1] | w[2] | w[3]) {
            uint32_t last = 0xffffffffu;
            for (uint32_t x = 0; x < 16; ++x)
                if ((w[x >> 2] >> (8 * (x & 3))) & 0xffu) {
                    const uint32_t r = owner_search(B, a + x);
                    if (r != last) { list_generic(O, r); last = r; }
                }
        }
        if (big_op) {
            uint32_t orv = 0;
            if (a + 16 <= ops_end) {
#pragma unroll
                for (int v = 0; v < 4; ++v) { const uint4 x = *reinterpret_cast<const uint4 *>(B.op_n + a + 4 * v); orv |= x.x | x.y | x.z | x.w; }
            } else for (uint64_t x = a; x < ops_end; ++x) orv |= B.op_n[x];
            if (orv >= PG_OP_N_LIMIT) *big_op = O.batch_id;
        }
    }
}

thread_local hipEvent_t pg_prof_start = nullptr, pg_prof_stop = nullptr;

hipError_t pg_launch_batch_init(hipStream_t st, uint32_t n_reads, uint8_t *read_needed, uint64_t *running, uint32_t n_slots,
                          int zero_running, int32_t *stat_flags, const PgDevBatch &B, double pa_min, double pa_max, void *plan_buf,
                          int32_t *stat_status, const PgWalkParams &W, const PgWalkOut &O, int force_generic, const PgLongState &LS, uint32_t *big_op) {
    uint64_t n = (n_reads + 1 > n_slots ? n_reads + 1 : n_slots);
    const uint64_t n_op_threads = (B.n_ops + 15) / 16;
    if (n_op_threads > n) n = n_op_threads;
    const int op_t_aligned = ((uintptr_t)B.op_t & 15) == 0;
    PG_LAUNCH(k_batch_init, dim3((uint32_t)((n + 255) / 256)), dim3(256), 0, st, n_reads, read_needed, running, n_slots, zero_running,
              stat_flags, B, pa_min, pa_max, reinterpret_cast<PgStatRec *>(plan_buf), stat_status, W, O, force_generic, op_t_aligned, LS, big_op);
    return hipSuccess;
}

hipError_t pg_launch_walk(hipStream_t st, const PgDevBatch &B, const PgWalkParams &W, const PgWalkOut &O) {
    if (B.n_reads == 0) return hipSuccess;
    if (W.pick_margin > 100) PG_LAUNCH(k_walk<true>, dim3(B.n_reads), dim3(64), 0, st, B, W, O);
    else PG_LAUNCH(k_walk<false>, dim3(B.n_reads), dim3(64), 0, st, B, W, O);
    return hipSuccess;
}

hipError_t pg_launch_events(hipStream_t st, const PgDevBatch &B, const PgWalkParams &W, const PgWalkOut &O, uint32_t n_slots, uint32_t *hist,
                            uint32_t part_hi_bits, uint32_t part_lo_bits, const PgFront &F, int pass) {
    if (B.n_reads == 0 || B.n_ops == 0) return hipSuccess;
    const uint32_t n_tiles = pg_tiles(B.n_ops, hist != nullptr);
    int nbits = 1; while ((1u << nbits) < n_slots) ++nbits;
    uint32_t blk0 = 0, blocks = (n_tiles + 3) / 4;
    const uint32_t *word = nullptr;
    if (pass != PG_PASS_WHOLE) {
        if (!hist || part_hi_bits || !F.word || F.tiles == 0 || (F.tiles & 3u) || F.tiles >= n_tiles) return hipErrorInvalidValue;
        if (pass == PG_PASS_FRONT) blocks = F.tiles / 4;
        else { blk0 = F.tiles / 4; blocks -= blk0; word = F.word; }
    }
    if (hist && part_hi_bits) PG_LAUNCH((k_events<2, false>), dim3(blocks), dim3(1024), 0, st, B, W, O, (int)part_hi_bits, n_tiles, hist, part_lo_bits, 0u, (const uint32_t *)nullptr);
    else if (hist && W.n_codes <= 1024) PG_LAUNCH((k_events<1, true>), dim3(blocks), dim3(1024), 0, st, B, W, O, nbits, n_tiles, hist, 0u, blk0, word);
    else if (hist) PG_LAUNCH((k_events<1, false>), dim3(blocks), dim3(1024), 0, st, B, W, O, nbits, n_tiles, hist, 0u, blk0, word);
    else PG_LAUNCH((k_events<0, false>), dim3(blocks), dim3(1024), 0, st, B, W, O, nbits, n_tiles, (uint32_t *)nullptr, 0u, 0u, (const uint32_t *)nullptr);
    return hipSuccess;
}

hipError_t pg_launch_apply_oor(hipStream_t st, const PgDevBatch &B, const PgWalkOut &O) {
    if (B.n_reads == 0 || !O.oor) return hipSuccess;
    PG_LAUNCH(k_apply_oor, dim3((B.n_reads + 255) / 256), dim3(256), 0, st, B.n_reads, O);
    return hipSuccess;
}

static uint32_t tiles_for(uint64_t n) { return pg_tiles(n, false); }

hipError_t pg_launch_rank_direct_count(hipStream_t st, const uint32_t *ev_slot, uint64_t n, uint32_t n_slots, const PgSortBufs &S,
                                 uint64_t *acc_cnt, uint64_t *running, uint32_t limit, int32_t *tile_last, uint64_t *acc_copy,
                                 uint64_t *plan_keep, uint64_t *plan_ev_off, uint64_t *plan_totals, uint32_t *plan_ticket, bool *plan_done,
                                 const uint32_t *btot, uint32_t *Bp, uint64_t *zero64, const PgFront &F, int pass, uint32_t batch_id,
                                 const uint32_t *tile_read, uint32_t n_reads) {
    int nbits = 1; while ((1u << nbits) < n_slots) ++nbits;
    const uint32_t n_tiles = pg_tiles(n, true);
    *plan_done = false;
// ... 85 lines not shown
        return hipSuccess;
    }
    PG_LAUNCH(k_slot_plan, dim3(1), dim3(1024), 0, st, acc_cnt, base, running, limit, n_slots, keep, ev_off, totals, hist, n_tiles, tile_last, G);
    if (hist && n_tiles && !tile_last) PG_LAUNCH(k_tile_max, dim3((n_slots + 63) / 64), dim3(64), 0, st, hist, n_tiles, (const uint64_t *)keep, n_slots, totals);
    return hipSuccess;
}

hipError_t pg_launch_kept_meta(hipStream_t st, const uint32_t *skey, const uint32_t *sval, const uint32_t *m_ptr, uint64_t n_upper,
                         const uint32_t *slot_start, const uint64_t *keep, const uint64_t *ev_off, const PgDevBatch &B,
                         const PgWalkParams &W, const PgWalkOut &O, const PgKeptOut &K, uint32_t *dst_scratch) {
    if (!n_upper) return hipSuccess;
    PG_LAUNCH(k_kept_pos, dim3((uint32_t)((n_upper + 255) / 256)), dim3(256), 0, st, skey, sval, m_ptr, slot_start, keep, ev_off, dst_scratch);
    PG_LAUNCH(k_kept_fill, dim3((uint32_t)((B.n_ops + 255) / 256)), dim3(256), 0, st, (const uint32_t *)O.ev_slot, (const uint32_t *)dst_scratch, B.n_ops, B, W, O, K);
    return hipSuccess;
}

hipError_t pg_launch_scan_u32_u64(hipStream_t st, const uint32_t *in, uint32_t stride, uint64_t n_cap, const uint64_t *n_ptr, uint64_t *out, uint64_t *scratch,
                                  const PgRareArgs *rare, uint64_t *total_out) {
    const uint32_t nb = (uint32_t)((n_cap + SCAN_CHUNK - 1) / SCAN_CHUNK), nbl = nb ? nb : 1;
    if (nbl <= 64) {
        if (rare) {
            const uint32_t want = rare->wide_blocks < 64 ? 64u : (rare->wide_blocks > 2048 ? 2048u : rare->wide_blocks);
            const uint32_t extra = (want + PG_HUGE_BLOCKS + 3) / 4;
            PG_LAUNCH(k_scan_chained<true>, dim3(nbl + extra), dim3(256), 0, st, in, stride, n_cap, n_ptr, out, scratch, nbl, *rare, total_out);
        } else PG_LAUNCH(k_scan_chained<false>, dim3(nbl), dim3(256), 0, st, in, stride, n_cap, n_ptr, out, scratch, nbl, PgRareArgs{}, total_out);
        return hipSuccess;
    }
    if (rare) PG_HIP(pg_launch_read_stats_rare(st, *rare));
    uint64_t *partial = scratch + 72;
    PG_LAUNCH(k_scan_partials, dim3(nbl), dim3(256), 0, st, in, stride, n_cap, n_ptr, partial);
    PG_LAUNCH(k_scan_partials_scan, dim3(1), dim3(256), 0, st, partial, nbl);
    PG_LAUNCH(k_scan_apply, dim3(nbl), dim3(256), 0, st, in, stride, n_cap, n_ptr, (const uint64_t *)partial, out, total_out);
    return hipSuccess;
}

__global__ __launch_bounds__(256) void k_base_open(const uint64_t *__restrict__ all_counts, uint32_t rows_below, uint32_t n_slots, uint64_t limit, uint32_t *__restrict__ flag) {
    bool open = false;
    for (uint32_t s = blockIdx.x * 256 + threadIdx.x; s < n_slots; s += gridDim.x * 256) {
        uint64_t base = 0;
        for (uint32_t h = 0; h < rows_below; ++h) base += all_counts[(uint64_t)h * n_slots + s];
        open |= base < limit;
    }
    if (__ballot(open) && lane_id() == 0) atomicOr(flag, 1u);
}
__global__ __launch_bounds__(256) void k_stats_cancel(uint32_t *__restrict__ flag, PgStatRec *__restrict__ rec, uint32_t n_reads) {
    if (flag[0] != 0) return;
    const uint32_t r = blockIdx.x * 256 + threadIdx.x;
    if (r < n_reads && rec[r].mode == PG_STAT_RUN) rec[r].mode = PG_STAT_SKIP;
    if (r == 0) flag[1] = 1u;
}
hipError_t pg_launch_stats_cancel_if_full(hipStream_t st, const uint64_t *all_counts, uint32_t rows_below, uint32_t n_slots, uint64_t limit, uint32_t *flag, void *plan_buf, uint32_t n_reads) {
    PG_HIP(hipMemsetAsync(flag, 0, 8, st));
    const uint32_t nb = (n_slots + 255) / 256;
    PG_LAUNCH(k_base_open, dim3(nb < 512u ? nb : 512u), dim3(256), 0, st, all_counts, rows_below, n_slots, limit, flag);
    if (n_reads) PG_LAUNCH(k_stats_cancel, dim3((n_reads + 255) / 256), dim3(256), 0, st, flag, reinterpret_cast<PgStatRec *>(plan_buf), n_reads);
    return hipSuccess;
}

__global__ void k_settle_pack(const uint32_t *__restrict__ errflag, const int32_t *__restrict__ stat_err, const int32_t *__restrict__ long_cnt, const uint64_t *__restrict__ totals,
                              const uint64_t *__restrict__ samp_off, uint64_t samp_off_entries, const uint32_t *__restrict__ cancel_flag, const uint32_t *__restrict__ front_word,
                              PgSettlePack *__restrict__ out) {
    PgSettlePack p;
    for (int i = 0; i < 6; ++i) p.errflag[i] = errflag[i];
    for (int i = 0; i < 4; ++i) p.stat_err[i] = stat_err ? stat_err[i] : (i == 0 ? INT_MAX : 0);
    p.stat_err[4] = long_cnt[0]; p.stat_err[5] = long_cnt[1];
    p.n_kept = totals[0]; p.full_slots = totals[1];
    p.n_samples = p.n_kept < samp_off_entries ? samp_off[p.n_kept] : 0;
    p.cancel[0] = cancel_flag ? cancel_flag[0] : 0u; p.cancel[1] = cancel_flag ? cancel_flag[1] : 0u;
    p.front[0] = front_word ? front_word[0] : 0u;
    p.front[1] = front_word && front_word[0] ? front_word[2] : 0u;
    *out = p;
}
hipError_t pg_launch_settle_pack(hipStream_t st, const uint32_t *errflag, const int32_t *stat_err, const int32_t *long_cnt, const uint64_t *totals, const uint64_t *samp_off,
                                 uint64_t samp_off_entries, const uint32_t *cancel_flag, const uint32_t *front_word, PgSettlePack *out) {
    PG_LAUNCH(k_settle_pack, dim3(1), dim3(1), 0, st, errflag, stat_err, long_cnt, totals, samp_off, samp_off_entries, cancel_flag, front_word, out);
    return hipSuccess;
}

hipError_t pg_launch_read_stats_rare(hipStream_t st, const PgRareArgs &A) {
    if (A.B.n_reads == 0) return hipSuccess;
    const uint32_t want = A.wide_blocks < 64 ? 64u : (A.wide_blocks > 2048 ? 2048u : A.wide_blocks);
    const uint32_t wide_blocks = A.B.n_reads < want ? A.B.n_reads : want;
    PG_LAUNCH(k_read_stats_rare, dim3(wide_blocks + PG_HUGE_BLOCKS), dim3(64), 0, st, A);
    return hipSuccess;
}

template <bool RARE> __global__ __launch_bounds__(256) void k_len_partials(const PgKeptRec *__restrict__ rec, const uint64_t *__restrict__ n_kept_ptr, uint32_t chunk, uint32_t n_chunks,
                                                                          uint64_t *__restrict__ part, PgRareArgs A) {
    if (RARE) {
        __shared__ __attribute__((aligned(16))) uint32_t rare_hist[4][PG_RARE_LDS_WORDS];
        if (blockIdx.x >= n_chunks) {
            const uint32_t workers = (gridDim.x - n_chunks) * 4u;
            rare_worker((blockIdx.x - n_chunks) * 4u + (threadIdx.x >> 6), workers - PG_HUGE_BLOCKS, rare_hist[threadIdx.x >> 6], A);
            return;
        }
    }
    __shared__ uint64_t wsum[4];
    const uint64_t n = n_kept_ptr[0], e0 = (uint64_t)blockIdx.x * chunk;
    uint64_t s = 0;
    if (e0 < n) {
        const uint64_t cnt = n - e0 < chunk ? n - e0 : chunk;
        const uint32_t *__restrict__ lens = reinterpret_cast<const uint32_t *>(rec + e0) + 2;
        for (uint64_t i0 = threadIdx.x; i0 < cnt; i0 += 4 * 256) {
            uint32_t v[4];
#pragma unroll
            for (int u = 0; u < 4; ++u) { const uint64_t i = i0 + (uint64_t)u * 256; v[u] = i < cnt ? lens[4 * i] : 0u; }
            s += (uint64_t)v[0] + v[1] + v[2] + v[3];
        }
    }
    for (int o = 32; o >= 1; o >>= 1) s += __shfl_xor(s, o, WAVE);
    if (lane_id() == 0) wsum[threadIdx.x >> 6] = s;
    __syncthreads();
    if (threadIdx.x == 0) {
        const uint64_t t = wsum[0] + wsum[1] + wsum[2] + wsum[3];
        part[blockIdx.x] = t;
        if (t) atomicAdd(reinterpret_cast<unsigned long long *>(part + PG_CHUNK_FINE + (blockIdx.x >> 6)), (unsigned long long)t);
    }
}
hipError_t pg_launch_len_partials(hipStream_t st, uint64_t n_kept_cap, const uint64_t *n_kept_ptr, const PgKeptRec *rec, uint64_t *part, const PgRareArgs *rare) {
    if (n_kept_cap == 0) { if (rare) return pg_launch_read_stats_rare(st, *rare); return hipSuccess; }
    uint32_t m; const uint32_t n_chunks = pg_gather_chunks(n_kept_cap, &m);
    if (rare && rare->B.n_reads) {
        const uint32_t want = rare->wide_blocks < 64 ? 64u : (rare->wide_blocks > 2048 ? 2048u : rare->wide_blocks);
        const uint32_t extra = (want + PG_HUGE_BLOCKS + 3) / 4;
        PG_LAUNCH(k_len_partials<true>, dim3(n_chunks + extra), dim3(256), 0, st, rec, n_kept_ptr, m * 1024u, n_chunks, part, *rare);
    } else PG_LAUNCH(k_len_partials<false>, dim3(n_chunks), dim3(256), 0, st, rec, n_kept_ptr, m * 1024u, n_chunks, part, PgRareArgs{});
    return hipSuccess;
}


hipError_t pg_launch_read_plan(hipStream_t st, const PgDevBatch &B, const uint8_t *read_needed, double pa_min, double pa_max, void *plan_buf,
                         int32_t *flags, int32_t *stat_status, bool flags_are_reset, const PgLongState &LS) {
    if (B.n_reads == 0) {
        if (!flags_are_reset) PG_LAUNCH(k_stat_flags_init, dim3(1), dim3(1), 0, st, flags);
        return hipSuccess;
    }
    PG_LAUNCH(k_read_plan, dim3((B.n_reads + 255) / 256), dim3(256), 0, st, B, read_needed, pa_min, pa_max,
                       reinterpret_cast<PgStatRec *>(plan_buf), stat_status, flags_are_reset ? (int32_t *)nullptr : flags, LS);
    return hipSuccess;
}

hipError_t pg_launch_read_stats(hipStream_t st, const PgDevBatch &B, const void *plan_buf, double *med, double *mad, int32_t *status, int32_t *err, int win,
                                uint32_t *wide_list, int32_t *wide_count, uint8_t *oor, int range_only, double *gcal, const PgLongState &LS,
                                const unsigned long long *cut_word, uint32_t batch_id, uint32_t group_from) {
    if (B.n_reads == 0) return hipSuccess;
    const PgStatRec *plan = reinterpret_cast<const PgStatRec *>(plan_buf);
    static_assert(PG_STATS_WPB == 1, "the group workgroups and the helpers of long reads are addressed as workgroups behind the reads' own");
    const uint32_t r1 = cut_word ? std::min(group_from, B.n_reads) : B.n_reads;
    const uint32_t n_groups = (B.n_reads - r1 + PG_STATS_GROUP - 1) / PG_STATS_GROUP;
    PG_LAUNCH(k_read_stats, dim3(r1 + n_groups + (LS.tab ? LS.cap : 0u)), dim3(64 * PG_STATS_WPB), 0, st, B, plan, med, mad, status, err, win, oor, range_only, wide_list, wide_count,
              B.n_reads / PG_STATS_CACHED_FRACTION, gcal, LS, cut_word, batch_id, r1, n_groups);
    return hipSuccess;
}
uint32_t pg_stats_group_from(uint32_t n_reads, uint64_t n_ops, uint32_t front_tiles) {
    if (n_ops == 0) return n_reads;
    const uint64_t est = ((uint64_t)n_reads * front_tiles * PG_SORT_TILE + n_ops - 1) / n_ops;
    return (uint32_t)std::min<uint64_t>(n_reads, est + est / 4 + 64);
}

template <int PER_WG> __global__ __launch_bounds__(256) void k_merge_segments(const PgSeg *__restrict__ seg, uint32_t n_seg, double *__restrict__ dst) {
    const uint32_t si = PER_WG == 1 ? blockIdx.x : blockIdx.x * PER_WG + (threadIdx.x >> 6);
    if (si >= n_seg) return;
    const PgSeg sg = seg[si];
    const double *__restrict__ src = sg.src;
    double *__restrict__ d = dst + sg.dst_off;
    const uint32_t t = PER_WG == 1 ? threadIdx.x : (uint32_t)lane_id(), step = PER_WG == 1 ? 256u : (uint32_t)WAVE;
    for (uint64_t i = t; i < sg.n; i += step) d[i] = src[i];
}
hipError_t pg_launch_merge_segments(hipStream_t st, const PgSeg *d_seg, uint32_t n_seg, double *dst, uint64_t n_total) {
    if (!n_seg) return hipSuccess;
    if (n_total / n_seg >= 1024) PG_LAUNCH(k_merge_segments<1>, dim3(n_seg), dim3(256), 0, st, d_seg, n_seg, dst);
    else PG_LAUNCH(k_merge_segments<4>, dim3((n_seg + 3) / 4), dim3(256), 0, st, d_seg, n_seg, dst);
    return hipSuccess;
}

hipError_t pg_launch_gather(hipStream_t st, const PgDevBatch &B, uint64_t n_kept_cap, const uint64_t *n_kept_ptr, const PgKeptRec *rec,
                      const uint64_t *samp_off, int scaling, double pa_min,
                      double pa_max, const double *med, const double *mad, double *samples, const double *gcal) {
    if (n_kept_cap == 0) return hipSuccess;
    uint64_t blocks = (n_kept_cap + 15) / 16;
    if (blocks > 256ull * 32) blocks = 256ull * 32;
    PG_LAUNCH(k_gather, dim3((uint32_t)blocks), dim3(256), 0, st, B, n_kept_ptr, rec, samp_off, scaling,
                       pa_min, pa_max, med, mad, samples, gcal);
    return hipSuccess;
}
```

### poregen_amd/csrc/pg_stats_plan.h

```cpp
#pragma once
#include "../../include/pgmove.h"
#include <cstdint>

enum PgStatsPlace { PG_STATS_NONE = 0, PG_STATS_OOR_FIRST, PG_STATS_SECOND_STREAM, PG_STATS_CHAIN, PG_STATS_TAIL_FORK, PG_STATS_DEFERRED, PG_STATS_LAZY };

struct PgStatsPlan {
    PgStatsPlace place;
    bool behind_cut;
    bool one_stream_batch;
    bool records_in_init;
    bool flags_in_init;
    bool rare_with_scan;
};

static inline bool pg_stats_on_second_stream(PgStatsPlace p) { return p == PG_STATS_SECOND_STREAM || p == PG_STATS_TAIL_FORK; }

static inline PgStatsPlan pg_stats_plan(uint32_t ctx_flags, int32_t scaling, uint32_t front_tiles, uint32_t n_reads, bool front_two_streams) {
    const bool skip_oor = (ctx_flags & PG_FLAG_SKIP_OUT_OF_RANGE) != 0;
    const bool lazy = !skip_oor && scaling == 1 && (ctx_flags & PG_FLAG_LAZY_STATS) != 0;
    const bool eager = skip_oor || (scaling == 1 && !lazy);
    const bool ctx_overlap = !skip_oor && (ctx_flags & PG_FLAG_OVERLAP) != 0;
    PgStatsPlan p{};
    p.behind_cut = front_tiles != 0 && eager && !skip_oor && !(ctx_flags & PG_FLAG_PROFILE);
    p.one_stream_batch = ctx_overlap && p.behind_cut && !front_two_streams;
    if (skip_oor) p.place = PG_STATS_OOR_FIRST;
    else if (lazy) p.place = PG_STATS_LAZY;
    else if (!eager) p.place = PG_STATS_NONE;
    else if (ctx_overlap) p.place = p.one_stream_batch ? PG_STATS_CHAIN : PG_STATS_SECOND_STREAM;
    else if (ctx_flags & PG_FLAG_DEFER_STATS) p.place = PG_STATS_DEFERRED;
    else if (ctx_flags & PG_FLAG_OVERLAP_TAIL) p.place = PG_STATS_TAIL_FORK;
    else p.place = PG_STATS_CHAIN;
    const bool second_from_start = ctx_overlap && !p.one_stream_batch;
    p.records_in_init = eager && !second_from_start && n_reads > 0;
    p.flags_in_init = !second_from_start;
    p.rare_with_scan = p.place == PG_STATS_CHAIN || p.place == PG_STATS_DEFERRED || p.place == PG_STATS_LAZY;
    return p;
}

static inline bool pg_stats_fork_waits(bool batch_is_host, bool user_stream, bool batch_resident, bool prev_one_stream) {
    return batch_is_host || (user_stream && !batch_resident) || prev_one_stream;
}
```

Measured before the change: 2463 billion samples/s.

## Fuse per-read stats kernel into the direct rank-emit launch

Adds a combined kernel that launches rank-emit workgroups and per-read median/MAD stats waves in one grid. The stats are no longer a separate launch before the collect step. In the chained, behind-cut placement with direct non-dense slots, the stats launch is deferred into collect and merged with emit so both workloads share the GPU concurrently. The goal is to remove a launch and the serialization between the two phases. The cost is an LDS footprint sized to the larger of the two users, which may lower occupancy, plus new ordering and grid-size tunables.

```diff
diff --git a/poregen_amd/csrc/pg_api.hip b/poregen_amd/csrc/pg_api.hip
--- a/poregen_amd/csrc/pg_api.hip
+++ b/poregen_amd/csrc/pg_api.hip
@@ -43,6 +43,7 @@
     bool all_matches = false;
     bool cut_in_scan = false;
     bool stats_pending = false;
+    bool emit_fused = false;
     bool rare_pending = false;
     PgRareArgs rare{};
 };
@@ -80,7 +81,7 @@
     PgDev<> blk_read, gen_flag, gen_list, cum, btot, tile_read;
     uint32_t batch_id = 0;
     BatchState bt;
-    uint64_t front_complete = 0, front_missed = 0, stats_cut_batches = 0, stats_cut_reads = 0, front_one_stream = 0;
+    uint64_t front_complete = 0, front_missed = 0, stats_cut_batches = 0, stats_cut_reads = 0, front_one_stream = 0, emit_stats_fused = 0;
     PgEvent ev_front;
     bool prev_one_stream = false;
     uint32_t gen_reads = 0;
@@ -502,7 +503,8 @@
 }
 
 static pg_status fill_long(pg_ctx *c, PgLongState &LS, bool ensure);
-static pg_status launch_stats(pg_ctx *c) {
+struct EmitArgs { const uint32_t *ev_slot; uint64_t n; uint32_t n_slots; const PgSortBufs *S; const uint64_t *keep, *ev_off, *totals; const PgWalkParams *W; const PgWalkOut *O; const PgKeptOut *K; };
+static pg_status launch_stats(pg_ctx *c, const EmitArgs *emit = nullptr) {
     const PgStatsPlan &P = c->bt.plan;
     hipStream_t st = pg_stats_on_second_stream(P.place) ? c->st2.h : c->st;
     const uint8_t *needed = P.place == PG_STATS_LAZY ? c->read_needed.as<uint8_t>() : nullptr;
@@ -527,7 +529,14 @@
         const char *ov = getenv("PGMOVE_STATS_GROUP_FROM");
         group_from = ov ? (uint32_t)std::min<unsigned long long>(strtoull(ov, nullptr, 10), 0xffffffffull) : pg_stats_group_from(c->B.n_reads, c->B.n_ops, c->bt.front_tiles);
     }
-    prof_begin(c, "k_read_stats", st);
+    prof_begin(c, emit ? "k_emit_stats" : "k_read_stats", st);
+    if (emit) {
+        PG_HIP_TRY(c, pg_launch_emit_stats(st, emit->ev_slot, emit->n, emit->n_slots, *emit->S, emit->keep, emit->ev_off, emit->totals, c->B, *emit->W, *emit->O, *emit->K,
+                             c->read_plan[sl].p, c->med[sl].as<double>(), c->mad[sl].as<double>(), c->stat_status[sl].as<int32_t>(), flags, win,
+                             c->wide_list[sl].as<uint32_t>(), flags + 1, oor, range_only, c->gcal[sl].as<double>(), LS,
+                             cut ? c->errflag.as<unsigned long long>() + 5 : nullptr, c->batch_id, group_from));
+        c->bt.emit_fused = true;
+    } else
     PG_HIP_TRY(c, pg_launch_read_stats(st, c->B, c->read_plan[sl].p, c->med[sl].as<double>(), c->mad[sl].as<double>(),
                          c->stat_status[sl].as<int32_t>(), flags, win, c->wide_list[sl].as<uint32_t>(), flags + 1, oor, range_only,
                          c->gcal[sl].as<double>(), LS, cut ? c->errflag.as<unsigned long long>() + 5 : nullptr, c->batch_id, group_from));
@@ -726,7 +735,7 @@
     c->slot ^= 1;
     c->bt.front_tiles = front_tiles_for(c, N, counts_out != nullptr);
     const PgFront FR{c->bt.front_tiles, c->errflag.as<uint32_t>() + 8};
-    const PgStatsPlan P = c->bt.plan = pg_stats_plan(c->prm.flags, c->prm.scaling, FR.tiles, n, getenv("PGMOVE_FRONT_TWO_STREAMS") != nullptr);
+    const PgStatsPlan P = c->bt.plan = pg_stats_plan(c->prm.flags, c->prm.scaling, FR.tiles, n, getenv("PGMOVE_FRONT_TWO_STREAMS") != nullptr, getenv("PGMOVE_NO_EMIT_STATS") != nullptr);
     if (P.one_stream_batch && c->stats_in_flight) PG_HIP_TRY(c, hipStreamWaitEvent(c->st, c->ev_join[c->slot ^ 1], 0));
     if (P.place == PG_STATS_SECOND_STREAM) {
         if (pg_stats_fork_waits(c->batch_is_host, c->user_stream, (b->flags & PG_BATCH_RESIDENT) != 0, c->prev_one_stream)) {
@@ -833,8 +842,8 @@
     }
 
     c->stats_in_flight = false;
-    c->bt.stats_pending = P.place == PG_STATS_DEFERRED;
-    if (P.place == PG_STATS_SECOND_STREAM || P.place == PG_STATS_CHAIN || P.place == PG_STATS_TAIL_FORK) {
+    c->bt.stats_pending = P.place == PG_STATS_DEFERRED || P.with_emit;
+    if (!P.with_emit && (P.place == PG_STATS_SECOND_STREAM || P.place == PG_STATS_CHAIN || P.place == PG_STATS_TAIL_FORK)) {
         if (P.place == PG_STATS_TAIL_FORK) {
             PG_HIP_TRY(c, hipEventRecord(c->ev_fork, c->st));
             PG_HIP_TRY(c, hipStreamWaitEvent(c->st2, c->ev_fork, 0));
@@ -903,10 +912,11 @@
     if (!c->have_count) return pg_fail(c, PG_ERR_STATE, "pg_collect without a preceding pg_count");
     PG_HIP_TRY(c, hipSetDevice(c->device));
     double tmark_ = timing_on() ? wall_now() : 0.0;
-    { pg_status s2 = launch_pending_stats(c); if (s2 != PG_OK) return s2; }
     const uint32_t ns = c->prm.n_slots;
     const uint64_t N = c->B.n_ops;
     const bool direct = ns <= PG_DIRECT_MAX_SLOTS;
+    const bool emit_stats = c->bt.stats_pending && c->bt.plan.with_emit && direct && !dense_direct(c, N);
+    if (!emit_stats) { pg_status s2 = launch_pending_stats(c); if (s2 != PG_OK) return s2; }
     const uint64_t *d_base = c->running.as<uint64_t>();
     PgGathered G{};
     if (all_counts) {
@@ -954,10 +964,16 @@
     if (direct) {
         PgSortBufs S{};
         fill_sort(c, S, 0);
+        if (emit_stats) {
+            const EmitArgs EA{O.ev_slot, N, ns, &S, c->keep.as<uint64_t>(), c->ev_off.as<uint64_t>(), totals, &W, &O, &K};
+            c->bt.stats_pending = false;
+            pg_status s2 = launch_stats(c, &EA); if (s2 != PG_OK) return s2;
+        } else {
         prof_begin(c, "k_rank_emit", c->st);
         if (dense_direct(c, N)) PG_HIP_TRY(c, pg_launch_rank_emit2(c->st, O.ev_slot, N, ns, S.hist, c->keep.as<uint64_t>(), c->ev_off.as<uint64_t>(), totals, c->B, W, O, K, c->part_Bp.as<uint32_t>()));
         else PG_HIP_TRY(c, pg_launch_rank_direct_emit(c->st, O.ev_slot, N, ns, S, c->keep.as<uint64_t>(), c->ev_off.as<uint64_t>(), totals, c->B, W, O, K));
         prof_end(c, c->st);
+        }
     } else if (c->part_mode) {
         PgPartBufs P{};
         fill_part(c, P, N ? N : 1);
@@ -1052,6 +1068,7 @@
     const PgSettlePack pk = *c->settle_host.p;
     if (c->bt.front_tiles) { if (pk.front[0]) c->front_complete++; else c->front_missed++; }
     if (c->bt.plan.one_stream_batch) c->front_one_stream++;
+    if (c->bt.emit_fused) c->emit_stats_fused++;
     if (c->bt.plan.behind_cut && pk.front[0]) { c->stats_cut_batches++; c->stats_cut_reads += c->B.n_reads - std::min(pk.front[1], c->B.n_reads); }
     pg_status s = check_read_errors(c, pk);
     if (s != PG_OK) { c->have_batch_result = false; c->downloaded = true; return s; }
@@ -1544,6 +1561,10 @@
         if (out && n < cap) { out[n].name = "stats_cut_reads"; out[n].launches = c->stats_cut_reads; out[n].total_ms = 0.0; }
         n++;
     }
+    if (c->emit_stats_fused) {
+        if (out && n < cap) { out[n].name = "emit_stats_fused"; out[n].launches = c->emit_stats_fused; out[n].total_ms = 0.0; }
+        n++;
+    }
     if (c->front_one_stream) {
         if (out && n < cap) { out[n].name = "front_one_stream"; out[n].launches = c->front_one_stream; out[n].total_ms = 0.0; }
         n++;
@@ -1571,7 +1592,7 @@
     PG_HIP_TRY(c, hipStreamSynchronize(c->st));
     if (c->st2) PG_HIP_TRY(c, hipStreamSynchronize(c->st2));
     prof_drain(c);
-    c->prof_acc.clear(); c->prof_names.clear(); c->stats_cancelled = 0; c->long_reads_split = 0; c->long_helpers_short = 0; c->front_complete = 0; c->front_missed = 0; c->stats_cut_batches = 0; c->stats_cut_reads = 0; c->front_one_stream = 0;
+    c->prof_acc.clear(); c->prof_names.clear(); c->stats_cancelled = 0; c->long_reads_split = 0; c->long_helpers_short = 0; c->front_complete = 0; c->front_missed = 0; c->stats_cut_batches = 0; c->stats_cut_reads = 0; c->front_one_stream = 0; c->emit_stats_fused = 0;
     for (uint64_t &f : c->gather_forms) f = 0;
     c->sort_scatters = 0;
     return PG_OK;
diff --git a/poregen_amd/csrc/pg_hosttest.cpp b/poregen_amd/csrc/pg_hosttest.cpp
--- a/poregen_amd/csrc/pg_hosttest.cpp
+++ b/poregen_amd/csrc/pg_hosttest.cpp
@@ -198,6 +198,9 @@
 extern "C" void pgt_stats_plan(uint32_t ctx_flags, int32_t scaling, uint32_t front_tiles, uint32_t n_reads, int front_two_streams, int32_t *out6) {
     const PgStatsPlan p = pg_stats_plan(ctx_flags, scaling, front_tiles, n_reads, front_two_streams != 0);
     out6[0] = p.place; out6[1] = p.behind_cut; out6[2] = p.one_stream_batch; out6[3] = p.records_in_init; out6[4] = p.flags_in_init; out6[5] = p.rare_with_scan;
+}
+extern "C" int pgt_stats_plan_with_emit(uint32_t ctx_flags, int32_t scaling, uint32_t front_tiles, uint32_t n_reads, int front_two_streams, int no_emit_stats) {
+    return pg_stats_plan(ctx_flags, scaling, front_tiles, n_reads, front_two_streams != 0, no_emit_stats != 0).with_emit ? 1 : 0;
 }
 extern "C" int pgt_stats_fork_waits(int batch_is_host, int user_stream, int batch_resident, int prev_one_stream) {
     return pg_stats_fork_waits(batch_is_host != 0, user_stream != 0, batch_resident != 0, prev_one_stream != 0) ? 1 : 0;
diff --git a/poregen_amd/csrc/pg_internal.h b/poregen_amd/csrc/pg_internal.h
--- a/poregen_amd/csrc/pg_internal.h
+++ b/poregen_amd/csrc/pg_internal.h
@@ -290,6 +290,10 @@
 hipError_t pg_launch_read_stats(hipStream_t st, const PgDevBatch &B, const void *plan_buf, double *med, double *mad, int32_t *status, int32_t *err, int win,
                                 uint32_t *wide_list, int32_t *wide_count, uint8_t *oor, int range_only, double *gcal, const PgLongState &LS,
                                 const unsigned long long *cut_word = nullptr, uint32_t batch_id = 0, uint32_t group_from = 0xffffffffu);
+hipError_t pg_launch_emit_stats(hipStream_t st, const uint32_t *ev_slot, uint64_t n, uint32_t n_slots, const PgSortBufs &S, const uint64_t *keep, const uint64_t *ev_off,
+                                const uint64_t *totals, const PgDevBatch &B, const PgWalkParams &W, const PgWalkOut &O, const PgKeptOut &K,
+                                const void *plan_buf, double *med, double *mad, int32_t *status, int32_t *err, int win, uint32_t *wide_list, int32_t *wide_count, uint8_t *oor,
+                                int range_only, double *gcal, const PgLongState &LS, const unsigned long long *cut_word, uint32_t batch_id, uint32_t group_from);
 uint32_t pg_stats_group_from(uint32_t n_reads, uint64_t n_ops, uint32_t front_tiles);
 struct PgSeg { const double *src; uint64_t dst_off, n; };
 hipError_t pg_launch_merge_segments(hipStream_t st, const PgSeg *d_seg, uint32_t n_seg, double *dst, uint64_t n_total );
diff --git a/poregen_amd/csrc/pg_kernels.hip b/poregen_amd/csrc/pg_kernels.hip
--- a/poregen_amd/csrc/pg_kernels.hip
+++ b/poregen_amd/csrc/pg_kernels.hip
@@ -1133,21 +1133,20 @@
 #define PG_EMIT_WAVES 16
 #define PG_EMIT_GRID 512
 #define PG_EMIT_ROWS (PG_SORT_TILE / (PG_EMIT_WAVES * WAVE))
-__global__ __launch_bounds__(PG_EMIT_WAVES * WAVE) void k_rank_emit(const uint32_t *__restrict__ keys, uint32_t n, int nbits, uint32_t n_slots, uint32_t n_tiles,
-                                                   const uint32_t *__restrict__ hist,
-                                                   const uint64_t *__restrict__ keep, const uint64_t *__restrict__ ev_off,
-                                                   const uint64_t *__restrict__ totals, PgDevBatch B, PgWalkParams W, PgWalkOut O,
-                                                   PgKeptOut K) {
-    __shared__ uint32_t wbase[PG_EMIT_WAVES][PG_RANK_MAX_DIGITS];
-    __shared__ uint32_t s_keep[PG_RANK_MAX_DIGITS], s_off[PG_RANK_MAX_DIGITS];
+__device__ __forceinline__ void rank_emit_block(uint32_t (*wbase)[PG_RANK_MAX_DIGITS], uint32_t *s_keep, uint32_t *s_off, const uint32_t bid, const uint32_t grid,
+                                                const uint32_t *__restrict__ keys, uint32_t n, int nbits, uint32_t n_slots, uint32_t n_tiles,
+                                                const uint32_t *__restrict__ hist,
+                                                const uint64_t *__restrict__ keep, const uint64_t *__restrict__ ev_off,
+                                                const uint64_t *__restrict__ totals, const PgDevBatch B, const PgWalkParams W, const PgWalkOut O,
+                                                const PgKeptOut K) {
     static_assert(PG_RANK_MAX_DIGITS <= PG_EMIT_WAVES * WAVE, "one digit per thread");
     const uint32_t tid = threadIdx.x, w = tid >> 6;
     const int lane = lane_id();
     const uint32_t ndig = 1u << nbits;
     PG_PROBE_BEGIN(2);
     const int64_t last_tile = (int64_t)totals[3];
-    for (uint32_t tile = blockIdx.x; tile < n_tiles && (int64_t)tile <= last_tile; tile += gridDim.x) {
-    if (tile != blockIdx.x) __syncthreads();
+    for (uint32_t tile = bid; tile < n_tiles && (int64_t)tile <= last_tile; tile += grid) {
+    if (tile != bid) __syncthreads();
     PG_MARK(2, 0);
     const uint32_t tile_first = O.tile_read[tile];
     const uint64_t base = (uint64_t)tile * PG_SORT_TILE + (uint64_t)w * PG_EMIT_ROWS * WAVE;
@@ -1235,8 +1234,18 @@
         if (K.read_needed) K.read_needed[rd[row]] = 1;
     }
     PG_MARK(2, 5);
-    if (tile == blockIdx.x) PG_PROBE_END(2, tile * PG_EMIT_WAVES + w);
-    }
+    if (tile == bid) PG_PROBE_END(2, tile * PG_EMIT_WAVES + w);
+    }
+}
+
+__global__ __launch_bounds__(PG_EMIT_WAVES * WAVE) void k_rank_emit(const uint32_t *__restrict__ keys, uint32_t n, int nbits, uint32_t n_slots, uint32_t n_tiles,
+                                                   const uint32_t *__restrict__ hist,
+                                                   const uint64_t *__restrict__ keep, const uint64_t *__restrict__ ev_off,
+                                                   const uint64_t *__restrict__ totals, PgDevBatch B, PgWalkParams W, PgWalkOut O,
+                                                   PgKeptOut K) {
+    __shared__ uint32_t wbase[PG_EMIT_WAVES][PG_RANK_MAX_DIGITS];
+    __shared__ uint32_t s_keep[PG_RANK_MAX_DIGITS], s_off[PG_RANK_MAX_DIGITS];
+    rank_emit_block(wbase, s_keep, s_off, blockIdx.x, gridDim.x, keys, n, nbits, n_slots, n_tiles, hist, keep, ev_off, totals, B, W, O, K);
 }
 
 
@@ -2134,16 +2143,11 @@
     PG_PROBE_END(0, r);
 }
 
-__global__ __launch_bounds__(64 * PG_STATS_WPB) __attribute__((amdgpu_waves_per_eu(PG_STATS_WAVES_PER_EU, PG_STATS_WAVES_PER_EU))) void k_read_stats(PgDevBatch B, const PgStatRec *__restrict__ rec, double *__restrict__ med,
-                                                   double *__restrict__ mad, int32_t *__restrict__ status, int32_t *__restrict__ err,
-                                                   int win, uint8_t *__restrict__ oor, int range_only, uint32_t *__restrict__ wide_list,
-                                                   int32_t *__restrict__ wide_count, uint32_t keep_cached, double *__restrict__ gcal, PgLongState LS,
-                                                   const unsigned long long *__restrict__ cut_word, uint32_t batch_id, uint32_t r1, uint32_t n_groups) {
-    __shared__ __attribute__((aligned(16))) uint32_t hist_all[PG_STATS_WPB][StatsGeom<1024>::LDS_WORDS];
-    static_assert(StatsGeom<1024>::LDS_WORDS + 1 <= PG_LONG_WORDS, "a long read's histogram in global memory");
-    static_assert(PG_STATS_WPB == 1, "the group workgroups and the helpers of long reads are found from blockIdx.x: [0, r1) reads, [r1, r1 + n_groups) groups, then helper blockIdx.x - r1 - n_groups");
-    uint32_t *hist = hist_all[0];
-    const uint32_t b = blockIdx.x;
+__device__ __forceinline__ void read_stats_wave(const uint32_t b, uint32_t *hist, const PgDevBatch &B, const PgStatRec *__restrict__ rec, double *__restrict__ med,
+                                                double *__restrict__ mad, int32_t *__restrict__ status, int32_t *__restrict__ err,
+                                                int win, uint8_t *__restrict__ oor, int range_only, uint32_t *__restrict__ wide_list,
+                                                int32_t *__restrict__ wide_count, uint32_t keep_cached, double *__restrict__ gcal, const PgLongState &LS,
+                                                const unsigned long long *__restrict__ cut_word, uint32_t batch_id, uint32_t r1, uint32_t n_groups) {
     const int lane = lane_id();
     uint32_t r = b;
     uint32_t slice = 0, base = 0;
@@ -2191,6 +2195,58 @@
         __builtin_amdgcn_wave_barrier();
         if (PG_STATS_SETPRIO) __builtin_amdgcn_s_setprio(0);
     }
+}
+
+__global__ __launch_bounds__(64 * PG_STATS_WPB) __attribute__((amdgpu_waves_per_eu(PG_STATS_WAVES_PER_EU, PG_STATS_WAVES_PER_EU))) void k_read_stats(PgDevBatch B, const PgStatRec *__restrict__ rec, double *__restrict__ med,
+                                                   double *__restrict__ mad, int32_t *__restrict__ status, int32_t *__restrict__ err,
+                                                   int win, uint8_t *__restrict__ oor, int range_only, uint32_t *__restrict__ wide_list,
+                                                   int32_t *__restrict__ wide_count, uint32_t keep_cached, double *__restrict__ gcal, PgLongState LS,
+                                                   const unsigned long long *__restrict__ cut_word, uint32_t batch_id, uint32_t r1, uint32_t n_groups) {
+    __shared__ __attribute__((aligned(16))) uint32_t hist_all[PG_STATS_WPB][StatsGeom<1024>::LDS_WORDS];
+    static_assert(StatsGeom<1024>::LDS_WORDS + 1 <= PG_LONG_WORDS, "a long read's histogram in global memory");
+    static_assert(PG_STATS_WPB == 1, "the group workgroups and the helpers of long reads are found from blockIdx.x: [0, r1) reads, [r1, r1 + n_groups) groups, then helper blockIdx.x - r1 - n_groups");
+    read_stats_wave(blockIdx.x, hist_all[0], B, rec, med, mad, status, err, win, oor, range_only, wide_list, wide_count, keep_cached, gcal, LS, cut_word, batch_id, r1, n_groups);
+}
+
+#ifndef PG_FUSED_EMIT_GRID
+#define PG_FUSED_EMIT_GRID 256
+#endif
+#ifndef PG_FUSED_ORDER
+#define PG_FUSED_ORDER 0
+#endif
+#ifndef PG_FUSED_STRIDED
+#define PG_FUSED_STRIDED 0
+#endif
+struct PgStatsArgs {
+    const PgStatRec *rec; double *med, *mad; int32_t *status, *err; int win; uint8_t *oor; int range_only; uint32_t *wide_list; int32_t *wide_count;
+    uint32_t keep_cached; double *gcal; PgLongState LS; const unsigned long long *cut_word; uint32_t batch_id, r1, n_groups;
+    uint32_t n_wgs;
+};
+__global__ __launch_bounds__(PG_EMIT_WAVES * WAVE) void k_emit_stats(uint32_t E, uint32_t n_sb, const uint32_t *__restrict__ keys, uint32_t n, int nbits, uint32_t n_slots, uint32_t n_tiles,
+                                                    const uint32_t *__restrict__ hist, const uint64_t *__restrict__ keep, const uint64_t *__restrict__ ev_off,
+                                                    const uint64_t *__restrict__ totals, PgDevBatch B, PgWalkParams W, PgWalkOut O, PgKeptOut K, PgStatsArgs A) {
+    constexpr uint32_t EMIT_WORDS = (PG_EMIT_WAVES + 2u) * PG_RANK_MAX_DIGITS, STAT_WORDS = PG_EMIT_WAVES * StatsGeom<1024>::LDS_WORDS;
+    static_assert(StatsGeom<1024>::LDS_WORDS % 4 == 0, "every wave's histogram 16-byte aligned");
+    __shared__ __attribute__((aligned(16))) uint32_t lds[EMIT_WORDS > STAT_WORDS ? EMIT_WORDS : STAT_WORDS];
+    const uint32_t bx = blockIdx.x;
+    bool emit; uint32_t idx;
+    if (PG_FUSED_ORDER == 0) { emit = bx < E; idx = emit ? bx : bx - E; }
+    else if (PG_FUSED_ORDER == 1) { emit = bx >= n_sb; idx = emit ? bx - n_sb : bx; }
+    else {
+        const uint32_t m = E < n_sb ? E : n_sb;
+        if (bx < 2u * m) { emit = !(bx & 1u); idx = bx >> 1; }
+        else { emit = E > n_sb; idx = bx - m; }
+    }
+    if (emit) {
+        rank_emit_block(reinterpret_cast<uint32_t (*)[PG_RANK_MAX_DIGITS]>(lds), lds + PG_EMIT_WAVES * PG_RANK_MAX_DIGITS, lds + (PG_EMIT_WAVES + 1u) * PG_RANK_MAX_DIGITS,
+                        idx, E, keys, n, nbits, n_slots, n_tiles, hist, keep, ev_off, totals, B, W, O, K);
+        return;
+    }
+    const uint32_t w = threadIdx.x >> 6;
+    const uint32_t v = (uint32_t)__builtin_amdgcn_readfirstlane((int)(PG_FUSED_STRIDED ? w * n_sb + idx : idx * PG_EMIT_WAVES + w));
+    if (v >= A.n_wgs) return;
+    read_stats_wave(v, lds + w * StatsGeom<1024>::LDS_WORDS, B, A.rec, A.med, A.mad, A.status, A.err, A.win, A.oor, A.range_only, A.wide_list, A.wide_count, A.keep_cached, A.gcal,
+                    A.LS, A.cut_word, A.batch_id, A.r1, A.n_groups);
 }
 
 static_assert(PG_RARE_LDS_WORDS == StatsGeom<PG_STATS_BINS>::LDS_WORDS, "k_scan_chained's rare histogram");
@@ -2582,6 +2638,24 @@
               B.n_reads / PG_STATS_CACHED_FRACTION, gcal, LS, cut_word, batch_id, r1, n_groups);
     return hipSuccess;
 }
+hipError_t pg_launch_emit_stats(hipStream_t st, const uint32_t *ev_slot, uint64_t n, uint32_t n_slots, const PgSortBufs &S, const uint64_t *keep, const uint64_t *ev_off,
+                                const uint64_t *totals, const PgDevBatch &B, const PgWalkParams &W, const PgWalkOut &O, const PgKeptOut &K,
+                                const void *plan_buf, double *med, double *mad, int32_t *status, int32_t *err, int win, uint32_t *wide_list, int32_t *wide_count, uint8_t *oor,
+                                int range_only, double *gcal, const PgLongState &LS, const unsigned long long *cut_word, uint32_t batch_id, uint32_t group_from) {
+    int nbits = 1; while ((1u << nbits) < n_slots) ++nbits;
+    const uint32_t n_tiles = pg_tiles(n, true);
+    const uint32_t E = n_tiles < PG_FUSED_EMIT_GRID ? n_tiles : PG_FUSED_EMIT_GRID;
+    PgStatsArgs A{};
+    A.rec = reinterpret_cast<const PgStatRec *>(plan_buf); A.med = med; A.mad = mad; A.status = status; A.err = err; A.win = win; A.oor = oor; A.range_only = range_only;
+    A.wide_list = wide_list; A.wide_count = wide_count; A.keep_cached = B.n_reads / PG_STATS_CACHED_FRACTION; A.gcal = gcal; A.LS = LS; A.cut_word = cut_word; A.batch_id = batch_id;
+    A.r1 = cut_word ? std::min(group_from, B.n_reads) : B.n_reads;
+    A.n_groups = (B.n_reads - A.r1 + PG_STATS_GROUP - 1) / PG_STATS_GROUP;
+    A.n_wgs = B.n_reads ? A.r1 + A.n_groups + (LS.tab ? LS.cap : 0u) : 0u;
+    const uint32_t n_sb = (A.n_wgs + PG_EMIT_WAVES - 1) / PG_EMIT_WAVES;
+    if (E + n_sb == 0) return hipSuccess;
+    PG_LAUNCH(k_emit_stats, dim3(E + n_sb), dim3(PG_EMIT_WAVES * WAVE), 0, st, E, n_sb, ev_slot, (uint32_t)n, nbits, n_slots, n_tiles, (const uint32_t *)S.hist, keep, ev_off, totals, B, W, O, K, A);
+    return hipSuccess;
+}
 uint32_t pg_stats_group_from(uint32_t n_reads, uint64_t n_ops, uint32_t front_tiles) {
     if (n_ops == 0) return n_reads;
     const uint64_t est = ((uint64_t)n_reads * front_tiles * PG_SORT_TILE + n_ops - 1) / n_ops;
diff --git a/poregen_amd/csrc/pg_stats_plan.h b/poregen_amd/csrc/pg_stats_plan.h
--- a/poregen_amd/csrc/pg_stats_plan.h
+++ b/poregen_amd/csrc/pg_stats_plan.h
@@ -11,11 +11,12 @@
     bool records_in_init;
     bool flags_in_init;
     bool rare_with_scan;
+    bool with_emit;
 };
 
 static inline bool pg_stats_on_second_stream(PgStatsPlace p) { return p == PG_STATS_SECOND_STREAM || p == PG_STATS_TAIL_FORK; }
 
-static inline PgStatsPlan pg_stats_plan(uint32_t ctx_flags, int32_t scaling, uint32_t front_tiles, uint32_t n_reads, bool front_two_streams) {
+static inline PgStatsPlan pg_stats_plan(uint32_t ctx_flags, int32_t scaling, uint32_t front_tiles, uint32_t n_reads, bool front_two_streams, bool no_emit_stats = false) {
     const bool skip_oor = (ctx_flags & PG_FLAG_SKIP_OUT_OF_RANGE) != 0;
     const bool lazy = !skip_oor && scaling == 1 && (ctx_flags & PG_FLAG_LAZY_STATS) != 0;
     const bool eager = skip_oor || (scaling == 1 && !lazy);
@@ -34,6 +35,7 @@
     p.records_in_init = eager && !second_from_start && n_reads > 0;
     p.flags_in_init = !second_from_start;
     p.rare_with_scan = p.place == PG_STATS_CHAIN || p.place == PG_STATS_DEFERRED || p.place == PG_STATS_LAZY;
+    p.with_emit = p.place == PG_STATS_CHAIN && p.behind_cut && !no_emit_stats;
     return p;
 }
 
```

New measurement: 2670 billion samples/s (median of 6 runs). 1.08x the previous value.
